# facebookresearch/gtn

Hardware: AMD Instinct MI355X
Metric: CTC forward+backward losses/sec (T=1000, C=256) (higher is better)
Workload: dtype f32; 1 GPU; BASELINE config C3: compose(ctc_target, emissions)+forwardScore CTC loss fwd+bwd, T=1000, C=256, U=100, batch=512 per GPU; global_batch=512, parallelism=dp1 (utterance sharding, all_gather of losses), rccl_ranks=0

## Files before the change

### gtn_amd/_capi.py

```python
import ctypes as C
import os

c_graph = C.c_void_p
c_graph_p = C.POINTER(C.c_void_p)
c_i32_p = C.POINTER(C.c_int)
c_i64_p = C.POINTER(C.c_int64)
c_u8_p = C.POINTER(C.c_uint8)
c_f32_p = C.POINTER(C.c_float)

GRAD_FN = C.CFUNCTYPE(C.c_int, C.c_void_p, c_graph_p, C.c_int, c_graph)
CTX_FREE = C.CFUNCTYPE(None, C.c_void_p)

OK, INVALID_ARGUMENT, LOGIC_ERROR, RUNTIME_ERROR, OUT_OF_RANGE, DEVICE_ERROR = range(6)

_SIGS = {
    "gtnx_set_device": [C.c_int],
    "gtnx_get_device": [c_i32_p],
    "gtnx_set_stream": [C.c_void_p],
    "gtnx_compose_mode": [C.c_int, C.POINTER(C.c_int)],
    "gtnx_synchronize": [],
    "gtnx_memory_stats": [C.POINTER(C.c_uint64), C.POINTER(C.c_uint64)],
    "gtnx_empty_cache": [],
    "gtnx_reclaim": [],
    "gtnx_graph_create": [C.c_int, c_graph_p],
# ... 5 lines not shown
    "gtnx_graph_add_nodes": [c_graph, C.c_int, C.c_void_p, C.c_void_p],
    "gtnx_graph_add_arcs": [c_graph, C.c_int, C.c_void_p, C.c_void_p, C.c_void_p, C.c_void_p, C.c_void_p],
    "gtnx_graph_num_nodes": [c_graph, c_i64_p],
    "gtnx_graph_num_arcs": [c_graph, c_i64_p],
    "gtnx_graph_num_start": [c_graph, c_i64_p],
    "gtnx_graph_num_accept": [c_graph, c_i64_p],
    "gtnx_graph_item": [c_graph, c_f32_p],
    "gtnx_graph_arc_sort": [c_graph, C.c_int],
    "gtnx_graph_mark_arc_sorted": [c_graph, C.c_int],
    "gtnx_graph_ilabel_sorted": [c_graph, c_i32_p],
    "gtnx_graph_olabel_sorted": [c_graph, c_i32_p],
    "gtnx_graph_weights": [c_graph, C.c_int, C.POINTER(c_f32_p)],
    "gtnx_graph_get_weights": [c_graph, C.c_void_p],
    "gtnx_graph_set_weights": [c_graph, C.c_void_p],
    "gtnx_graph_set_weights_device": [c_graph, C.c_void_p],
    "gtnx_graph_weights_device": [c_graph, C.POINTER(C.c_void_p)],
    "gtnx_graph_labels_to_array": [c_graph, C.c_void_p, C.c_int],
    "gtnx_graph_get_start": [c_graph, C.c_void_p],
    "gtnx_graph_get_accept": [c_graph, C.c_void_p],
    "gtnx_graph_is_start": [c_graph, C.c_int, c_i32_p],
    "gtnx_graph_is_accept": [c_graph, C.c_int, c_i32_p],
    "gtnx_graph_make_accept": [c_graph, C.c_int],
    "gtnx_graph_num_out": [c_graph, C.c_int, c_i64_p],
    "gtnx_graph_num_in": [c_graph, C.c_int, c_i64_p],
    "gtnx_graph_get_out": [c_graph, C.c_int, C.c_void_p],
    "gtnx_graph_get_in": [c_graph, C.c_int, C.c_void_p],
    "gtnx_graph_get_arcs": [c_graph, C.c_void_p, C.c_void_p, C.c_void_p, C.c_void_p],
    "gtnx_graph_get_arc": [c_graph, C.c_int, c_i32_p, c_i32_p, c_i32_p, c_i32_p, c_f32_p],
    "gtnx_graph_set_weight": [c_graph, C.c_int, C.c_float],
    "gtnx_graph_calc_grad": [c_graph, c_i32_p],
    "gtnx_graph_set_calc_grad": [c_graph, C.c_int],
    "gtnx_graph_is_grad_available": [c_graph, c_i32_p],
    "gtnx_graph_grad": [c_graph, c_graph_p],
    "gtnx_graph_zero_grad": [c_graph],
    "gtnx_graph_add_grad": [c_graph, C.c_void_p, C.c_int64],
    "gtnx_graph_add_grad_graph": [c_graph, c_graph],
    "gtnx_graph_id": [c_graph, C.POINTER(C.c_size_t)],
    "gtnx_graph_create_op": [c_graph_p, C.c_int, GRAD_FN, C.c_void_p, CTX_FREE, c_graph_p],
    "gtnx_graph_num_inputs": [c_graph, c_i64_p],
    "gtnx_graph_get_input": [c_graph, C.c_int, c_graph_p],
    "gtnx_graph_set_inputs": [c_graph, c_graph_p, C.c_int],
    "gtnx_graph_set_grad_fn": [c_graph, GRAD_FN, C.c_void_p, CTX_FREE],
    "gtnx_graph_has_grad_fn": [c_graph, c_i32_p],
    "gtnx_scalar_graph": [C.c_float, C.c_int, c_graph_p],
    "gtnx_linear_graph": [C.c_int, C.c_int, C.c_int, c_graph_p],
    "gtnx_linear_graph_n": [C.c_int, C.c_int, C.c_int, C.c_int, C.c_void_p, c_graph_p],
    "gtnx_linear_graph_borrow_n": [C.c_int, C.c_int, C.c_int, C.c_int, C.c_void_p, c_graph_p],
    "gtnx_negate": [c_graph, c_graph_p],
    "gtnx_add": [c_graph, c_graph, c_graph_p],
    "gtnx_subtract": [c_graph, c_graph, c_graph_p],
    "gtnx_compose": [c_graph, c_graph, c_graph_p],
    "gtnx_intersect": [c_graph, c_graph, c_graph_p],
    "gtnx_forward_score": [c_graph, c_graph_p],
    "gtnx_viterbi_score": [c_graph, c_graph_p],
    "gtnx_viterbi_path": [c_graph, c_graph_p],
    "gtnx_negate_n": [c_graph_p, C.c_int, c_graph_p],
    "gtnx_add_n": [c_graph_p, C.c_int, c_graph_p, C.c_int, c_graph_p],
    "gtnx_subtract_n": [c_graph_p, C.c_int, c_graph_p, C.c_int, c_graph_p],
    "gtnx_compose_n": [c_graph_p, C.c_int, c_graph_p, C.c_int, c_graph_p],
    "gtnx_intersect_n": [c_graph_p, C.c_int, c_graph_p, C.c_int, c_graph_p],
    "gtnx_forward_score_n": [c_graph_p, C.c_int, c_graph_p],
    "gtnx_viterbi_score_n": [c_graph_p, C.c_int, c_graph_p],
    "gtnx_viterbi_path_n": [c_graph_p, C.c_int, c_graph_p],
    "gtnx_items_n": [c_graph_p, C.c_int, C.c_void_p],
    "gtnx_items_device_n": [c_graph_p, C.c_int, C.c_void_p],
    "gtnx_grads_device_n": [c_graph_p, C.c_int, C.c_void_p, C.c_void_p],
    "gtnx_grads_bind_device_n": [c_graph_p, C.c_int, C.c_void_p, C.c_void_p],
    "gtnx_clone": [c_graph, C.c_int, c_graph_p],
    "gtnx_concat": [c_graph_p, C.c_int, c_graph_p],
    "gtnx_closure": [c_graph, c_graph_p],
    "gtnx_union": [c_graph_p, C.c_int, c_graph_p],
    "gtnx_batch_from_graphs": [c_graph_p, C.c_int, c_graph_p],
    "gtnx_batch_ctc_targets": [C.c_void_p, C.c_void_p, C.c_int, C.c_int, C.c_int, c_graph_p],
    "gtnx_batch_asg_force_align": [C.c_void_p, C.c_void_p, C.c_int, c_graph, C.c_int, c_graph_p],
    "gtnx_batch_linear": [C.c_int, C.c_int, C.c_int, C.c_int, C.c_void_p, C.c_int, c_graph_p],
    "gtnx_batch_linear_rows": [C.c_int, C.c_int, C.c_int, C.c_void_p, C.c_int, C.c_void_p, C.c_int, c_graph_p],
    "gtnx_batch_destroy": [c_graph],
    "gtnx_batch_size": [c_graph, c_i32_p],
    "gtnx_batch_get": [c_graph, C.c_int, c_graph_p],
    "gtnx_batch_negate": [c_graph, c_graph_p],
    "gtnx_batch_add": [c_graph, c_graph, c_graph_p],
    "gtnx_batch_subtract": [c_graph, c_graph, c_graph_p],
    "gtnx_batch_subtract_into": [c_graph, c_graph, C.c_void_p, c_graph_p],
    "gtnx_batch_compose": [c_graph, c_graph, c_graph_p],
    "gtnx_batch_intersect": [c_graph, c_graph, c_graph_p],
    "gtnx_batch_forward_score": [c_graph, c_graph_p],
    "gtnx_batch_viterbi_score": [c_graph, c_graph_p],
    "gtnx_batch_viterbi_path": [c_graph, c_graph_p],
    "gtnx_batch_viterbi_align": [c_graph, C.c_void_p, C.c_void_p, C.c_int64, C.c_void_p, C.c_void_p],
    "gtnx_batch_align_stats": [c_i64_p, c_i64_p],
    "gtnx_batch_viterbi_decode": [c_graph, c_graph, C.c_void_p, C.c_void_p, C.c_int64, C.c_void_p, C.c_void_p,
                                  C.c_void_p],
    "gtnx_batch_decode_stats": [c_i64_p, c_i64_p],
    "gtnx_batch_full_connect_stats": [c_i64_p, c_i64_p],
    "gtnx_batch_linear_decode": [c_graph, C.c_void_p, C.c_int, C.c_void_p, C.c_int64, C.c_void_p, C.c_void_p,
                                 C.c_void_p, C.c_void_p],
    "gtnx_batch_linear_decode_stats": [c_i64_p, c_i64_p],
    "gtnx_batch_ctc_beam_decode": [c_graph, C.c_void_p, C.c_int, C.c_int, C.c_int, C.c_int, C.c_void_p, C.c_int64,
                                   C.c_void_p, C.c_void_p],
    "gtnx_batch_ctc_beam_stats": [c_i64_p, c_i64_p],
    "gtnx_batch_linear_shape": [c_graph, c_i32_p, c_i32_p],
    "gtnx_batch_edit_distance": [C.c_void_p, C.c_int64, C.c_void_p, C.c_void_p, C.c_int64, C.c_void_p, C.c_int, C.c_int,
                                 C.c_int, C.c_int, C.c_void_p, C.c_void_p],
    "gtnx_batch_edit_distance_stats": [c_i64_p, c_i64_p],
    "gtnx_batch_backward": [c_graph, C.c_int],
    "gtnx_batch_items": [c_graph, C.c_void_p],
    "gtnx_batch_items_device": [c_graph, C.c_void_p],
    "gtnx_batch_grads_bind_device": [c_graph, C.c_void_p, C.c_void_p],
    "gtnx_batch_grads_device": [c_graph, C.c_void_p, C.c_void_p],
    "gtnx_backward": [c_graph, C.c_int],
    "gtnx_backward_with_grad": [c_graph, c_graph, C.c_int],
    "gtnx_backward_n": [c_graph_p, C.c_int, C.c_int],
    "gtnx_equal": [c_graph, c_graph, c_i32_p],
    "gtnx_isomorphic": [c_graph, c_graph, c_i32_p],
    "gtnx_remove": [c_graph, C.c_int, C.c_int, c_graph_p],
    "gtnx_graph_load_buffer": [C.c_void_p, C.c_size_t, c_graph_p],
    "gtnx_parallel_enter": [],
    "gtnx_parallel_leave": [],
    "gtnx_parallel_flush": [],
    "gtnx_prof_enable": [C.c_int],
    "gtnx_prof_reset": [],
    "gtnx_prof_get": [C.c_char_p, C.POINTER(C.c_double), c_i64_p, C.POINTER(C.c_double)],
    "gtnx_prof_names": [C.c_char_p, C.c_size_t],
    "gtnx_debug_symbolic_route": [c_graph, C.c_int, c_i32_p],
    "gtnx_debug_route_name": [C.c_int, C.c_char_p, C.c_size_t],
    "gtnx_debug_viterbi_ties": [c_i64_p, c_i64_p],
    "gtnx_debug_tie_ranks": [c_graph, C.c_void_p, C.c_void_p, C.c_void_p],
    "gtnx_comm_create": [c_i32_p, C.c_int, C.POINTER(C.c_void_p)],
    "gtnx_comm_destroy": [C.c_void_p],
    "gtnx_comm_size": [C.c_void_p, c_i32_p],
    "gtnx_comm_all_gather_f32": [C.c_void_p, C.POINTER(C.c_void_p), C.POINTER(C.c_void_p), C.c_int64],
    "gtnx_comm_all_reduce_sum_f32": [C.c_void_p, C.POINTER(C.c_void_p), C.c_int64],
}

_RESTYPE = {
    "gtnx_last_error": (C.c_char_p, []),
    "gtnx_version": (C.c_char_p, []),
    "gtnx_backend": (C.c_char_p, []),
    "gtnx_device_count": (C.c_int, []),
}

ALL_SYMBOLS = sorted(list(_SIGS) + list(_RESTYPE))


def default_library_path():
    return os.path.join(os.path.dirname(os.path.abspath(__file__)), "lib", "libgtn_amd.so")


def load(path=None):
    path = path or default_library_path()
    if not os.path.exists(path):
        raise ImportError(
            f"gtn_amd: native library not found at {path}. Build it with "
            "`python -c 'import __graft_entry__ as g; g.build()'` (hipcc, gfx950). "
            "There is no CPU fallback."
        )
    lib = C.CDLL(path, mode=C.RTLD_GLOBAL if hasattr(C, "RTLD_GLOBAL") else 0)
    for name, args in _SIGS.items():
        try:
            fn = getattr(lib, name)
        except AttributeError:
            if name.startswith("gtnx_batch_") or name.startswith("gtnx_comm_") or name in ("gtnx_linear_graph_borrow_n", "gtnx_grads_bind_device_n",
                                                             "gtnx_parallel_enter", "gtnx_parallel_leave", "gtnx_parallel_flush"):
                continue
            raise
        fn.argtypes = args
# ... 8 lines not shown
```

### gtn_amd/api.py

```python
import ctypes as C
import types

import numpy as np

from . import _capi

_EXC = {
    _capi.INVALID_ARGUMENT: ValueError,
    _capi.LOGIC_ERROR: RuntimeError,
    _capi.RUNTIME_ERROR: RuntimeError,
    _capi.OUT_OF_RANGE: IndexError,
    _capi.DEVICE_ERROR: RuntimeError,
}


class GtnError(RuntimeError):
    pass


def _is_seq(x):
    return isinstance(x, (list, tuple))


def make_api(lib):
# ... 698 lines not shown
                if stride is not None and t.stride(0) != stride:
                    raise ValueError("linear_decode: labels_out, collapsed_out and starts_out must have the same "
                                     "row stride")
                stride = t.stride(0)
            if stride is None:
                raise ValueError("linear_decode: a device address needs row_stride")
            if (lengths_out is not None or starts_out is not None) and collapsed_out is None:
                raise ValueError("linear_decode: lengths_out and starts_out need collapsed_out")
            fr = None if frames is None else np.ascontiguousarray(frames, dtype=np.int32)
            if fr is not None and fr.shape != (n,):
                raise ValueError("linear_decode: one frame count per element")
            check(lib.gtnx_batch_linear_decode(self._h, fr.ctypes.data if fr is not None else None, int(blank),
                                               _as_dev_ptr(labels_out), int(stride),
                                               _as_dev_ptr(scores_out) if scores_out is not None else None,
                                               _as_dev_ptr(collapsed_out) if collapsed_out is not None else None,
                                               _as_dev_ptr(starts_out) if starts_out is not None else None,
                                               _as_dev_ptr(lengths_out) if lengths_out is not None else None))

        def ctc_beam_decode(self, tokens_out, lengths_out, scores_out, frames=None, blank=0, beam_size=16,
                            cutoff_top_n=16, nbest=1, row_stride=None):
            n = len(self)
            stride = row_stride
            t = tokens_out
            if t is not None and hasattr(t, "data_ptr"):
                if (str(t.dtype) != "torch.int32" or t.dim() != 3 or t.shape[0] < n or t.shape[1] != int(nbest)
                        or (t.shape[2] > 1 and t.stride(2) != 1) or (n > 1 and t.stride(0) != t.shape[1] * t.stride(1))):
                    raise ValueError("ctc_beam_decode: tokens_out must be an int32 tensor [B, nbest, M] with contiguous "
                                     "rows, equally spaced")
                if stride is not None and t.stride(1) != stride:
                    raise ValueError("ctc_beam_decode: row_stride is not the row stride of tokens_out")
                stride = t.stride(1)
                m, c = C.c_int(-1), C.c_int(-1)
                check(lib.gtnx_batch_linear_shape(self._h, C.byref(m), C.byref(c)))
                if t.shape[2] < m.value:
                    raise ValueError(f"ctc_beam_decode: tokens_out has rows of {t.shape[2]} entries, the batch has "
                                     f"{m.value} rows")
            if stride is None:
                raise ValueError("ctc_beam_decode: a device address needs row_stride")
            for o, dt, what in ((lengths_out, "torch.int32", "lengths_out must be an int32"),
                                (scores_out, "torch.float32", "scores_out must be a float32")):
                if o is not None and hasattr(o, "data_ptr") and (str(o.dtype) != dt or not o.is_contiguous()
                                                                 or o.numel() < n * int(nbest)):
                    raise ValueError(f"ctc_beam_decode: {what} contiguous tensor [B, nbest]")
            fr = None if frames is None else np.ascontiguousarray(frames, dtype=np.int32)
            if fr is not None and fr.shape != (n,):
                raise ValueError("ctc_beam_decode: one frame count per element")
            check(lib.gtnx_batch_ctc_beam_decode(self._h, fr.ctypes.data if fr is not None else None, int(blank),
                                                 int(beam_size), int(cutoff_top_n), int(nbest),
                                                 _as_dev_ptr(tokens_out) if tokens_out is not None else None,
                                                 int(stride),
                                                 _as_dev_ptr(lengths_out) if lengths_out is not None else None,
                                                 _as_dev_ptr(scores_out) if scores_out is not None else None))

    ns.Batch = Batch

    def _batch_fn(cfn, *args):
        h = C.c_void_p()
        check(cfn(*[a._h for a in args], C.byref(h)))
        return Batch._from_handle(h.value)

    def _with_batches(plain, cfn):
        def f(*args, **kw):
            if args and all(isinstance(a, Batch) for a in args) and not kw:
                return _batch_fn(cfn, *args)
            return plain(*args, **kw)
        f.__doc__ = plain.__doc__
        f.__name__ = getattr(plain, "__name__", "f")
        return f

    if hasattr(lib, "gtnx_batch_negate"):
        for _name in ("negate", "add", "subtract", "compose", "intersect", "forward_score", "viterbi_score",
                      "viterbi_path"):
            setattr(ns, _name, _with_batches(getattr(ns, _name), getattr(lib, "gtnx_batch_" + _name)))

    def subtract_into(a, b, items_device):
        h = C.c_void_p()
        check(lib.gtnx_batch_subtract_into(a._h, b._h, _as_dev_ptr(items_device), C.byref(h)))
        r = Batch._from_handle(h.value)
        r._keep = items_device
        return r

    if hasattr(lib, "gtnx_batch_subtract_into"):
        ns.subtract_into = subtract_into

    _plain_backward = ns.backward

    def backward(g, grad_or_retain=None, retain_graph=False):
        if isinstance(g, Batch):
            r = grad_or_retain if isinstance(grad_or_retain, bool) else retain_graph
            check(lib.gtnx_batch_backward(g._h, int(bool(r))))
            return
        return _plain_backward(g, grad_or_retain, retain_graph)

    ns.backward = backward

    def parallel_for(fn, iterable):
        for i in iterable:
            fn(i)

    ns.parallel_for = parallel_for

    def backend():
        return lib.gtnx_backend().decode()

    def device_count():
        return lib.gtnx_device_count()

    def synchronize():
        check(lib.gtnx_synchronize())

    def set_device(i):
        check(lib.gtnx_set_device(int(i)))

    def set_stream(stream):
        check(lib.gtnx_set_stream(int(stream) if stream else None))

    def compose_mode(mode):
        prev = C.c_int()
        check(lib.gtnx_compose_mode(int(mode), C.byref(prev)))
        return prev.value

    def memory_stats():
        r, u = C.c_uint64(), C.c_uint64()
        check(lib.gtnx_memory_stats(C.byref(r), C.byref(u)))
        return {"reserved": r.value, "in_use": u.value}

    def prof_enable(on=True):
        check(lib.gtnx_prof_enable(int(bool(on))))

    def prof_reset():
        check(lib.gtnx_prof_reset())

    def prof_get(name):
        ms, n, b = C.c_double(), C.c_int64(), C.c_double()
        check(lib.gtnx_prof_get(name.encode(), C.byref(ms), C.byref(n), C.byref(b)))
        return {"total_ms": ms.value, "launches": n.value, "algorithmic_bytes": b.value}

    def prof_names():
        buf = C.create_string_buffer(4096)
        check(lib.gtnx_prof_names(buf, 4096))
        return [s for s in buf.value.decode().split("\n") if s]

    def debug_symbolic_route(g, tropical=False):
        r = C.c_int(-1)
        check(lib.gtnx_debug_symbolic_route(g._h, int(bool(tropical)), C.byref(r)))
        if r.value < 0:
            return None
        buf = C.create_string_buffer(32)
        check(lib.gtnx_debug_route_name(r.value, buf, 32))
        return buf.value.decode()

    def debug_viterbi_ties():
        a, b = C.c_int64(0), C.c_int64(0)
        check(lib.gtnx_debug_viterbi_ties(C.byref(a), C.byref(b)))
        return int(a.value), int(b.value)

    def debug_align_stats():
        a, b = C.c_int64(0), C.c_int64(0)
        check(lib.gtnx_batch_align_stats(C.byref(a), C.byref(b)))
        return int(a.value), int(b.value)

    def debug_decode_stats():
        a, b = C.c_int64(0), C.c_int64(0)
        check(lib.gtnx_batch_decode_stats(C.byref(a), C.byref(b)))
        return int(a.value), int(b.value)

# ... 137 lines not shown
```

### gtn_amd/criteria/ctc_criterion.h

```cpp
#pragma once

#include <chrono>
#include <cstdint>
#include <stdexcept>
#include <vector>

#include "gtn/gtn.h"

namespace gtn {
namespace criteria {

inline Graph ctcTargetGraph(const std::vector<int>& target, int blank = 0, bool calcGrad = true) {
  const int L = 2 * (int)target.size() + 1;
  std::vector<uint8_t> st(L, 0), ac(L, 0);
  std::vector<int> src, dst, lab;
  src.reserve(3 * L);
  dst.reserve(3 * L);
  lab.reserve(3 * L);
  for (int l = 0; l < L; l++) {
    const int idx = (l - 1) / 2;
    st[l] = l == 0;
    ac[l] = l == L - 1 || l + 2 == L;
    const int label = l % 2 ? target[idx] : blank;
    src.push_back(l), dst.push_back(l), lab.push_back(label);
    if (l > 0) src.push_back(l - 1), dst.push_back(l), lab.push_back(label);
    if (l % 2 && l > 1 && label != target[idx - 1]) src.push_back(l - 2), dst.push_back(l), lab.push_back(label);
  }
  Graph ctc(calcGrad);
  detail::check(gtnx_graph_add_nodes(ctc.handle(), L, st.data(), ac.data()));
  detail::check(gtnx_graph_add_arcs(ctc.handle(), (int)src.size(), src.data(), dst.data(), lab.data(), lab.data(), nullptr));
  ctc.arcSort();
  return ctc;
}

struct CtcStepTimes {
  double build = 0, linear = 0, intersect = 0, forward = 0, backward = 0;
};

inline void ctcLossBatch(
    const void* emissions,
    const int* labels,
    const int* lengths,
    int B,
    int T,
    int C,
    int blank,
    void* lossDev,
    void* gradDev,
    bool targetGrad = true,
    CtcStepTimes* times = nullptr,
    Batch* targetsOut = nullptr,
    const int* frames = nullptr) {
  auto now = [] { return std::chrono::steady_clock::now(); };
  auto ms = [](auto a, auto b) { return std::chrono::duration<double, std::milli>(b - a).count(); };
  if (frames)
    for (int b = 0; b < B; ++b)
      if (frames[b] < 1 || frames[b] > T) throw std::invalid_argument("[ctcLossBatch] a frame count outside 1 .. T");
  auto t0 = now();
  Batch ctcs = Batch::ctcTargets(labels, lengths, B, blank, targetGrad);
  auto t1 = now();
  Batch ems = Batch::linear(B, T, C, emissions, gradDev != nullptr, true, frames);
  std::vector<int64_t> off(B);
  for (int b = 0; b < B; ++b) off[b] = (int64_t)b * T * C;
  if (gradDev) ems.bindGrads(gradDev, off.data());
  auto t2 = now();
  Batch comp = batched::intersect(ctcs, ems);
  auto t3 = now();
  Batch score = batched::forwardScore(comp);
  Batch norm = batched::forwardScore(ems);
  Batch losses = batched::subtract(norm, score, lossDev);
  auto t4 = now();
  if (gradDev) batched::backward(losses);
  auto t5 = now();
  if (times) *times = {ms(t0, t1), ms(t1, t2), ms(t2, t3), ms(t3, t4), ms(t4, t5)};
  losses.itemsToDevice(lossDev);
  if (gradDev) ems.gradsToDevice(gradDev, off.data());
  if (targetsOut) *targetsOut = std::move(ctcs);
}

inline void ctcLossBatch(
    const void* emissions,
    const std::vector<std::vector<int>>& targets,
    int T,
    int C,
    int blank,
    void* lossDev,
    void* gradDev,
    bool targetGrad = true,
    CtcStepTimes* times = nullptr) {
  std::vector<int> flat, len;
  for (auto& t : targets) {
    flat.insert(flat.end(), t.begin(), t.end());
    len.push_back((int)t.size());
  }
  ctcLossBatch(emissions, flat.data(), len.data(), (int)targets.size(), T, C, blank, lossDev, gradDev, targetGrad, times);
}

inline void ctcAlignBatch(
    const void* emissions,
    const int* targets,
    const int* lengths,
    int B,
    int T,
    int C,
    int blank,
    const int* frames,
    void* labels,
    void* tokens,
    void* scores) {
  Batch ctcs = Batch::ctcTargets(targets, lengths, B, blank, false);
  Batch ems = Batch::linear(B, T, C, emissions, false, true);
  Batch comp = batched::intersect(ctcs, ems);
  batched::viterbiAlign(comp, static_cast<int*>(labels), T, static_cast<int*>(tokens), static_cast<float*>(scores), frames);
}

inline void ctcDecodeBatch(
    const void* emissions,
    int B,
    int T,
    int C,
    int blank,
    const int* frames,
    void* labelsDev,
    void* scoresDev,
    void* collapsedDev,
    void* startsDev,
    void* lengthsDev) {
  Batch ems = Batch::linear(B, T, C, emissions, false, true);
  batched::linearDecode(ems, static_cast<int*>(labelsDev), T, static_cast<float*>(scoresDev), frames, blank,
                        static_cast<int*>(collapsedDev), static_cast<int*>(startsDev), static_cast<int*>(lengthsDev));
}

inline void ctcBeamDecodeBatch(
    const void* emissions,
    int B,
    int T,
    int C,
    int blank,
    const int* frames,
    int beamSize,
    int cutoffTopN,
    int nbest,
    void* tokensDev,
    void* lengthsDev,
    void* scoresDev) {
  Batch ems = Batch::linear(B, T, C, emissions, false, true);
  batched::ctcBeamDecode(ems, static_cast<int*>(tokensDev), T, static_cast<int*>(lengthsDev),
                         static_cast<float*>(scoresDev), blank, beamSize, cutoffTopN, nbest, frames);
}

}
}
```

### gtn_amd/csrc/band.hip

```cpp
#include <hip/hip_runtime.h>

#include <algorithm>
#include <cstdlib>
#include <stdexcept>
#include <type_traits>

#include "kernels.h"

#ifdef GTNX_BAND_TIMING
__device__ long long g_band_timing[256];
#endif

namespace gtnx {
namespace {

constexpr float NEGF = -1.0e30f;
constexpr float DEADF = -1.0e29f;
constexpr float LOG2E = 1.44269504088896340736f;
constexpr double LN2 = 0.693147180559945309417;
constexpr int BW = 256;
constexpr int WG = 512;
constexpr int WGB = 768;
constexpr int NBE = 5;
constexpr int NBG = 7;
// ... 242 lines not shown
      for (int i = 0; i < NS / 4; ++i) {
        if (i > 0 && 4 * i * LN >= cnt) break;
        if (4 * (i * LN + tid) < cnt) {
          const int e = min(4 * (i * LN + tid), cnt - 4);
          const int r0 = row_of(e, W, invW), c0 = e - r0 * W;
#pragma unroll
          for (int k = 0; k < 4; ++k) {
            int r = r0, col = c0 + k;
            if (col >= W) {
              col -= W;
              ++r;
            }
            f(i, e + k, r, col, gtnx_f4{v[4 * i + k], 0.0f, 0.0f, 0.0f});
          }
        }
      }
    }
  }
};

struct BandLds {
  int CS;
  int o_ering, o_aring, o_oring, o_snode, o_misc, total;
};
__host__ __device__ inline BandLds band_lds(int C, int K, int NSmax, bool backward) {
  BandLds L;
  L.CS = C + 4;
  int o = 0;
  L.o_ering = o;
  o += (backward ? NBGE : NBE) * K * L.CS;
  o = (o + 3) & ~3;
  L.o_aring = o;
  o += backward ? NBE * K * NSmax : 0;
  o = (o + 3) & ~3;
  L.o_oring = o;
  o += backward ? max(NBG * K * NSmax, 2 * C) : 0;
  o = (o + 3) & ~3;
  L.o_snode = o;
  o += backward ? 512 : 0;
  L.o_misc = o;
  o += 160 + 32 + 8 + 2 * NBE * K * 4 + 40 * K + 8 + 512;
  L.total = o;
  return L;
}
struct BandMisc {
  double *offr, *red, *find, *aofr;
  float *bndr, *fin, *lsep;
};
template <int K>
__device__ __forceinline__ BandMisc band_misc(float* lds, const BandLds& L) {
  BandMisc m;
  m.offr = reinterpret_cast<double*>(lds + L.o_misc);
  m.red = m.offr + 80;
  m.find = m.red + 16;
  m.aofr = m.find + 4;
  m.bndr = lds + L.o_misc + 200 + 2 * NBE * K * 4;
  m.fin = m.bndr + 40 * K;
  m.lsep = m.fin + 8;
  return m;
}

__device__ __forceinline__ float wave_max_of(const float* v, int n) {
  float mx = v[0];
  for (int j = 1; j < n; ++j) mx = fmaxf(mx, v[j]);
  return wave_max(mx);
}

template <int NPL, bool UNIT, int K, bool VEC>
__global__ __launch_bounds__(WG) void band_forward_kernel(const BandPair* __restrict__ pairs, int NSmax) {
#define GTNX_BAND_PAIR pairs[blockIdx.x]
#include "band_forward_body.inc"
#undef GTNX_BAND_PAIR
}
template <int NPL, bool UNIT, int K, bool VEC>
__global__ __launch_bounds__(WG) void band_forward_one_kernel(BandPair one, int NSmax) {
#define GTNX_BAND_PAIR one
#include "band_forward_body.inc"
#undef GTNX_BAND_PAIR
}

__device__ __forceinline__ BandPair band_patched(BandPair P, const BandPatch& pt) {
  if (pt.on) {
    const int b = P.bidx;
    P.delta = pt.delta + b;
    P.delta_norm = pt.delta_norm ? pt.delta_norm + b : nullptr;
    P.rowlse = pt.rowlse ? pt.rowlse + int64_t(b) * pt.M : nullptr;
    P.norm = nullptr;
    P.em_copy = nullptr;
    P.grad_em = pt.grad_em ? pt.grad_em + int64_t(b) * pt.A : nullptr;
    P.grad_fixed = pt.grad_fixed ? pt.grad_fixed + P.goff : nullptr;
  }
  return P;
}
template <int NPL, bool UNIT, bool GRADG, int K, bool VEC, bool BIG>
__global__ __launch_bounds__(WGB, BIG ? 3 : 6) void band_backward_kernel(const BandPair* __restrict__ pairs, int NSmax, BandPatch patch) {
#define GTNX_BAND_PAIR band_patched(pairs[blockIdx.x], patch)
#include "band_backward_body.inc"
#undef GTNX_BAND_PAIR
}
template <int NPL, bool UNIT, bool GRADG, int K, bool VEC, bool BIG>
__global__ __launch_bounds__(WGB, BIG ? 3 : 6) void band_backward_one_kernel(BandPair one, int NSmax) {
#define GTNX_BAND_PAIR one
#include "band_backward_body.inc"
#undef GTNX_BAND_PAIR
}


__global__ __launch_bounds__(512) void ctc_targets_kernel(const CtcTargetArgs* __restrict__ args, int blank) {
  const CtcTargetArgs a = args[blockIdx.x];
  __shared__ __attribute__((aligned(16))) int tl[256 + 4];
  __shared__ __attribute__((aligned(16))) int tk[256 + 4];
  const int N = a.N, U = (N - 1) >> 1, m = threadIdx.x;
  if (m < 260) {
    const int v = m < U ? a.labels[m] : 0x7fffffff;
    tl[m] = v;
    tk[m] = (m > 0 && m < U && v != a.labels[m - 1]) ? 1 : 0;
  }
  __syncthreads();
  if (m >= N) return;
  const bool odd = (m & 1) != 0;
  const int my = odd ? tl[(m - 1) >> 1] : blank;
  const int skip = odd ? tk[(m - 1) >> 1] : 0;
  const int mi = (m - 1) >> 1;
  const int before = odd ? mi : (m >> 1);
  int rank = 0, skips = 0;
  for (int o = 0; o < U; o += 4) {
    const gtnx_i4 l4 = *reinterpret_cast<const gtnx_i4*>(tl + o), k4 = *reinterpret_cast<const gtnx_i4*>(tk + o);
    const int lo[4] = {l4.x, l4.y, l4.z, l4.w}, ko[4] = {k4.x, k4.y, k4.z, k4.w};
#pragma unroll
    for (int k = 0; k < 4; ++k) {
      const bool front = o + k < before;
      rank += (lo[k] < my || (lo[k] == my && front)) ? 1 : 0;
      skips += front ? ko[k] : 0;
    }
  }
  rank += blank < my ? U + 1 : (blank == my ? (m + 1) >> 1 : 0);
  const int base = (m > 0 ? 2 * m - 1 : 0) + skips;
  GTNX_G BandNode* nd = const_cast<GTNX_G BandNode*>(a.nodes);
  nd[m].lab = my;
  nd[m].aid[0] = base;
  nd[m].aid[1] = m > 0 ? base + 1 : -1;
  nd[m].aid[2] = skip ? base + 2 : -1;
  a.nflags[m] = uint8_t((m == 0 ? NF_START : 0) | (m + 2 >= N ? NF_ACCEPT : 0));
  a.snode[rank] = m;
  a.slab[rank] = my;
  if (m == N - 1 && a.n_arcs) a.n_arcs[0] = base + 1 + (m > 0 ? 1 : 0) + skip;
}

__global__ __launch_bounds__(512) void band_viterbi_kernel(const BandDecode* __restrict__ pairs) {
  const BandDecode P = pairs[blockIdx.x];
  const int T = P.T, C = P.C, N = P.N, NS = P.NS;
  extern __shared__ float lds[];
  const float NINF = -__builtin_inff();
  float* a0 = lds;
  float* a1 = lds + 516;
  float* stage = lds + 1032;
  const int m = threadIdx.x;
  const GTNX_G gtnx_i4* nodes = reinterpret_cast<const GTNX_G gtnx_i4*>(P.nodes);
  int lab = 0;
  float wi[3] = {NINF, NINF, NINF};
  bool accept = false, start = false;
  if (m < N) {
    const gtnx_i4 q = nodes[m];
    lab = q.x >= 0 ? q.x : 0;
    const int a[3] = {q.y, q.z, q.w};
#pragma unroll
    for (int k = 0; k < 3; ++k)
      if (a[k] >= 0) wi[k] = P.w ? P.w[a[k]] : 0.0f;
    const uint8_t f = P.nflags[m];
    start = (f & NF_START) != 0;
    accept = (f & NF_ACCEPT) != 0;
  }
  if (m < 2) a0[m] = a1[m] = NINF;
  a0[2 + m] = start ? 0.0f : NINF;
  a1[2 + m] = NINF;
  int tie = 0;
  const int R = max(1, min(64, P.stage_floats / C));
  float* cur = a0;
  float* nxt = a1;
  __syncthreads();
  for (int t0 = 0; t0 < T; t0 += R) {
    const int rows = min(R, T - t0);
    for (int e = threadIdx.x; e < rows * C; e += blockDim.x) stage[e] = P.em[int64_t(t0) * C + e];
    __syncthreads();
    for (int i = 0; i < rows; ++i) {
      const float e = stage[i * C + lab];
      const float c0 = cur[2 + m] + (wi[0] + e), c1 = cur[1 + m] + (wi[1] + e), c2 = cur[m] + (wi[2] + e);
      float best = c0;
      int k = 0;
      if (c1 > best) best = c1, k = 1;
      if (c2 > best) best = c2, k = 2;
      if (best > NINF && ((k != 0 && c0 == best) || (k != 1 && c1 == best) || (k != 2 && c2 == best))) tie = 1;
      if (m < NS) P.bp[int64_t(t0 + i) * NS + m] = uint8_t(best > NINF ? k : 3);
      nxt[2 + m] = m < N ? best : NINF;
      __syncthreads();
      float* sw = cur;
      cur = nxt;
      nxt = sw;
    }
  }
  __shared__ float red_v[8];
  __shared__ int red_m[8], s_best, s_tie;
  float v = accept ? cur[2 + m] : NINF;
  int bm = (m < N && accept && v > NINF) ? m : 1 << 30;
  const float wmx = wave_max(v);
  if (!(v == wmx)) bm = 1 << 30;
  int cnt = (bm != (1 << 30)) ? 1 : 0;
  for (int o = 32; o > 0; o >>= 1) {
    bm = min(bm, __shfl_xor(bm, o));
    cnt += __shfl_xor(cnt, o);
  }
  if ((threadIdx.x & 63) == 0) {
    red_v[threadIdx.x >> 6] = wmx;
    red_m[threadIdx.x >> 6] = bm;
  }
  if (cnt > 1) tie = 1;
  if (threadIdx.x == 0) s_tie = 0;
  __syncthreads();
  if (threadIdx.x == 0) {
    float bv = NINF;
    int bn = -1;
    for (int w = 0; w < 8; ++w) {
      if (red_m[w] == (1 << 30)) continue;
      if (red_v[w] > bv) bv = red_v[w], bn = red_m[w];
      else if (red_v[w] == bv && bv > NINF) s_tie = 1;
    }
    s_best = bn;
    P.score[0] = bv;
  }
// ... 419 lines not shown
  return 0;
}

bool band_one_ok(int npl, int C, int max_NS, bool vec, bool backward) {
  if (npl != 1 || !vec) return false;
  if (!backward) return true;
  const int K = band_block_rows(C, max_NS, true);
  return !(K * C > 1024 || K * max_NS > 1024);
}
void launch_band_forward(const BandPair* d_pairs, int n, int npl, int C, int max_NS, bool unit, bool vec, hipStream_t st,
                         const BandPair* one) {
  if (n <= 0) return;
  if (one && (n != 1 || !band_one_ok(npl, C, max_NS, vec, false))) throw std::logic_error("band.hip: not a single-pair launch");
  const int K = band_block_rows(C, 0, false);
  const size_t lds = 4 * size_t(band_lds(C, K, max_NS, false).total) + 64;
  if (npl == 1) {
    if (K == 8) launch_fwd<1, 8>(d_pairs, one, n, max_NS, lds, unit, vec, st);
    else if (K == 4) launch_fwd<1, 4>(d_pairs, one, n, max_NS, lds, unit, vec, st);
    else launch_fwd<1, 2>(d_pairs, one, n, max_NS, lds, unit, vec, st);
  } else {
    if (K == 8) launch_fwd<2, 8>(d_pairs, one, n, max_NS, lds, unit, vec, st);
    else if (K == 4) launch_fwd<2, 4>(d_pairs, one, n, max_NS, lds, unit, vec, st);
    else launch_fwd<2, 2>(d_pairs, one, n, max_NS, lds, unit, vec, st);
  }
}

void launch_band_backward(const BandPair* d_pairs, int n, int npl, int C, int max_NS, bool unit, bool gradg, bool vec,
                          hipStream_t st, const BandPair* one, const BandPatch* patch) {
  if (n <= 0) return;
  if (one && patch) throw std::logic_error("band.hip: a patched launch reads a device table");
  BandPatch pt{};
  if (patch) pt = *patch;
  if (one && (n != 1 || !band_one_ok(npl, C, max_NS, vec, true))) throw std::logic_error("band.hip: not a single-pair launch");
  const int K = band_block_rows(C, max_NS, true);
  const bool big = K * C > 1024 || K * max_NS > 1024;
  const int ns_lds = band_backward_lds_stride(K, max_NS);
  const size_t lds = 4 * size_t(band_lds(C, K, ns_lds, true).total) + 64;
  if (npl == 1) {
    if (K == 4) launch_bwd<1, 4>(d_pairs, one, n, ns_lds, lds, unit, gradg, vec, big, st, pt);
    else launch_bwd<1, 2>(d_pairs, one, n, ns_lds, lds, unit, gradg, vec, big, st, pt);
  } else {
    if (K == 4) throw std::logic_error("band.hip: four rows per block with two nodes per lane");
    launch_bwd<2, 2>(d_pairs, one, n, ns_lds, lds, unit, gradg, vec, big, st, pt);
  }
}

template <int NPL>
static void launch_viterbi_wave(const BandDecode* d_pairs, int n, int ranked, hipStream_t st) {
  if (ranked) hipLaunchKernelGGL((band_viterbi_wave_kernel<NPL, true>), dim3(n), dim3(64), 0, st, d_pairs);
  else hipLaunchKernelGGL((band_viterbi_wave_kernel<NPL, false>), dim3(n), dim3(64), 0, st, d_pairs);
}
bool band_viterbi_wave_ok(int max_nodes, int max_labels, int vec) {
  static const bool force_wg = std::getenv("GTNX_VITERBI_WG") != nullptr;
  return !force_wg && vec && max_nodes <= 512 && max_labels <= VBLK;
}
void launch_band_viterbi(const BandDecode* d_pairs, int n, int stage_floats, int max_nodes, int max_labels, int vec,
                         hipStream_t st, int ranked) {
  if (n <= 0) return;
  if (band_viterbi_wave_ok(max_nodes, max_labels, vec)) {
    if (max_nodes <= 64) launch_viterbi_wave<1>(d_pairs, n, ranked, st);
    else if (max_nodes <= 128) launch_viterbi_wave<2>(d_pairs, n, ranked, st);
    else if (max_nodes <= 256) launch_viterbi_wave<4>(d_pairs, n, ranked, st);
    else launch_viterbi_wave<8>(d_pairs, n, ranked, st);
    return;
  }
  if (ranked) return;
  static std::atomic<uint64_t> done{0};
  if (gtnx_first_on_device first{done}) big_lds(band_viterbi_kernel);
  hipLaunchKernelGGL(band_viterbi_kernel, dim3(n), dim3(512), 4 * size_t(1032 + stage_floats) + 64, st, d_pairs);
}

void launch_asg_fal_targets(const AsgFalArgs* d_args, int n, int n_labels, hipStream_t st) {
  if (n > 0) hipLaunchKernelGGL(asg_fal_targets_kernel, dim3(n), dim3(512), 0, st, d_args, n_labels);
}
void launch_asg_fal_scatter(const float* g, const int* maps, const int64_t* tab, int n_seq, int64_t longest, float* trans_grad,
                            hipStream_t st) {
  if (n_seq > 0 && longest > 0)
    hipLaunchKernelGGL(asg_fal_scatter_kernel, dim3(unsigned(std::min<int64_t>((longest + 255) / 256, 64)), unsigned(n_seq)),
                       dim3(256), 0, st, g, maps, tab, trans_grad);
}
void launch_ctc_targets(const CtcTargetArgs* d_args, int n, int blank, hipStream_t st) {
  if (n > 0) hipLaunchKernelGGL(ctc_targets_kernel, dim3(n), dim3(512), 0, st, d_args, blank);
}

}
```

### gtn_amd/csrc/batch.cpp

```cpp
#include "batch.h"

#include <algorithm>
#include <atomic>
#include <cstdlib>
#include <cstring>
#include <limits>
#include <unordered_map>
#include <unordered_set>

namespace gtnx {

namespace {

std::atomic<uint64_t> g_batch_seq{1};

struct CompMode {
  int old;
  CompMode() : old(compose_mode_hint(2)) {}
  ~CompMode() { compose_mode_hint(old); }
};

BatchP make_batch(Batch::Kind k, int n, bool cg) {
  auto b = std::make_shared<Batch>();
  b->kind = k;
  b->n = n;
  b->calc_grad = cg;
  return b;
}

BatchP result(Batch::Kind k, int n, std::shared_ptr<BatchOp> op) {
  bool cg = false;
  for (auto& i : op->inputs) cg |= i->calc_grad;
  BatchP r = make_batch(k, n, cg);
  op->seq = g_batch_seq.fetch_add(1);
  r->op = std::move(op);
  return r;
}

bool native(const Batch& b, Batch::Kind k) { return b.kind == k; }

void pad_fill(Batch& b, float* base, const int64_t* offs = nullptr) {
  if (b.kind != Batch::LINEAR || b.pad_floats <= 0) return;
  Runtime& rt = Runtime::get();
  const size_t n = size_t(b.n);
  const size_t rows_bytes = align_up(sizeof(int) * n, 256);
  if (!b.pad_mem) {
    std::vector<int64_t> tab(rows_bytes / 8 + n + 1);
    std::memcpy(tab.data(), b.rows.data(), sizeof(int) * n);
    int64_t* prefix = tab.data() + rows_bytes / 8;
    prefix[0] = 0;
    for (size_t i = 0; i < n; ++i) prefix[i + 1] = prefix[i] + int64_t(b.M - b.rows[i]) * b.C;
    b.pad_mem = upload_vec(tab);
  }
  PadFillArgs a{};
  a.base = base;
  a.rows = b.pad_mem->as<int>();
  a.prefix = reinterpret_cast<const int64_t*>(b.pad_mem->as<char>(rows_bytes));
  a.stride = int64_t(b.M) * b.C;
  a.n = b.n;
  a.C = b.C;
  DevMemP d_offs;
  if (offs) {
    d_offs = upload_vec(std::vector<int64_t>(offs, offs + n));
    a.offs = d_offs->as<int64_t>();
  }
  GTNX_PROF("linear_pad_fill", 4.0 * double(b.pad_floats));
  launch_pad_fill(a, b.pad_floats, rt.stream());
}

void alloc_grad(Batch& b, bool zero) {
  Runtime& rt = Runtime::get();
  b.g_off.resize(size_t(b.n) + 1);
  b.g_off[0] = 0;
  for (int i = 0; i < b.n; ++i) b.g_off[size_t(i) + 1] = b.g_off[size_t(i)] + b.elem_size(i);
  const size_t bytes = sizeof(float) * size_t(b.g_off[size_t(b.n)]);
  if (b.dest) {
    b.g_mem = b.dest_mem;
    b.g_dev = b.dest;
    b.dest = nullptr;
    if (zero && bytes) HIP_CHECK(hipMemsetAsync(b.g_dev, 0, bytes, rt.stream()));
  } else {
    b.g_mem = zero ? rt.alloc_zero(bytes ? bytes : 4) : rt.alloc(bytes ? bytes : 4);
    b.g_dev = b.g_mem->as<float>();
  }
  if (!zero) pad_fill(b, b.g_dev);
}

struct GradTarget {
  float* ptr = nullptr;
  DevMemP scratch;
};
GradTarget grad_target(Batch& b, bool zero) {
  GradTarget t;
  if (!b.g_dev) {
    alloc_grad(b, zero);
    t.ptr = b.g_dev;
    return t;
  }
  Runtime& rt = Runtime::get();
  const size_t bytes = sizeof(float) * size_t(b.g_off[size_t(b.n)]);
  t.scratch = zero ? rt.alloc_zero(bytes ? bytes : 4) : rt.alloc(bytes ? bytes : 4);
  t.ptr = t.scratch->as<float>();
  if (!zero) pad_fill(b, t.ptr);
  return t;
}
void add_scratch(Batch& b, const GradTarget& t) {
  if (!t.scratch) return;
  launch_vec_axpby(b.g_dev, t.ptr, nullptr, size_t(b.g_off[size_t(b.n)]), 1.0f, 0.0f, 1, Runtime::get().stream());
}

struct BScalarOp : BatchOp {
  ScalarKind kind;
  void backward(Batch& out) override {
    Runtime& rt = Runtime::get();
    for (size_t i = 0; i < inputs.size(); ++i) {
      Batch& in = *inputs[i];
      if (!in.calc_grad) continue;
      const float s = (kind == SK_NEGATE || (kind == SK_SUBTRACT && i == 1)) ? -1.0f : 1.0f;
      const bool have = in.g_dev != nullptr;
      if (!have) alloc_grad(in, false);
      launch_vec_axpby(in.g_dev, out.g_dev, nullptr, size_t(in.n), s, 0.0f, have ? 1 : 0, rt.stream());
    }
  }
};

struct BackwardPlan {
  std::unordered_map<Batch*, Batch*> lin;
  std::unordered_set<Batch*> fused;
};
thread_local BackwardPlan* t_plan = nullptr;
thread_local bool t_batch_retain = false;

struct BFsLinearOp : BatchOp {
  void backward(Batch& out) override {
    Batch& e = *inputs[0];
    if (!e.calc_grad) return;
    if (t_plan && e.nc_rowlse && !t_plan->lin.count(&e)) {
      t_plan->lin[&e] = &out;
      return;
    }
    run(out);
  }
  void run(Batch& out) {
    Batch& e = *inputs[0];
    Runtime& rt = Runtime::get();
    if (e.w_pend) e.w_pend->settle();
    const bool have = e.g_dev != nullptr;
    if (!have) alloc_grad(e, false);
    std::vector<LinArgs> args;
    args.resize(size_t(e.n));
    const size_t A = size_t(e.M) * size_t(e.C);
    for (int b = 0; b < e.n; ++b) {
      LinArgs& a = args[size_t(b)];
      a.w = e.w_dev + size_t(b) * A;
      a.M = e.rows_of(b);
      a.C = e.C;
      a.out_score = nullptr;
      a.partial = nullptr;
      a.delta = out.g_dev + b;
      a.grad = e.g_dev + size_t(b) * A;
      a.accumulate = have ? 1 : 0;
    }
    DevMemP d = upload_vec(args);
    const bool vec_rows = e.C % 4 == 0 && e.C <= 1024 && (reinterpret_cast<uintptr_t>(e.w_dev) & 15) == 0 &&
                          (reinterpret_cast<uintptr_t>(e.g_dev) & 15) == 0;
    GTNX_PROF("linear_forward_grad", (have ? 12.0 : 8.0) * double(A) * e.n);
    launch_linear_backward(d->as<LinArgs>(), e.n, 0, vec_rows ? 1 : 0, rt.stream());
  }
};

struct BFsBandOp : BatchOp {
  std::vector<BandPair> pairs;
  DevMemP arena;
  DevMemP fwd_table;
  DevMemP through_acc;
  void backward(Batch& out) override {
    Batch& prod = *inputs[0];
    Batch& fx = *prod.fixed;
    Batch& ch = *prod.chain;
    Runtime& rt = Runtime::get();
    const float* delta = out.g_dev;
    if (through_acc || t_batch_retain) {
      const size_t n = size_t(prod.n);
      if (!through_acc) through_acc = rt.alloc_zero(sizeof(float) * (n ? n : 1));
      launch_vec_axpby(through_acc->as<float>(), out.g_dev, nullptr, n, 1.0f, 0.0f, 1, rt.stream());
      delta = through_acc->as<float>();
    }
    GradTarget ge, gf;
    if (ch.calc_grad) ge = grad_target(ch, false);
    if (fx.calc_grad) gf = grad_target(fx, fx.fal);
    Batch* lin_out = nullptr;
    if (t_plan && ch.calc_grad && !ge.scratch) {
      auto it = t_plan->lin.find(&ch);
      if (it != t_plan->lin.end() && !t_plan->fused.count(&ch)) {
        lin_out = it->second;
        t_plan->fused.insert(&ch);
      }
    }
    std::vector<std::pair<BandLaunchKey, BandPair>> tab;
    tab.reserve(pairs.size());
    double bytes = 0;
    const size_t A = size_t(ch.M) * size_t(ch.C);
    bool one_key = true;
    int max_ns = 0;
    for (int b = 0; b < prod.n; ++b) {
      BandPair p = pairs[size_t(b)];
      p.delta = delta + b;
      p.delta_norm = lin_out ? lin_out->g_dev + b : nullptr;
      p.rowlse = lin_out ? ch.nc_rowlse + size_t(b) * size_t(ch.M) : nullptr;
      p.norm = nullptr;
      p.grad_em = ge.ptr ? ge.ptr + size_t(b) * A : nullptr;
      p.grad_fixed = gf.ptr ? gf.ptr + fx.g_off[size_t(b)] : nullptr;
      tab.push_back({BandLaunchKey{p.C, band_npl(p.N), fx.fal ? 0 : 1, p.grad_fixed ? 1 : 0, band_vec_ok(p)}, p});
      one_key = one_key && tab.back().first == tab.front().first;
      max_ns = std::max(max_ns, p.NS);
      bytes += 4.0 * p.T * p.C * (p.grad_em ? 2 : 1) + 4.0 * double(p.T + 1) * p.NS +
               (p.grad_fixed ? 4.0 * double(fx.elem_size(b)) : 0.0);
    }
    static const bool no_patch = std::getenv("GTNX_NO_BAND_PATCH") != nullptr;
    if (fwd_table && one_key && prod.n > 1 && !no_patch) {
      BandPatch pt{};
      pt.on = 1;
      pt.M = ch.M;
      pt.delta = delta;
      pt.delta_norm = lin_out ? lin_out->g_dev : nullptr;
      pt.rowlse = lin_out ? ch.nc_rowlse : nullptr;
      pt.grad_em = ge.ptr;
      pt.grad_fixed = gf.ptr;
      pt.A = int64_t(A);
      band_launch_patched(fwd_table, prod.n, tab.front().first, max_ns, pt, "band_forward_score_grad", bytes);
    } else {
      band_launch(tab, true, "band_forward_score_grad", bytes);
    }
    if (ch.calc_grad) add_scratch(ch, ge);
    if (fx.calc_grad) add_scratch(fx, gf);
    (void)rt;
  }
};


struct BFalOp : BatchOp {
  void backward(Batch& out) override {
    Graph& tr = out.trans;
    if (!tr.calc_grad() || !out.g_dev) return;
    Runtime& rt = Runtime::get();
    const int64_t A = tr.num_arcs();
    DevMemP gm = rt.alloc_zero(sizeof(float) * size_t(A ? A : 1));
    std::vector<int64_t> tab(size_t(out.n) * 3);
    int64_t longest = 0;
    for (int b = 0; b < out.n; ++b) {
      const int64_t len = out.g_off[size_t(b) + 1] - out.g_off[size_t(b)];
      tab[size_t(b) * 3 + 0] = out.g_off[size_t(b)];
      tab[size_t(b) * 3 + 1] = int64_t(out.map_off[size_t(b)] / sizeof(int));
      tab[size_t(b) * 3 + 2] = len;
      longest = std::max(longest, len);
    }
    DevMemP dt = upload_vec(tab);
    launch_asg_fal_scatter(out.g_dev, out.rec_mem->as<int>(), dt->as<int64_t>(), out.n, longest, gm->as<float>(), rt.stream());
    tr.add_grad_device(gm, gm->as<float>(), true);
  }
};

std::atomic<int64_t> g_full_fast{0}, g_full_fallback{0};
struct BFullOp : BatchOp {
  AsgFullArgs args{};
  DevMemP arena;
  DevMemP rows_mem;
  DevMemP w_mem;
  DevMemP through_acc;
  void backward(Batch& out) override {
    Batch& prod = *inputs[0];
    Batch& ch = *prod.chain;
    Graph& tr = prod.fixed->graphs[0];
    Runtime& rt = Runtime::get();
    const float* delta = out.g_dev;
    if (through_acc || t_batch_retain) {
      const size_t n = size_t(prod.n);
      if (!through_acc) through_acc = rt.alloc_zero(sizeof(float) * (n ? n : 1));
      launch_vec_axpby(through_acc->as<float>(), out.g_dev, nullptr, n, 1.0f, 0.0f, 1, rt.stream());
      delta = through_acc->as<float>();
    }
    const bool want_tr = tr.calc_grad();
    if (!ch.calc_grad && !want_tr) return;
    GradTarget ge;
    if (ch.calc_grad) ge = grad_target(ch, false);
    AsgFullArgs a = args;
    a.delta = delta;
    a.grad_em = ge.ptr;
    const size_t A = size_t(a.N) + size_t(a.N) * size_t(a.N);
    DevMemP part;
    if (want_tr) {
      part = rt.alloc(sizeof(float) * A * size_t(a.n));
      a.partial = part->as<float>();
    }
    {
      GTNX_PROF("asg_full_backward", 4.0 * double(a.n) * a.M * a.N * (ge.ptr ? 3 : 2) + (want_tr ? 4.0 * double(A) * a.n : 0.0));
      launch_asg_full_backward(a, rt.stream());
    }
    if (ch.calc_grad) add_scratch(ch, ge);
    if (want_tr) {
      DevMemP gm = rt.alloc(sizeof(float) * A);
      {
        GTNX_PROF("asg_full_reduce", 4.0 * double(A) * (a.n + 1));
        launch_asg_full_reduce(part->as<float>(), a.n, a.N, gm->as<float>(), rt.stream());
      }
      tr.add_grad_device(gm, gm->as<float>(), true);
    }
  }
};

struct BFromGraphsOp : BatchOp {
  DevMemP passed;
  void backward(Batch& out) override {
    Batch& src = *inputs[0];
    Runtime& rt = Runtime::get();
    const size_t n = size_t(src.n);
    DevMemP delta = rt.alloc(sizeof(float) * (n ? n : 1));
    if (passed)
      launch_vec_axpby(delta->as<float>(), out.g_dev, passed->as<float>(), n, 1.0f, -1.0f, 0, rt.stream());
    else
// ... 35 lines not shown
    const size_t e = std::min(graphs.size(), i + 32);
    part->reserve(e - i);
    for (size_t k = i; k < e; ++k) part->push_back(std::move(graphs[k]));
    rt.defer_delete(part, [](void* q) { delete static_cast<std::vector<Graph>*>(q); }, e - i);
  }
  graphs.clear();
}

int64_t Batch::elem_size(int b) const {
  switch (kind) {
    case SCALAR: return 1;
    case LINEAR: return int64_t(M) * C;
    case CTC_TARGETS:
      if (fal) return 2 * int64_t(lab_off[size_t(b) + 1] - lab_off[size_t(b)]);
      return 3 * int64_t(2 * (lab_off[size_t(b) + 1] - lab_off[size_t(b)]) + 1);
    default: return 0;
  }
}

BatchP batch_from_graphs(std::vector<Graph> gs) {
  bool cg = false;
  for (auto& g : gs) cg |= g.calc_grad();
  BatchP b = make_batch(Batch::GRAPHS, int(gs.size()), cg);
  b->graphs = std::move(gs);
  b->materialised = true;
  return b;
}

namespace {
Graph ctc_target_graph_host(const int* t, int U, int blank, bool cg) {
  const int L = 2 * U + 1;
  std::vector<uint8_t> st(size_t(L), 0), ac(size_t(L), 0);
  std::vector<int> src, dst, lab;
  src.reserve(size_t(3 * L));
  dst.reserve(size_t(3 * L));
  lab.reserve(size_t(3 * L));
  for (int l = 0; l < L; ++l) {
    const int idx = (l - 1) / 2;
    st[size_t(l)] = l == 0;
    ac[size_t(l)] = l == L - 1 || l + 2 == L;
    const int label = l % 2 ? t[idx] : blank;
    src.push_back(l), dst.push_back(l), lab.push_back(label);
    if (l > 0) src.push_back(l - 1), dst.push_back(l), lab.push_back(label);
    if (l % 2 && l > 1 && label != t[idx - 1]) src.push_back(l - 2), dst.push_back(l), lab.push_back(label);
  }
  Graph g(cg);
  g.add_nodes(L, st.data(), ac.data());
  g.add_arcs(int(src.size()), src.data(), dst.data(), lab.data(), lab.data(), nullptr);
  g.arc_sort(false);
  return g;
}
}

BatchP batch_ctc_targets(const int* labels, const int* lengths, int n, int blank, bool calc_grad) {
  GTNX_HOST_T("batch.ctc_targets");
  if (n < 0) throw_invalid("[gtnx_batch_ctc_targets] negative batch size");
  BatchP b = make_batch(Batch::CTC_TARGETS, n, calc_grad);
  b->blank = blank;
  b->lab_off.resize(size_t(n) + 1);
  b->lab_off[0] = 0;
  for (int i = 0; i < n; ++i) {
    if (lengths[i] < 0) throw_invalid("[gtnx_batch_ctc_targets] negative length");
    b->lab_off[size_t(i) + 1] = b->lab_off[size_t(i)] + lengths[i];
    b->max_nodes = std::max(b->max_nodes, 2 * lengths[i] + 1);
  }
  const size_t total = size_t(b->lab_off[size_t(n)]);
  b->labels.assign(labels, labels + total);
  int mn = blank;
  b->max_label = blank;
  for (size_t i = 0; i < total; ++i) {
    b->max_label = std::max(b->max_label, labels[i]);
    mn = std::min(mn, labels[i]);
  }
  if (mn < 0 || b->max_nodes > band_max_nodes() || n == 0) {
    std::vector<Graph> gs;
    gs.reserve(size_t(n));
    for (int i = 0; i < n; ++i)
      gs.push_back(ctc_target_graph_host(labels + b->lab_off[size_t(i)], lengths[i], blank, calc_grad));
    return batch_from_graphs(std::move(gs));
  }
  Runtime& rt = Runtime::get();
  const size_t lab_bytes = align_up(sizeof(int) * (total ? total : 1), 256);
  const size_t arg_bytes = align_up(sizeof(CtcTargetArgs) * size_t(n), 256);
  size_t bytes = lab_bytes + arg_bytes;
  b->rec_off.resize(size_t(n));
  for (int i = 0; i < n; ++i) {
    const size_t N = size_t(2 * lengths[i] + 1);
    b->rec_off[size_t(i)] = bytes;
    bytes += align_up(sizeof(BandNode) * N, 64) + align_up(N, 64) + 2 * align_up(4 * N, 64) + 64;
  }
  b->rec_mem = rt.alloc(bytes);
  PinnedMemP pin = rt.alloc_pinned(lab_bytes + arg_bytes);
  std::memcpy(pin->ptr, labels, sizeof(int) * total);
  CtcTargetArgs* args = reinterpret_cast<CtcTargetArgs*>(static_cast<char*>(pin->ptr) + lab_bytes);
  for (int i = 0; i < n; ++i) {
    const size_t N = size_t(2 * lengths[i] + 1);
    char* base = b->rec_mem->as<char>(b->rec_off[size_t(i)]);
    CtcTargetArgs& a = args[size_t(i)];
    a.labels = b->rec_mem->as<int>() + b->lab_off[size_t(i)];
    a.nodes = reinterpret_cast<BandNode*>(base);
    base += align_up(sizeof(BandNode) * N, 64);
    a.nflags = reinterpret_cast<uint8_t*>(base);
    base += align_up(N, 64);
    a.snode = reinterpret_cast<int*>(base);
    base += align_up(4 * N, 64);
    a.slab = reinterpret_cast<int*>(base);
    base += align_up(4 * N, 64);
    a.n_arcs = reinterpret_cast<int*>(base);
    a.N = int(N);
    a.pad = 0;
  }
  rt.h2d_pinned(b->rec_mem->ptr, pin->ptr, lab_bytes + arg_bytes);
  launch_ctc_targets(reinterpret_cast<const CtcTargetArgs*>(b->rec_mem->as<char>(lab_bytes)), n, blank, rt.stream());
  return b;
}


BatchP batch_asg_force_align(const int* labels, const int* lengths, int n, Graph& transitions, int n_labels) {
  if (n < 0) throw_invalid("[gtnx_batch_asg_force_align] negative batch size");
  if (transitions.num_nodes() != int64_t(n_labels) + 1 || transitions.num_arcs() != int64_t(n_labels) * (n_labels + 1))
    throw_invalid("[gtnx_batch_asg_force_align] the transitions graph must have the asgTransitions(N) layout");
  BatchP b = make_batch(Batch::CTC_TARGETS, n, transitions.calc_grad());
  b->fal = true;
  b->trans = transitions;
  b->trans_labels = n_labels;
  b->lab_off.resize(size_t(n) + 1);
  b->lab_off[0] = 0;
  int max_u = 0;
  for (int i = 0; i < n; ++i) {
    if (lengths[i] < 0) throw_invalid("[gtnx_batch_asg_force_align] negative length");
    b->lab_off[size_t(i) + 1] = b->lab_off[size_t(i)] + lengths[i];
    max_u = std::max(max_u, lengths[i]);
  }
  b->max_nodes = max_u + 1;
  const size_t total = size_t(b->lab_off[size_t(n)]);
  b->labels.assign(labels, labels + total);
  int mn = 0;
  for (size_t i = 0; i < total; ++i) {
    b->max_label = std::max(b->max_label, labels[i]);
    mn = std::min(mn, labels[i]);
  }
  if (mn < 0 || b->max_label >= n_labels || b->max_nodes > band_max_nodes() || n == 0) {
    b->kind = Batch::GRAPHS;
    batch_materialise(*b);
    return b;
  }
  Runtime& rt = Runtime::get();
  std::vector<Weights*> ws{transitions.w.get()};
  ensure_weights_device_batch(ws);
  size_t bytes = align_up(sizeof(int) * (total ? total : 1), 256);
  b->rec_off.resize(size_t(n));
  b->w_off.resize(size_t(n));
  b->map_off.resize(size_t(n));
  for (int i = 0; i < n; ++i) {
    const size_t N = size_t(lengths[i]) + 1, A = 2 * size_t(lengths[i]);
    b->rec_off[size_t(i)] = bytes;
    bytes += align_up(sizeof(BandNode) * N, 64) + align_up(N, 64) + 2 * align_up(4 * N, 64);
    b->w_off[size_t(i)] = bytes;
    bytes += align_up(4 * (A ? A : 1), 64);
    b->map_off[size_t(i)] = bytes;
    bytes += align_up(4 * (A ? A : 1), 64);
  }
  b->rec_mem = rt.alloc(bytes);
  {
    PinnedMemP pin = rt.alloc_pinned(sizeof(int) * (total ? total : 1));
    std::memcpy(pin->ptr, labels, sizeof(int) * total);
    rt.h2d_pinned(b->rec_mem->ptr, pin->ptr, sizeof(int) * total);
  }
  std::vector<AsgFalArgs> args;
  args.resize(size_t(n));
  for (int i = 0; i < n; ++i) {
    const size_t N = size_t(lengths[i]) + 1;
    char* base = b->rec_mem->as<char>(b->rec_off[size_t(i)]);
    AsgFalArgs& a = args[size_t(i)];
    a.labels = b->rec_mem->as<int>() + b->lab_off[size_t(i)];
    a.trans_w = transitions.w->dev;
    a.nodes = reinterpret_cast<BandNode*>(base);
    base += align_up(sizeof(BandNode) * N, 64);
    a.nflags = reinterpret_cast<uint8_t*>(base);
    base += align_up(N, 64);
    a.snode = reinterpret_cast<int*>(base);
    base += align_up(4 * N, 64);
    a.slab = reinterpret_cast<int*>(base);
    a.w = b->rec_mem->as<float>(b->w_off[size_t(i)]);
    a.arc_map = b->rec_mem->as<int>(b->map_off[size_t(i)]);
    a.U = lengths[i];
    a.pad = 0;
  }
  DevMemP d = upload_vec(args);
  launch_asg_fal_targets(d->as<AsgFalArgs>(), n, n_labels, rt.stream());
  auto op = std::make_shared<BFalOp>();
  op->seq = g_batch_seq.fetch_add(1);
  b->op = op;
  return b;
}

BatchP batch_linear(int n, int M, int C, bool calc_grad, const void* dev, bool borrow, const int* rows) {
  if (n < 0 || M < 0 || C < 0) throw_invalid("[gtnx_batch_linear] negative size");
  int64_t pad_rows = 0;
  if (rows)
    for (int i = 0; i < n; ++i) {
      if (rows[i] < 1 || rows[i] > M) throw_invalid("[gtnx_batch_linear_rows] a row count outside 1 .. M");
      pad_rows += M - rows[i];
    }
  Runtime& rt = Runtime::get();
  BatchP b = make_batch(Batch::LINEAR, n, calc_grad);
  b->M = M;
  b->C = C;
  const size_t bytes = sizeof(float) * size_t(n) * size_t(M) * size_t(C);
  if (borrow && dev) {
    b->w_mem = std::make_shared<DevMem>();
    b->w_mem->ptr = const_cast<void*>(dev);
    b->w_mem->bytes = bytes;
    b->w_mem->borrowed = true;
  } else {
    b->w_mem = dev ? rt.alloc(bytes ? bytes : 4) : rt.alloc_zero(bytes ? bytes : 4);
    if (dev && bytes) rt.d2d(b->w_mem->ptr, dev, bytes);
  }
  b->w_dev = b->w_mem->as<float>();
  if (pad_rows > 0) {
    b->rows.assign(rows, rows + n);
    b->pad_floats = pad_rows * C;
  }
  return b;
}

BatchP batch_ctc_targets_from_graphs(const std::vector<Graph>& gs) {
  GTNX_HOST_T("batch.ctc_targets_from_graphs");
  const int n = int(gs.size());
  if (n == 0) return nullptr;
  detect_ctc_shape(*gs[0].s);
  const Structure& s0 = *gs[0].s;
  if (!s0.ctc_labels) return nullptr;
  const bool cg = gs[0].calc_grad();
  std::vector<int> flat, len;
  len.reserve(size_t(n));
  flat.reserve(size_t(n) * s0.ctc_labels->size());
  for (auto& g : gs) {
    detect_ctc_shape(*g.s);
    const Structure& s = *g.s;
    if (!s.ctc_labels || s.ctc_blank != s0.ctc_blank || g.calc_grad() != cg || s.N > band_max_nodes() ||
        !g.w->is_all_zero())
      return nullptr;
    flat.insert(flat.end(), s.ctc_labels->begin(), s.ctc_labels->end());
    len.push_back(int(s.ctc_labels->size()));
  }
  BatchP b = batch_ctc_targets(flat.data(), len.data(), n, s0.ctc_blank, cg);
  if (b->kind != Batch::CTC_TARGETS) return nullptr;
  b->graphs = gs;
  b->leaf = true;
  for (auto& g : gs) g.s->leaf_batch = b;
  return b;
}

BatchP batch_linear_from_graphs(const std::vector<Graph>& gs) {
  GTNX_HOST_T("batch.linear_from_graphs");
  const int n = int(gs.size());
  if (n == 0) return nullptr;
  const Structure& s0 = *gs[0].s;
  if (s0.kind != KIND_LINEAR || s0.M < 1 || s0.C < 1) return nullptr;
  const bool cg = gs[0].calc_grad();
  std::vector<Weights*> ws;
  ws.reserve(size_t(n));
  std::unordered_set<Weights*> distinct;
  for (auto& g : gs) {
    const Structure& s = *g.s;
    if (s.kind != KIND_LINEAR || s.M != s0.M || s.C != s0.C || g.calc_grad() != cg || g.w->host_escaped ||
        !distinct.insert(g.w.get()).second)
      return nullptr;
    ws.push_back(g.w.get());
  }
  ensure_weights_device_batch(ws);
  Runtime& rt = Runtime::get();
  const size_t A = size_t(s0.M) * size_t(s0.C);
  BatchP b = make_batch(Batch::LINEAR, n, cg);
  b->M = s0.M;
  b->C = s0.C;
  bool contiguous = true;
  for (int i = 0; i < n && contiguous; ++i)
    contiguous = ws[size_t(i)]->dev == ws[0]->dev + size_t(i) * A && ws[size_t(i)]->dev_mem == ws[0]->dev_mem;
  if (contiguous) {
    b->w_mem = ws[0]->dev_mem;
    b->w_dev = ws[0]->dev;
  } else {
    b->w_mem = rt.alloc(sizeof(float) * A * size_t(n));
    b->w_dev = b->w_mem->as<float>();
    std::vector<CopySeg> segs;
    segs.resize(size_t(n));
    for (int i = 0; i < n; ++i) segs[size_t(i)] = {b->w_dev + size_t(i) * A, ws[size_t(i)]->dev, int64_t(4 * A)};
    DevMemP d = upload_vec(segs);
    launch_copy_segments(d->as<CopySeg>(), n, int64_t(4 * A), rt.stream());
    for (int i = 0; i < n; ++i) {
      ws[size_t(i)]->dev_mem = b->w_mem;
      ws[size_t(i)]->dev = b->w_dev + size_t(i) * A;
    }
  }
  b->graphs = gs;
  b->leaf = true;
  for (auto& g : gs) {
    g.w->leaf_batch = b;
    g.w->leaf_version = g.w->version;
  }
  if (cg && gs[0].g->grad_dest && !gs[0].is_grad_available()) {
    bool block = true;
    for (int i = 0; i < n && block; ++i)
      block = gs[size_t(i)].g->grad_dest == gs[0].g->grad_dest + size_t(i) * A && !gs[size_t(i)].is_grad_available();
    if (block) {
      b->dest_mem = gs[0].g->grad_dest_mem;
      b->dest = gs[0].g->grad_dest;
    }
  }
  return b;
}

namespace {
void push_grads_to_graphs(Batch& x) {
  if (!x.g_dev) return;
  GTNX_HOST_T("batch.push_grads_to_graphs");
  GradSink sink;
  const size_t n = size_t(x.n);
  for (size_t i = 0; i < n; ++i) {
    if (i + 6 < n) __builtin_prefetch(x.graphs[i + 6].g.get(), 1);
    if (i + 3 < n) __builtin_prefetch(x.graphs[i + 3].s.get(), 1);
    Graph& g = x.graphs[i];
    if (!g.calc_grad()) continue;
    float* ptr = x.g_dev + x.g_off[i];
    if (!g.s->deferred) {
      std::lock_guard<std::mutex> lk(g.s->grad_lock);
      if (!g.is_grad_available()) {
        g.g->lazy_owner = x.g_mem;
        g.g->lazy_ptr = ptr;
// ... 224 lines not shown
    std::vector<Weights*> ws{tr.w.get()};
    ensure_weights_device_batch(ws);
    const int n = x->n, M = ch.M, N = ch.C;
    const bool keep = x->calc_grad;
    auto op = std::make_shared<BFullOp>();
    op->inputs = {x};
    size_t bytes = align_up(4 * size_t(n), 256);
    const size_t o_zd = bytes;
    bytes = align_up(bytes + 8 * size_t(n), 256);
    const size_t o_L = bytes;
    if (keep) bytes = align_up(bytes + 8 * size_t(n) * size_t(M), 256);
    const size_t o_la = bytes;
    if (keep) bytes += 4 * size_t(n) * size_t(M) * size_t(N);
    op->arena = rt.alloc(bytes);
    if (!ch.rows.empty()) op->rows_mem = upload_vec(ch.rows);
    op->w_mem = tr.w->dev_mem;
    AsgFullArgs& a = op->args;
    a.em = ch.w_dev;
    a.rows = op->rows_mem ? op->rows_mem->as<int>() : nullptr;
    a.w = tr.w->dev;
    a.score = op->arena->as<float>();
    a.zd = op->arena->as<double>(o_zd);
    a.L = keep ? op->arena->as<double>(o_L) : nullptr;
    a.la = keep ? op->arena->as<float>(o_la) : nullptr;
    a.n = n;
    a.M = M;
    a.N = N;
    int64_t frames = 0;
    for (int b = 0; b < n; ++b) frames += ch.rows_of(b);
    {
      GTNX_PROF("asg_full_forward", 4.0 * double(frames) * N * (keep ? 2 : 1));
      launch_asg_full_forward(a, rt.stream());
    }
    g_full_fast.fetch_add(n);
    DevMemP arena = op->arena;
    BatchP r = result(Batch::SCALAR, n, op);
    r->v_mem = arena;
    r->v_dev = arena->as<float>();
    return r;
  }
  if (!tropical && native(*x, Batch::PRODUCT) && !x->materialised && !x->wide && !x->full) {
    Batch& fx = *x->fixed;
    Batch& ch = *x->chain;
    const int n = x->n, T = ch.M, C = ch.C;
    auto op = std::make_shared<BFsBandOp>();
    op->inputs = {x};
    const bool want_norm = ch.nc_norm == nullptr;
    size_t bytes = align_up(4 * size_t(n), 256);
    const size_t o_norm = bytes;
    bytes = align_up(bytes + 4 * size_t(n), 256);
    const size_t o_lse = bytes;
    bytes = align_up(bytes + 4 * size_t(n) * size_t(T > 0 ? T : 1), 256);
    std::vector<size_t> oo, ao;
    oo.resize(size_t(n));
    ao.resize(size_t(n));
    for (int b = 0; b < n; ++b) {
      const int Ub = fx.lab_off[size_t(b) + 1] - fx.lab_off[size_t(b)];
      const int N = fx.fal ? Ub + 1 : 2 * Ub + 1;
      const int ns = band_row_stride(N, band_npl(N));
      oo[size_t(b)] = bytes;
      bytes = align_up(bytes + 8 * (4 * size_t(T) + 16), 256);
      ao[size_t(b)] = bytes;
      bytes = align_up(bytes + 4 * size_t(T + 1) * size_t(ns), 256);
    }
    op->arena = rt.alloc(bytes);
    op->pairs.resize(size_t(n));
    std::vector<std::pair<BandLaunchKey, BandPair>> tab;
    tab.reserve(size_t(n));
    double abytes = 0;
    std::shared_ptr<PendingCopy> pend = ch.w_pend;
    std::unique_lock<std::mutex> pend_lock;
    bool fuse_copy = false;
    if (pend && !pend->done.load(std::memory_order_acquire)) {
      pend_lock = std::unique_lock<std::mutex>(pend->mu);
      fuse_copy = !pend->done.load(std::memory_order_relaxed) && pend->device == rt.device();
      const size_t A = size_t(T) * size_t(C);
      for (int b = 0; b < n && fuse_copy; ++b) fuse_copy = pend->src_of(ch.w_dev + size_t(b) * A) != nullptr;
      fuse_copy = fuse_copy && pend->segs.size() == size_t(n);
      if (!fuse_copy) {
        pend_lock.unlock();
        pend->settle();
      }
    }
    int64_t goff_run = 0;
    for (int b = 0; b < n; ++b) {
      BandPair& p = op->pairs[size_t(b)];
      p = BandPair{};
      const int U = fx.lab_off[size_t(b) + 1] - fx.lab_off[size_t(b)];
      const size_t N = fx.fal ? size_t(U) + 1 : size_t(2 * U + 1);
      char* base = fx.rec_mem->as<char>(fx.rec_off[size_t(b)]);
      p.nodes = reinterpret_cast<BandNode*>(base);
      base += align_up(sizeof(BandNode) * N, 64);
      p.nflags = reinterpret_cast<uint8_t*>(base);
      base += align_up(N, 64);
      p.snode = reinterpret_cast<int*>(base);
      base += align_up(4 * N, 64);
      p.slab = reinterpret_cast<int*>(base);
      p.n_lab = fx.fal ? U : int(N);
      p.w = fx.fal ? fx.rec_mem->as<float>(fx.w_off[size_t(b)]) : nullptr;
      p.em = ch.w_dev + size_t(b) * size_t(T) * size_t(C);
      p.N = int(N);
      p.T = ch.rows_of(b);
      p.C = C;
      p.NS = band_row_stride(p.N, band_npl(p.N));
      p.alpha = op->arena->as<float>(ao[size_t(b)]);
      p.aoff = op->arena->as<double>(oo[size_t(b)]);
      p.score = op->arena->as<float>(4 * size_t(b));
      if (want_norm) {
        p.norm = op->arena->as<float>(o_norm + 4 * size_t(b));
        p.rowlse = op->arena->as<float>(o_lse + 4 * size_t(b) * size_t(T));
      }
      p.hot = (!fx.fal && U + 1 >= 8) ? fx.blank : -1;
      p.lgrn = band_forward_lgrn(C);
      p.bidx = b;
      p.goff = goff_run;
      goff_run += int64_t(fx.elem_size(b));
      BandPair q = p;
      if (fuse_copy) {
        q.em = static_cast<const float*>(pend->src_of(p.em));
        q.em_copy = const_cast<float*>(p.em);
      }
      tab.push_back({BandLaunchKey{C, band_npl(q.N), fx.fal ? 0 : 1, 0, band_vec_ok(q)}, q});
      abytes += 4.0 * p.T * C + 4.0 * double(p.T + 1) * p.NS + (fuse_copy ? 4.0 * T * C : 0.0);
    }
    band_launch(tab, false, "band_forward_score", abytes, fuse_copy ? nullptr : &op->fwd_table);
    if (fuse_copy) pend->done.store(true, std::memory_order_release);
    if (want_norm) {
      ch.nc_mem = op->arena;
      ch.nc_norm = op->arena->as<float>(o_norm);
      ch.nc_rowlse = op->arena->as<float>(o_lse);
    }
    DevMemP arena = op->arena;
    BatchP r = result(Batch::SCALAR, n, op);
    r->v_mem = arena;
    r->v_dev = arena->as<float>();
    return r;
  }
  if (!tropical && native(*x, Batch::LINEAR) && !x->materialised && x->nc_norm) {
    auto op = std::make_shared<BFsLinearOp>();
    op->inputs = {x};
    BatchP r = result(Batch::SCALAR, x->n, op);
    r->v_mem = x->nc_mem;
    r->v_dev = x->nc_norm;
    return r;
  }
  if (!tropical && native(*x, Batch::LINEAR) && !x->materialised && x->n > 0 && x->M > 0) {
    if (x->w_pend) x->w_pend->settle();
    auto op = std::make_shared<BFsLinearOp>();
    op->inputs = {x};
    const int n = x->n;
    DevMemP res = rt.alloc(sizeof(float) * size_t(n) * 9);
    float* scal = res->as<float>();
    float* partial = scal + n;
    std::vector<LinArgs> args;
    args.resize(size_t(n));
    const size_t A = size_t(x->M) * size_t(x->C);
    for (int b = 0; b < n; ++b) {
      LinArgs& a = args[size_t(b)];
      a.w = x->w_dev + size_t(b) * A;
      a.M = x->rows_of(b);
      a.C = x->C;
      a.out_score = scal + b;
      a.partial = partial + size_t(b) * 8;
      a.delta = nullptr;
      a.grad = nullptr;
      a.accumulate = 0;
    }
    DevMemP d = upload_vec(args);
    const bool vec_rows = x->C % 4 == 0 && x->C <= 1024 && (reinterpret_cast<uintptr_t>(x->w_dev) & 15) == 0 && (A % 4) == 0;
    {
      GTNX_PROF("linear_forward", 4.0 * double(A) * n);
      launch_linear_forward(d->as<LinArgs>(), n, 0, vec_rows ? 1 : 0, rt.stream());
    }
    BatchP r = result(Batch::SCALAR, n, op);
    r->v_mem = res;
    r->v_dev = scal;
    return r;
  }
  batch_materialise(*x);
  return batch_from_graphs(op_shortest_distance(x->graphs, tropical));
}

BatchP batch_viterbi_path(const BatchP& x) {
  batch_materialise(*x);
  return batch_from_graphs(op_viterbi_path(x->graphs));
}

namespace {
std::atomic<int64_t> g_align_fast{0}, g_align_fallback{0};

void align_fallback(const BatchP& x, const int* frames, int* labels_dev, int64_t row_stride, int* tokens_dev,
                    float* scores_dev) {
  if (tokens_dev)
    throw_invalid("[gtnx_batch_viterbi_align] token indices are defined for device-built CTC targets or ASG force-alignment "
                  "acceptors composed with a linear batch only (this batch takes the path-graph route)");
  if (frames)
    throw_invalid("[gtnx_batch_viterbi_align] per-utterance frame counts need device-built CTC targets or ASG "
                  "force-alignment acceptors composed with a linear batch (this batch takes the path-graph route)");
  GTNX_HOST_T("batch.viterbi_align.fallback");
  Runtime& rt = Runtime::get();
  const int n = x->n;
  int64_t width = (x->kind == Batch::PRODUCT && x->chain && x->chain->kind == Batch::LINEAR) ? x->chain->M : 0;
  BatchP paths = batch_viterbi_path(x);
  for (int b = 0; b < n; ++b) width = std::max<int64_t>(width, paths->graphs[size_t(b)].num_arcs());
  if (width > row_stride) throw_invalid("[gtnx_batch_viterbi_align] row_stride is shorter than the longest path");
  PinnedMemP hl = rt.alloc_pinned(sizeof(int) * size_t(n) * size_t(width ? width : 1));
  PinnedMemP hs = rt.alloc_pinned(sizeof(float) * size_t(n));
  std::fill(hl->as<int>(), hl->as<int>() + size_t(n) * size_t(width), -1);
  for (int b = 0; b < n; ++b) {
    Graph& g = paths->graphs[size_t(b)];
    const int64_t len = g.num_arcs();
    float score = g.num_nodes() > 0 ? 0.0f : -std::numeric_limits<float>::infinity();
    if (len > 0) {
      g.s->ensure_host();
      std::copy(g.s->il.begin(), g.s->il.begin() + len, hl->as<int>() + size_t(b) * size_t(width));
      const float* w = g.weights_host(false);
      for (int64_t t = 0; t < len; ++t) score += w[t];
    }
    hs->as<float>()[b] = score;
  }
  if (width > 0)
    HIP_CHECK(hipMemcpy2DAsync(labels_dev, sizeof(int) * size_t(row_stride), hl->ptr, sizeof(int) * size_t(width),
                               sizeof(int) * size_t(width), size_t(n), hipMemcpyHostToDevice, rt.stream()));
  if (scores_dev) rt.h2d_pinned(scores_dev, hs->ptr, sizeof(float) * size_t(n));
  g_align_fallback.fetch_add(n);
}
}

void batch_align_stats(int64_t* fast, int64_t* fallback) {
  if (fast) *fast = g_align_fast.load();
  if (fallback) *fallback = g_align_fallback.load();
}

void batch_viterbi_align(const BatchP& x, const int* frames, int* labels_dev, int64_t row_stride, int* tokens_dev,
                         float* scores_dev) {
  GTNX_HOST_T("batch.viterbi_align");
  Runtime& rt = Runtime::get();
  if (!labels_dev) throw_invalid("[gtnx_batch_viterbi_align] null labels pointer");
  if (row_stride < 0) throw_invalid("[gtnx_batch_viterbi_align] negative row stride");
  const int n = x->n;
  if (n <= 0) return;
  if (!ptr_local_to(labels_dev, rt.device()) || (tokens_dev && !ptr_local_to(tokens_dev, rt.device())) ||
      (scores_dev && !ptr_local_to(scores_dev, rt.device())))
    throw_invalid("[gtnx_batch_viterbi_align] an output pointer is not memory of the engine's current device");
  bool fast = x->kind == Batch::PRODUCT && x->fixed && x->chain && x->fixed->kind == Batch::CTC_TARGETS && !x->fixed->fal &&
              x->chain->kind == Batch::LINEAR && x->fixed->rec_mem && x->fixed->n == n && x->chain->n == n;
  if (fast) {
    const Batch& fx = *x->fixed;
    const Batch& ch = *x->chain;
    const int vec = ch.C % 4 == 0 && (reinterpret_cast<uintptr_t>(ch.w_dev) & 15) == 0;
    fast = band_align_ok(fx.max_nodes, ch.C, vec) && fx.max_label < ch.C;
    for (size_t i = 0; i < fx.labels.size() && fast; ++i) fast = fx.labels[i] > fx.blank;
  }
  bool asg = x->kind == Batch::PRODUCT && x->fixed && x->chain && x->fixed->kind == Batch::CTC_TARGETS && x->fixed->fal &&
             x->chain->kind == Batch::LINEAR && x->fixed->rec_mem && x->fixed->n == n && x->chain->n == n;
  if (asg) {
    const Batch& fx = *x->fixed;
    const Batch& ch = *x->chain;
    const int vec = ch.C % 4 == 0 && (reinterpret_cast<uintptr_t>(ch.w_dev) & 15) == 0;
    asg = asg_align_ok(fx.max_nodes, ch.C, vec) && fx.trans_labels == ch.C && fx.max_label < ch.C;
  }
  if (!fast && !asg) {
    align_fallback(x, frames, labels_dev, row_stride, tokens_dev, scores_dev);
    return;
  }
  Batch& fx = *x->fixed;
  Batch& ch = *x->chain;
  const int T = ch.M, C = ch.C;
  if (row_stride < T) throw_invalid("[gtnx_batch_viterbi_align] row_stride is shorter than the chains");
  if (frames)
    for (int b = 0; b < n; ++b) {
      if (frames[b] < 0 || frames[b] > T) throw_invalid("[gtnx_batch_viterbi_align] a frame count outside 0 .. T");
      if (frames[b] > ch.rows_of(b))
        throw_invalid("[gtnx_batch_viterbi_align] a frame count beyond the rows the chain carries");
    }
  if (ch.w_pend) ch.w_pend->settle();
  if (asg) {
    const int npl = asg_align_npl(fx.max_nodes);
    const size_t plane = asg_align_plane_bytes(T, npl);
    DevMemP work = rt.alloc(plane * size_t(n));
    std::vector<AsgAlignArgs> tab(static_cast<size_t>(n));
    double abytes = 0;
    for (int b = 0; b < n; ++b) {
      AsgAlignArgs& a = tab[size_t(b)];
      a = AsgAlignArgs{};
      const int U = fx.lab_off[size_t(b) + 1] - fx.lab_off[size_t(b)];
      const size_t N = size_t(U) + 1;
      char* base = fx.rec_mem->as<char>(fx.rec_off[size_t(b)]);
      a.nodes = reinterpret_cast<BandNode*>(base);
      a.nflags = reinterpret_cast<uint8_t*>(base + align_up(sizeof(BandNode) * N, 64));
      a.w = fx.rec_mem->as<float>(fx.w_off[size_t(b)]);
      a.em = ch.w_dev + size_t(b) * size_t(T) * size_t(C);
      a.bp = work->as<unsigned>(plane * size_t(b));
      a.labels = labels_dev + int64_t(b) * row_stride;
      a.tokens = tokens_dev ? tokens_dev + int64_t(b) * row_stride : nullptr;
      a.score = scores_dev ? scores_dev + b : nullptr;
      a.N = int(N);
      a.T = frames ? frames[b] : ch.rows_of(b);
      a.T_full = T;
      a.C = C;
      abytes += 4.0 * a.T * C + 0.25 * double(a.T) * double(N) + 8.0 * a.T;
    }
    DevMemP d = upload_vec(tab);
    GTNX_PROF("asg_viterbi_align", abytes);
    launch_asg_align(d->as<AsgAlignArgs>(), n, fx.max_nodes, rt.stream());
    g_align_fast.fetch_add(n);
    return;
  }
  const int npl = align_npl(fx.max_nodes);
  const size_t plane = align_up((size_t(T) * size_t(npl) + 15) / 16 * 256 + 256, 256);
  DevMemP work = rt.alloc(plane * size_t(n));
  std::vector<AlignArgs> tab(static_cast<size_t>(n));
  double abytes = 0;
  for (int b = 0; b < n; ++b) {
    AlignArgs& a = tab[size_t(b)];
    a = AlignArgs{};
    const int* t = fx.labels.data() + fx.lab_off[size_t(b)];
    const int U = fx.lab_off[size_t(b) + 1] - fx.lab_off[size_t(b)];
    const size_t N = size_t(2 * U + 1);
    char* base = fx.rec_mem->as<char>(fx.rec_off[size_t(b)]);
    a.nodes = reinterpret_cast<BandNode*>(base);
    a.nflags = reinterpret_cast<uint8_t*>(base + align_up(sizeof(BandNode) * N, 64));
    a.em = ch.w_dev + size_t(b) * size_t(T) * size_t(C);
    a.bp = work->as<unsigned>(plane * size_t(b));
    a.labels = labels_dev + int64_t(b) * row_stride;
    a.tokens = tokens_dev ? tokens_dev + int64_t(b) * row_stride : nullptr;
    a.score = scores_dev ? scores_dev + b : nullptr;
    a.N = int(N);
    a.T = frames ? frames[b] : ch.rows_of(b);
    a.T_full = T;
    a.C = C;
    int p = 0;
    while (p + 1 < U && t[p] < t[p + 1]) ++p;
    a.p = p;
    abytes += 4.0 * a.T * C + 0.5 * double(a.T) * double(N) + 8.0 * a.T;
  }
  DevMemP d = upload_vec(tab);
  GTNX_PROF("band_viterbi_align", abytes);
  launch_band_align(d->as<AlignArgs>(), n, fx.max_nodes, rt.stream());
  g_align_fast.fetch_add(n);
}

namespace {
std::atomic<int64_t> g_decode_fast{0}, g_decode_fallback{0};

void decode_fallback(const BatchP& ems, Graph& transitions, const int* frames, int* labels_dev, int64_t row_stride,
                     float* scores_dev, int* collapsed_dev, int* lengths_dev) {
  if (frames)
    throw_invalid("[gtnx_batch_viterbi_decode] per-utterance frame counts need a linear batch and a dense transitions "
                  "graph of 8 .. 1024 nodes whose ties go by node order (this batch takes the path-graph route, which "
                  "decodes the rows the elements carry: pass frames = null)");
  GTNX_HOST_T("batch.viterbi_decode.fallback");
  Runtime& rt = Runtime::get();
  const int n = ems->n;
  batch_materialise(*ems);
  std::vector<Graph> tr{transitions};
  std::vector<Graph> comp = op_compose(ems->graphs, tr, false);
  std::vector<Graph> paths = op_viterbi_path(comp);
  int64_t width = ems->kind == Batch::LINEAR ? ems->M : 0;
// ... 370 lines not shown
  a.ops = ops_dev;
  a.hyp_stride = hyp_stride;
  a.ref_stride = ref_stride;
  a.N = N;
  a.L = L;
  a.U = U;
  a.nbU = nbU;
  const double io_bytes = double(pairs) * (4.0 * L + 8.0) + double(B) * (4.0 * U + 4.0);
  if (!ops_dev) {
    a.pair0 = 0;
    a.count = int(pairs);
    GTNX_PROF("edit_distance", io_bytes);
    launch_edit_distance(a, rt.stream());
  } else {
    const int64_t per_pair = int64_t(16) * L * nbU;
    const int64_t slice = per_pair > 0 ? std::max<int64_t>(1, edit_distance_scratch_cap() / per_pair) : pairs;
    for (int64_t p0 = 0; p0 < pairs; p0 += slice) {
      const int64_t cnt = std::min(slice, pairs - p0);
      DevMemP words = rt.alloc(size_t(std::max<int64_t>(per_pair * cnt, 16)));
      a.scratch = words->as<gtnx_ul2>();
      a.pair0 = p0;
      a.count = int(cnt);
      GTNX_PROF("edit_distance_ops", (io_bytes / double(pairs) + 2.0 * double(per_pair) + 12.0) * double(cnt));
      launch_edit_distance(a, rt.stream());
    }
  }
  g_edit_distance_calls.fetch_add(1);
  g_edit_distance_pairs.fetch_add(pairs);
}


namespace {
BatchP scalars_from_graphs(const BatchP& gsb) {
  Runtime& rt = Runtime::get();
  for (auto& g : gsb->graphs)
    if (g.num_arcs() != 1) return nullptr;
  auto op = std::make_shared<BFromGraphsOp>();
  op->inputs = {gsb};
  BatchP r = result(Batch::SCALAR, gsb->n, op);
  r->v_mem = rt.alloc(sizeof(float) * size_t(gsb->n ? gsb->n : 1));
  r->v_dev = r->v_mem->as<float>();
  items_device(gsb->graphs, r->v_dev);
  return r;
}
}

BatchP batch_scalar(ScalarKind k, const BatchP& a0, const BatchP& b0, void* items_dev) {
  BatchP a = a0, b = b0;
  const bool binary = k != SK_NEGATE;
  if (binary && a->n == b->n) {
    const bool an = a->kind == Batch::SCALAR && !a->materialised, bn = b->kind == Batch::SCALAR && !b->materialised;
    if (an && !bn && b->kind == Batch::GRAPHS) {
      if (BatchP w = scalars_from_graphs(b)) b = w;
    } else if (bn && !an && a->kind == Batch::GRAPHS) {
      if (BatchP w = scalars_from_graphs(a)) a = w;
    }
  }

  if (native(*a, Batch::SCALAR) && !a->materialised &&
      (!binary || (native(*b, Batch::SCALAR) && !b->materialised && b->n == a->n))) {
    Runtime& rt = Runtime::get();
    auto op = std::make_shared<BScalarOp>();
    op->kind = k;
    op->inputs = binary ? std::vector<BatchP>{a, b} : std::vector<BatchP>{a};
    BatchP r = result(Batch::SCALAR, a->n, op);
    if (items_dev) {
      r->v_dev = static_cast<float*>(items_dev);
    } else {
      r->v_mem = rt.alloc(sizeof(float) * size_t(a->n ? a->n : 1));
      r->v_dev = r->v_mem->as<float>();
    }
    launch_vec_axpby(r->v_dev, a->v_dev, binary ? b->v_dev : nullptr, size_t(a->n), k == SK_NEGATE ? -1.0f : 1.0f,
                     k == SK_SUBTRACT ? -1.0f : 1.0f, 0, rt.stream());
    return r;
  }
  batch_materialise(*a);
  std::vector<Graph> none;
  if (binary) batch_materialise(*b);
  BatchP r = batch_from_graphs(op_scalar(k, a->graphs, binary ? b->graphs : none));
  if (items_dev) batch_items_device(r, items_dev);
  return r;
}

void batch_backward(const BatchP& root, bool retain) {
  GTNX_HOST_T("batch.backward");
  if (root->tape_cleared)
    throw_invalid("[autograd::backward] Cannot Backward twice without retaining the graph.");
  if (root->materialised || !root->op || root->kind != Batch::SCALAR) {
    batch_materialise(*root);
    op_backward(root->graphs, nullptr, retain);
    return;
  }
  Runtime& rt = Runtime::get();
  std::vector<Batch*> order;
  std::unordered_set<Batch*> seen;
  std::vector<BatchP> hold;
  std::vector<BatchP> stack{root};
  while (!stack.empty()) {
    BatchP b = stack.back();
    stack.pop_back();
    if (!b->calc_grad || !seen.insert(b.get()).second) continue;
    hold.push_back(b);
    if (b->op) {
      order.push_back(b.get());
      for (auto& in : b->op->inputs) stack.push_back(in);
    }
  }
  std::sort(order.begin(), order.end(), [](Batch* a, Batch* b) { return a->op->seq > b->op->seq; });
  bool root_done = false;
  if (!root->g_dev) {
    alloc_grad(*root, false);
    auto* sop = dynamic_cast<BScalarOp*>(root->op.get());
    bool plain = sop != nullptr && !sop->inputs.empty() && sop->inputs.size() <= 2;
    if (plain)
      for (auto& in : sop->inputs) plain = plain && in->kind == Batch::SCALAR && !in->materialised && in->n == root->n;
    if (plain && sop->inputs.size() == 2 && sop->inputs[0].get() == sop->inputs[1].get()) plain = false;
    if (plain) {
      float* g[2] = {nullptr, nullptr};
      float sc[2] = {0.0f, 0.0f};
      int acc[2] = {0, 0};
      for (size_t i = 0; i < sop->inputs.size(); ++i) {
        Batch& in = *sop->inputs[i];
        if (!in.calc_grad) continue;
        sc[i] = (sop->kind == SK_NEGATE || (sop->kind == SK_SUBTRACT && i == 1)) ? -1.0f : 1.0f;
        acc[i] = in.g_dev != nullptr;
        if (!in.g_dev) alloc_grad(in, false);
        g[i] = in.g_dev;
      }
      launch_scalar_seed(root->g_dev, g[0], sc[0], acc[0], g[1], sc[1], acc[1], size_t(root->n), rt.stream());
      root_done = true;
    } else {
      launch_fill_f32(root->g_dev, 1.0f, size_t(root->n), rt.stream());
    }
  } else {
    DevMemP ones = rt.alloc(sizeof(float) * size_t(root->n ? root->n : 1));
    launch_fill_f32(ones->as<float>(), 1.0f, size_t(root->n), rt.stream());
    launch_vec_axpby(root->g_dev, ones->as<float>(), nullptr, size_t(root->n), 1.0f, 0.0f, 1, rt.stream());
  }
  std::vector<Batch*> from_graphs;
  BackwardPlan plan;
  t_plan = &plan;
  struct RetainScope {
    bool prev;
    explicit RetainScope(bool r) : prev(t_batch_retain) { t_batch_retain = r; }
    ~RetainScope() { t_batch_retain = prev; }
  } retain_scope(retain);
  try {
    for (Batch* b : order) {
      if (!b->g_dev) continue;
      if (root_done && b == root.get()) continue;
      if (auto* f = dynamic_cast<BFromGraphsOp*>(b->op.get())) {
        f->retain = retain;
        from_graphs.push_back(b);
        continue;
      }
      b->op->backward(*b);
    }
    for (auto& kv : plan.lin)
      if (!plan.fused.count(kv.first)) static_cast<BFsLinearOp*>(kv.second->op.get())->run(*kv.second);
  } catch (...) {
    t_plan = nullptr;
    throw;
  }
  t_plan = nullptr;
  for (Batch* b : seen)
    if ((b->materialised || b->leaf) && b->g_dev && !b->op) push_grads_to_graphs(*b);
  for (Batch* b : from_graphs) b->op->backward(*b);
  if (!retain)
    for (Batch* b : order) {
      if (b != root.get()) {
        b->g_dev = nullptr;
        b->g_mem.reset();
      }
      b->op.reset();
      b->tape_cleared = true;
    }
}

void batch_items_device(const BatchP& x, void* dev_out) {
  if (x->kind == Batch::SCALAR && !x->materialised) {
    if (static_cast<const void*>(x->v_dev) == dev_out) return;
    Runtime::get().d2d(dev_out, x->v_dev, sizeof(float) * size_t(x->n));
    return;
  }
  batch_materialise(*x);
  items_device(x->graphs, dev_out);
}
float batch_item_host(const BatchP& x, int i) {
  if (i < 0 || i >= x->n) throw_range("[gtnx_batch_get] element index out of range");
  if (!x->host_vals_valid) {
    x->host_vals.resize(size_t(x->n));
    if (x->host_ev) {
      Runtime::get().drain_until(x->host_ev);
      std::memcpy(x->host_vals.data(), x->host_pin->ptr, sizeof(float) * size_t(x->n));
      (void)hipEventDestroy(static_cast<hipEvent_t>(x->host_ev));
      x->host_ev = nullptr;
      x->host_pin.reset();
    } else {
      Runtime::get().d2h_sync(x->host_vals.data(), x->v_dev, sizeof(float) * size_t(x->n));
    }
    x->host_vals_valid = true;
  }
  return x->host_vals[size_t(i)];
}
void batch_prefetch_items(const BatchP& x) {
  if (!x || x->kind != Batch::SCALAR || x->materialised || x->host_vals_valid || x->host_ev || x->n <= 0 || !x->v_dev) return;
  Runtime& rt = Runtime::get();
  hipEvent_t ev;
  if (hipEventCreateWithFlags(&ev, hipEventDisableTiming) != hipSuccess) {
    (void)hipGetLastError();
    return;
  }
  x->host_pin = rt.alloc_pinned(sizeof(float) * size_t(x->n));
  rt.d2h_pinned_async(x->host_pin->ptr, x->v_dev, sizeof(float) * size_t(x->n));
  HIP_CHECK(hipEventRecord(ev, rt.stream()));
  x->host_ev = ev;
}
void batch_items_host(const BatchP& x, float* out) {
  if (x->kind == Batch::SCALAR && !x->materialised) {
    Runtime::get().d2h_sync(out, x->v_dev, sizeof(float) * size_t(x->n));
    return;
  }
  batch_materialise(*x);
  items_host(x->graphs, out);
}
void batch_grads_bind(const BatchP& x, void* dev_out, const int64_t* offsets) {
  if (x->materialised) {
    grads_bind_device(x->graphs, dev_out, offsets);
    return;
  }
  if (x->kind != Batch::LINEAR && x->kind != Batch::SCALAR) return;
  int64_t o = 0;
  for (int i = 0; i < x->n; ++i) {
    if (offsets[i] != offsets[0] + o) return;
    o += x->elem_size(i);
  }
  if (x->n == 0) return;
  x->dest_mem = std::make_shared<DevMem>();
  x->dest_mem->ptr = dev_out;
  x->dest_mem->borrowed = true;
  x->dest = static_cast<float*>(dev_out) + offsets[0];
}
void batch_grads_device(const BatchP& x, void* dev_out, const int64_t* offsets) {
  if (x->kind == Batch::CTC_TARGETS) batch_materialise(*x);
  if (x->materialised) {
    grads_device(x->graphs, dev_out, offsets);
    pad_fill(*x, static_cast<float*>(dev_out), offsets);
    return;
  }
  if (!x->g_dev) throw_logic("[gtn::Graph::grad] Gradient not calculated yet.");
  Runtime& rt = Runtime::get();
  std::vector<AxpyArgs> ax;
  int64_t maxn = 0;
  for (int i = 0; i < x->n; ++i) {
    float* dst = static_cast<float*>(dev_out) + offsets[i];
    float* src = x->g_dev + x->g_off[size_t(i)];
    if (dst == src) continue;
    const int64_t len = x->g_off[size_t(i) + 1] - x->g_off[size_t(i)];
    ax.push_back({dst, src, len, 1.0f});
    maxn = std::max(maxn, len);
  }
  if (ax.empty()) return;
  DevMemP d = upload_vec(ax);
  launch_axpy_batch(d->as<AxpyArgs>(), int(ax.size()), maxn,  2, rt.stream());
}

}
```

### gtn_amd/csrc/batch.h

```cpp
#pragma once

#include <memory>
#include <vector>

#include "ops.h"

namespace gtnx {

struct Batch;
using BatchP = std::shared_ptr<Batch>;

struct BatchOp {
  uint64_t seq = 0;
  std::vector<BatchP> inputs;
  virtual void backward(Batch& out) = 0;
  virtual ~BatchOp() {}
};

struct Batch {
  enum Kind { GRAPHS, CTC_TARGETS, LINEAR, PRODUCT, SCALAR };
  Kind kind = GRAPHS;
  int n = 0;
  bool calc_grad = false;

  bool materialised = false;
  std::vector<Graph> graphs;
  bool leaf = false;
  struct Origin {
    std::shared_ptr<void> home;
    size_t begin, end;
  };
  std::vector<Origin> origins;
  void (*give_back)(const std::shared_ptr<void>& home, std::vector<Graph>* part) = nullptr;
  std::vector<float> host_vals;
  bool host_vals_valid = false;
  PinnedMemP host_pin;
  void* host_ev = nullptr;

  std::vector<int> labels, lab_off;
  int blank = 0;
  int max_label = -1, max_nodes = 0;
  DevMemP rec_mem;
  std::vector<size_t> rec_off;
  bool fal = false;
  Graph trans;
  int trans_labels = 0;
  std::vector<size_t> w_off, map_off;
  int M = 0, C = 0;
  DevMemP w_mem;
  float* w_dev = nullptr;
  std::shared_ptr<PendingCopy> w_pend;
  DevMemP nc_mem;
  float* nc_norm = nullptr;
  float* nc_rowlse = nullptr;
  std::vector<int> rows;
  int64_t pad_floats = 0;
  DevMemP pad_mem;
  int rows_of(int b) const { return rows.empty() ? M : rows[size_t(b)]; }
  BatchP fixed, chain;
  bool chain_first = false, intersect = false;
  bool wide = false;
  bool full = false;
  DevMemP v_mem;
  float* v_dev = nullptr;

  std::shared_ptr<BatchOp> op;
  bool tape_cleared = false;
  DevMemP g_mem;
  float* g_dev = nullptr;
  std::vector<int64_t> g_off;
  DevMemP dest_mem;
  float* dest = nullptr;

  int64_t elem_size(int b) const;
  ~Batch();
};

BatchP batch_from_graphs(std::vector<Graph> gs);
BatchP batch_ctc_targets(const int* labels, const int* lengths, int n, int blank, bool calc_grad);
BatchP batch_asg_force_align(const int* labels, const int* lengths, int n, Graph& transitions, int n_labels);
BatchP batch_linear(int n, int M, int C, bool calc_grad, const void* dev, bool borrow, const int* rows = nullptr);
BatchP batch_compose(const BatchP& a, const BatchP& b, bool intersect);
BatchP batch_shortest_distance(const BatchP& x, bool tropical);
void batch_full_connect_stats(int64_t* fast, int64_t* fallback);
BatchP batch_viterbi_path(const BatchP& x);
void batch_viterbi_align(const BatchP& x, const int* frames, int* labels_dev, int64_t row_stride, int* tokens_dev,
                         float* scores_dev);
void batch_align_stats(int64_t* fast, int64_t* fallback);
void batch_viterbi_decode(const BatchP& ems, Graph& transitions, const int* frames, int* labels_dev, int64_t row_stride,
                          float* scores_dev, int* collapsed_dev, int* lengths_dev);
void batch_decode_stats(int64_t* fast, int64_t* fallback);
void batch_linear_decode(const BatchP& ems, const int* frames, int blank, int* labels_dev, int64_t row_stride,
                         float* scores_dev, int* collapsed_dev, int* starts_dev, int* lengths_dev);
void batch_linear_decode_stats(int64_t* fast, int64_t* fallback);
void batch_ctc_beam_decode(const BatchP& ems, const int* frames, int blank, int beam, int topn, int nbest,
                           int* tokens_dev, int64_t row_stride, int* lengths_dev, float* scores_dev);
void batch_ctc_beam_stats(int64_t* calls, int64_t* utterances);
void batch_edit_distance(const int* hyp_dev, int64_t hyp_stride, const int* hyp_len_dev, const int* ref_dev,
                         int64_t ref_stride, const int* ref_len_dev, int B, int N, int L, int U, int* dist_dev,
                         int* ops_dev);
void batch_edit_distance_stats(int64_t* calls, int64_t* pairs);
BatchP batch_scalar(ScalarKind k, const BatchP& a, const BatchP& b, void* items_dev = nullptr);
void batch_backward(const BatchP& root, bool retain);
void batch_items_host(const BatchP& x, float* out);
void batch_items_device(const BatchP& x, void* dev_out);
void batch_grads_device(const BatchP& x, void* dev_out, const int64_t* offsets);
void batch_grads_bind(const BatchP& x, void* dev_out, const int64_t* offsets);
Graph batch_get(const BatchP& x, int i);
float batch_item_host(const BatchP& x, int i);
void batch_prefetch_items(const BatchP& x);
BatchP batch_ctc_targets_from_graphs(const std::vector<Graph>& gs);
BatchP batch_linear_from_graphs(const std::vector<Graph>& gs);
void batch_materialise(Batch& x);

}
```

### gtn_amd/csrc/capi.cpp

```cpp
#include <atomic>
#include <chrono>
#include <condition_variable>
#include <cstdlib>
#include <cstring>
#include <mutex>
#include <string>
#include <vector>

#include "batch.h"
#include "ops.h"
#include "ops_internal.h"
#include "region.h"

#define GTNX_API extern "C" __attribute__((visibility("default")))

using namespace gtnx;

namespace {
thread_local std::string g_err;

gtnx_status_t fail(gtnx_status_t s, const std::string& m) {
  g_err = m;
  return s;
}
// ... 702 lines not shown
  return guard([&] {
    if (projection < 0 || projection > 2) throw_invalid("[gtnx_clone] projection must be 0, 1 or 2");
    std::vector<Graph> v{G(g)};
    *out = H(op_rational(RAT_CLONE, v, projection));
  });
}
GTNX_API gtnx_status_t gtnx_concat(const gtnx_graph_t* g, int n, gtnx_graph_t* out) {
  return guard([&] {
    auto v = vec(g, n);
    *out = H(op_rational(RAT_CONCAT, v, 0));
  });
}
GTNX_API gtnx_status_t gtnx_closure(gtnx_graph_t g, gtnx_graph_t* out) {
  return guard([&] {
    std::vector<Graph> v{G(g)};
    *out = H(op_rational(RAT_CLOSURE, v, 0));
  });
}
GTNX_API gtnx_status_t gtnx_union(const gtnx_graph_t* g, int n, gtnx_graph_t* out) {
  return guard([&] {
    auto v = vec(g, n);
    *out = H(op_rational(RAT_UNION, v, 0));
  });
}

GTNX_API gtnx_status_t gtnx_remove(gtnx_graph_t g, int ilabel, int olabel, gtnx_graph_t* out) {
  return guard([&] { *out = H(op_remove(G(g), ilabel, olabel)); });
}

namespace {
inline BatchP& BH(gtnx_batch_t h) {
  if (!h) throw_invalid("null batch handle");
  return *reinterpret_cast<BatchP*>(h);
}
inline gtnx_batch_t HB(BatchP b) { return reinterpret_cast<gtnx_batch_t>(new BatchP(std::move(b))); }
}
GTNX_API gtnx_status_t gtnx_batch_from_graphs(const gtnx_graph_t* g, int n, gtnx_batch_t* out) {
  return guard([&] { *out = HB(batch_from_graphs(vec(g, n, true))); });
}
GTNX_API gtnx_status_t gtnx_batch_ctc_targets(const int* labels, const int* lengths, int n, int blank, int cg,
                                              gtnx_batch_t* out) {
  return guard([&] { *out = HB(batch_ctc_targets(labels, lengths, n, blank, cg != 0)); });
}
GTNX_API gtnx_status_t gtnx_batch_asg_force_align(const int* labels, const int* lengths, int n, gtnx_graph_t transitions,
                                                  int n_labels, gtnx_batch_t* out) {
  return guard([&] { *out = HB(batch_asg_force_align(labels, lengths, n, G(transitions), n_labels)); });
}
GTNX_API gtnx_status_t gtnx_batch_linear(int n, int M, int N, int cg, const void* dev, int borrow, gtnx_batch_t* out) {
  return guard([&] { *out = HB(batch_linear(n, M, N, cg != 0, dev, borrow != 0)); });
}
GTNX_API gtnx_status_t gtnx_batch_linear_rows(int n, int M, int N, const int* rows, int cg, const void* dev, int borrow,
                                             gtnx_batch_t* out) {
  return guard([&] { *out = HB(batch_linear(n, M, N, cg != 0, dev, borrow != 0, rows)); });
}
GTNX_API gtnx_status_t gtnx_batch_destroy(gtnx_batch_t b) {
  return guard([&] {
    auto* p = reinterpret_cast<BatchP*>(b);
    if (!p) return;
    if (Runtime::initialized())
      Runtime::get().defer_delete(p, [](void* q) { delete static_cast<BatchP*>(q); },
                                  (*p && (*p)->materialised) ? size_t((*p)->n > 0 ? (*p)->n : 1) : 1);
    else
      delete p;
  });
}
GTNX_API gtnx_status_t gtnx_batch_size(gtnx_batch_t b, int* out) {
  return guard([&] { *out = BH(b)->n; });
}
GTNX_API gtnx_status_t gtnx_batch_get(gtnx_batch_t b, int i, gtnx_graph_t* out) {
  return guard([&] { *out = H(batch_get(BH(b), i)); });
}
GTNX_API gtnx_status_t gtnx_batch_negate(gtnx_batch_t a, gtnx_batch_t* out) {
  return guard([&] { *out = HB(batch_scalar(SK_NEGATE, BH(a), nullptr)); });
}
GTNX_API gtnx_status_t gtnx_batch_add(gtnx_batch_t a, gtnx_batch_t b, gtnx_batch_t* out) {
  return guard([&] { *out = HB(batch_scalar(SK_ADD, BH(a), BH(b))); });
}
GTNX_API gtnx_status_t gtnx_batch_subtract(gtnx_batch_t a, gtnx_batch_t b, gtnx_batch_t* out) {
  return guard([&] { *out = HB(batch_scalar(SK_SUBTRACT, BH(a), BH(b))); });
}
GTNX_API gtnx_status_t gtnx_batch_subtract_into(gtnx_batch_t a, gtnx_batch_t b, void* items_device, gtnx_batch_t* out) {
  return guard([&] { *out = HB(batch_scalar(SK_SUBTRACT, BH(a), BH(b), items_device)); });
}
GTNX_API gtnx_status_t gtnx_batch_compose(gtnx_batch_t a, gtnx_batch_t b, gtnx_batch_t* out) {
  return guard([&] { *out = HB(batch_compose(BH(a), BH(b), false)); });
}
GTNX_API gtnx_status_t gtnx_batch_intersect(gtnx_batch_t a, gtnx_batch_t b, gtnx_batch_t* out) {
  return guard([&] { *out = HB(batch_compose(BH(a), BH(b), true)); });
}
GTNX_API gtnx_status_t gtnx_batch_forward_score(gtnx_batch_t a, gtnx_batch_t* out) {
  return guard([&] { *out = HB(batch_shortest_distance(BH(a), false)); });
}
GTNX_API gtnx_status_t gtnx_batch_viterbi_score(gtnx_batch_t a, gtnx_batch_t* out) {
  return guard([&] { *out = HB(batch_shortest_distance(BH(a), true)); });
}
GTNX_API gtnx_status_t gtnx_batch_full_connect_stats(int64_t* fast, int64_t* fallback) {
  return guard([&] { batch_full_connect_stats(fast, fallback); });
}
GTNX_API gtnx_status_t gtnx_batch_viterbi_path(gtnx_batch_t a, gtnx_batch_t* out) {
  return guard([&] { *out = HB(batch_viterbi_path(BH(a))); });
}
GTNX_API gtnx_status_t gtnx_batch_viterbi_align(gtnx_batch_t a, const int* frames, void* labels_device, int64_t row_stride,
                                                void* tokens_device, void* scores_device) {
  return guard([&] {
    batch_viterbi_align(BH(a), frames, static_cast<int*>(labels_device), row_stride, static_cast<int*>(tokens_device),
                        static_cast<float*>(scores_device));
  });
}
GTNX_API gtnx_status_t gtnx_batch_align_stats(int64_t* fast, int64_t* fallback) {
  return guard([&] { batch_align_stats(fast, fallback); });
}
GTNX_API gtnx_status_t gtnx_batch_viterbi_decode(gtnx_batch_t ems, gtnx_graph_t transitions, const int* frames,
                                                 void* labels_device, int64_t row_stride, void* scores_device,
                                                 void* collapsed_device, void* lengths_device) {
  return guard([&] {
    batch_viterbi_decode(BH(ems), G(transitions), frames, static_cast<int*>(labels_device), row_stride,
                         static_cast<float*>(scores_device), static_cast<int*>(collapsed_device),
                         static_cast<int*>(lengths_device));
  });
}
GTNX_API gtnx_status_t gtnx_batch_decode_stats(int64_t* fast, int64_t* fallback) {
  return guard([&] { batch_decode_stats(fast, fallback); });
}
GTNX_API gtnx_status_t gtnx_batch_linear_decode(gtnx_batch_t ems, const int* frames, int blank, void* labels_device,
                                                int64_t row_stride, void* scores_device, void* collapsed_device,
                                                void* starts_device, void* lengths_device) {
  return guard([&] {
    batch_linear_decode(BH(ems), frames, blank, static_cast<int*>(labels_device), row_stride,
                        static_cast<float*>(scores_device), static_cast<int*>(collapsed_device),
                        static_cast<int*>(starts_device), static_cast<int*>(lengths_device));
  });
}
GTNX_API gtnx_status_t gtnx_batch_linear_decode_stats(int64_t* fast, int64_t* fallback) {
  return guard([&] { batch_linear_decode_stats(fast, fallback); });
}
GTNX_API gtnx_status_t gtnx_batch_ctc_beam_decode(gtnx_batch_t ems, const int* frames, int blank, int beam_size,
                                                  int cutoff_top_n, int nbest, void* tokens_device, int64_t row_stride,
                                                  void* lengths_device, void* scores_device) {
  return guard([&] {
    batch_ctc_beam_decode(BH(ems), frames, blank, beam_size, cutoff_top_n, nbest, static_cast<int*>(tokens_device),
                          row_stride, static_cast<int*>(lengths_device), static_cast<float*>(scores_device));
  });
}
GTNX_API gtnx_status_t gtnx_batch_ctc_beam_stats(int64_t* calls, int64_t* utterances) {
  return guard([&] { batch_ctc_beam_stats(calls, utterances); });
}
GTNX_API gtnx_status_t gtnx_batch_edit_distance(const void* hyp_device, int64_t hyp_stride,
                                                const void* hyp_lengths_device, const void* ref_device,
                                                int64_t ref_stride, const void* ref_lengths_device, int B, int N, int L,
                                                int U, void* dist_device, void* ops_device) {
  return guard([&] {
    batch_edit_distance(static_cast<const int*>(hyp_device), hyp_stride, static_cast<const int*>(hyp_lengths_device),
                        static_cast<const int*>(ref_device), ref_stride, static_cast<const int*>(ref_lengths_device), B,
                        N, L, U, static_cast<int*>(dist_device), static_cast<int*>(ops_device));
  });
}
GTNX_API gtnx_status_t gtnx_batch_edit_distance_stats(int64_t* calls, int64_t* pairs) {
  return guard([&] { batch_edit_distance_stats(calls, pairs); });
}
GTNX_API gtnx_status_t gtnx_batch_linear_shape(gtnx_batch_t ems, int* rows, int* labels) {
  return guard([&] {
    const BatchP& b = BH(ems);
    const bool linear = b->kind == Batch::LINEAR;
    if (rows) *rows = linear ? b->M : -1;
    if (labels) *labels = linear ? b->C : -1;
  });
// ... 102 lines not shown
```

### gtn_amd/csrc/kernels.h

```cpp
#pragma once

#include <hip/hip_runtime.h>

#include <cstdint>

#include <atomic>
#include <cstdint>
struct gtnx_first_on_device {
  std::atomic<uint64_t>& done;
  uint64_t bit;
  bool first;
  explicit gtnx_first_on_device(std::atomic<uint64_t>& d) : done(d) {
    int dev = 0;
    (void)hipGetDevice(&dev);
    bit = uint64_t(1) << (dev & 63);
    first = !(done.load(std::memory_order_acquire) & bit);
  }
  gtnx_first_on_device(const gtnx_first_on_device&) = delete;
  ~gtnx_first_on_device() {
    if (first) done.fetch_or(bit, std::memory_order_acq_rel);
  }
  explicit operator bool() const { return first; }
};

// ... 282 lines not shown
  const int* mp_colidx;
  const int* mp_colnode;
  const int* mp_dead;
  int mp_ncol, mp_ndead;
};
size_t lazy_step_lds_bytes(const LazyGroup& g);
int lazy_tile_nodes();
int lazy_tile_batch();
void launch_lazy_pack(const LazyGroup& g, gtnx_i4* lrec_in, gtnx_i4* lrec_out, hipStream_t st);
void launch_lazy_init(const LazyGroup& g, int which, hipStream_t st);
void launch_lazy_step(const LazyGroup& g, int t, int mode, int backward, hipStream_t st);
void launch_lazy_final(const LazyGroup& g, int mode, hipStream_t st);
void launch_lazy_path(const LazyGroup& g, int* path_arc, int* path_il, int* path_ol, float* path_w, int* path_len,
                      hipStream_t st);
void launch_lazy_local_z(const LazyGroup& g, float* zt, hipStream_t st);
void launch_lazy_chain_grad(const LazyGroup& g, const int* node_label, hipStream_t st);
bool lazy_z_chain_grad_ok(const LazyGroup& g);
void launch_lazy_z_chain_grad(const LazyGroup& g, const int* node_label, float* zt, hipStream_t st);
void launch_lazy_fixed_grad(const LazyGroup& g, int max_in_deg, hipStream_t st);
struct LazyPathGrad {
  const float* delta;
  int delta_stride;
  const int* path_arc;
  const int* il;
  const int* ol;
  int len, C, chain_first;
  float* grad_chain;
  float* grad_fixed;
};
void launch_lazy_path_grad(const LazyPathGrad& a, hipStream_t st);
struct LazyPair {
  DGraph g;
  const GTNX_G float* em;
  GTNX_G float* alpha;
  GTNX_G float* score;
  const GTNX_G float* delta;
  GTNX_G float* grad_em;
  GTNX_G float* grad_fixed;
  int T, C, chain_first, pad;
};
int lazy_pair_max_nodes();
int lazy_pair_max_degree();
int lazy_pair_block(int max_nodes);
int lazy_pair_max_labels(int block);
void launch_lazy_pair_forward(const LazyPair* d_pairs, int n, int block, int C, int cus, hipStream_t st);
void launch_lazy_pair_backward(const LazyPair* d_pairs, int n, int block, int C, int cus, hipStream_t st);
struct BandNode {
  int lab;
  int aid[3];
};
struct BandPair {
  const GTNX_G BandNode* nodes;
  const GTNX_G uint8_t* nflags;
  const GTNX_G int* snode;
  const GTNX_G int* slab;
  const GTNX_G float* w;
  const GTNX_G float* em;
  GTNX_G float* em_copy;
  GTNX_G float* alpha;
  GTNX_G double* aoff;
  GTNX_G float* score;
  GTNX_G float* norm;
  GTNX_G float* rowlse;
  const GTNX_G float* delta;
  const GTNX_G float* delta_norm;
  GTNX_G float* grad_em;
  GTNX_G float* grad_fixed;
  int N, T, C, NS;
  int hot;
  int lgrn;
  int n_lab;
  int bidx;
  int64_t goff;
};
struct BandPatch {
  int on;
  int M;
  const GTNX_G float* delta;
  const GTNX_G float* delta_norm;
  GTNX_G float* rowlse;
  GTNX_G float* grad_em;
  GTNX_G float* grad_fixed;
  int64_t A;
};
struct BandDecode {
  const GTNX_G BandNode* nodes;
  const GTNX_G uint8_t* nflags;
  const GTNX_G float* w;
  const GTNX_G float* em;
  GTNX_G uint8_t* bp;
  GTNX_G int* pnode;
  GTNX_G int* path_arc;
  GTNX_G int* path_lab;
  GTNX_G float* path_w;
  GTNX_G int* path_len;
  GTNX_G float* score;
  GTNX_G int* tie;
  const GTNX_G int* rank_in;
  const GTNX_G int* rank_acc;
  int N, T, C, NS;
  int stage_floats, pad;
};
void launch_band_viterbi(const BandDecode* d_pairs, int n, int stage_floats, int max_nodes, int max_labels, int vec,
                         hipStream_t st, int ranked = 0);
bool band_viterbi_wave_ok(int max_nodes, int max_labels, int vec);
struct AlignArgs {
  const GTNX_G BandNode* nodes;
  const GTNX_G uint8_t* nflags;
  const GTNX_G float* em;
  GTNX_G unsigned* bp;
  GTNX_G int* labels;
  GTNX_G int* tokens;
  GTNX_G float* score;
  int N, T, T_full, C;
  int p, pad;
};
int align_npl(int max_nodes);
bool band_align_ok(int max_nodes, int max_labels, int vec);
void launch_band_align(const AlignArgs* d_args, int n, int max_nodes, hipStream_t st);
struct AsgAlignArgs {
  const GTNX_G BandNode* nodes;
  const GTNX_G uint8_t* nflags;
  const GTNX_G float* w;
  const GTNX_G float* em;
  GTNX_G unsigned* bp;
  GTNX_G int* labels;
  GTNX_G int* tokens;
  GTNX_G float* score;
  int N, T, T_full, C;
};
int asg_align_npl(int max_nodes);
int asg_align_max_labels();
bool asg_align_ok(int max_nodes, int max_labels, int vec);
size_t asg_align_plane_bytes(int T, int npl);
void launch_asg_align(const AsgAlignArgs* d_args, int n, int max_nodes, hipStream_t st);
struct RationalSeg {
  DGraph g;
  int node_off, arc_off;
  int conn_off;
  int keep_start, keep_accept;
  int pad;
};
struct RationalOut {
  int N, A;
  GTNX_G int* src;
  GTNX_G int* dst;
  GTNX_G int* il;
  GTNX_G int* ol;
  GTNX_G float* w;
  GTNX_G uint8_t* nflags;
  GTNX_G int* start_list;
  GTNX_G int* accept_list;
  GTNX_G int* out_off;
  GTNX_G int* out_list;
  GTNX_G int* in_off;
  GTNX_G int* in_list;
};
size_t rational_csr_temp_bytes(int N, int A);
void launch_rational_build(const RationalSeg* d_segs, int nseg, int max_A, int max_N, int max_conn, const RationalOut& out,
                           int projection, int closure, void* temp, hipStream_t st);
void launch_rational_adjacency(const RationalOut& out, void* temp, hipStream_t st);
struct RemoveArgs {
  DGraph g;
  int ilabel, olabel;
  const GTNX_G int* new_id;
  const GTNX_G int* roots;
  int K, root0, rows;
  GTNX_G int* stamp;
  GTNX_G int* queue;
  GTNX_G int* arc_cnt;
  const GTNX_G int* arc_off;
  RationalOut out;
};
void launch_remove_keep(const DGraph& g, int ilabel, int olabel, int* keep, hipStream_t st);
void launch_remove_roots(const int* keep, const int* new_id, int N, int* roots, hipStream_t st);
void launch_remove_walk(const RemoveArgs& a, bool emit, hipStream_t st);
size_t scan_temp_bytes(int n);
void launch_exclusive_scan(const int* in, int* out, int n, void* temp, size_t temp_bytes, hipStream_t st);
void launch_rational_load(const void* rows, const float* w, const uint8_t* flags, const RationalOut& out, void* temp,
                          hipStream_t st);
struct CtcTargetArgs {
  const GTNX_G int* labels;
  GTNX_G BandNode* nodes;
  GTNX_G uint8_t* nflags;
  GTNX_G int* snode;
  GTNX_G int* slab;
  GTNX_G int* n_arcs;
  int N, pad;
};
void launch_ctc_targets(const CtcTargetArgs* d_args, int n, int blank, hipStream_t st);
struct AsgFalArgs {
  const GTNX_G int* labels;
  const GTNX_G float* trans_w;
  GTNX_G BandNode* nodes;
  GTNX_G uint8_t* nflags;
  GTNX_G int* snode;
  GTNX_G int* slab;
  GTNX_G float* w;
  GTNX_G int* arc_map;
  int U, pad;
};
void launch_asg_fal_targets(const AsgFalArgs* d_args, int n, int n_labels, hipStream_t st);
void launch_asg_fal_scatter(const float* g, const int* maps, const int64_t* tab , int n_seq, int64_t longest,
                            float* trans_grad, hipStream_t st);
int band_max_nodes();
int band_max_labels();
int band_min_labels();
int band_npl(int max_nodes);
int band_row_stride(int N, int npl);
int band_forward_lgrn(int C);
bool band_one_ok(int npl, int C, int max_NS, bool vec, bool backward);
void launch_band_forward(const BandPair* d_pairs, int n, int npl, int C, int max_NS, bool unit, bool vec, hipStream_t st,
                         const BandPair* one = nullptr);
void launch_band_backward(const BandPair* d_pairs, int n, int npl, int C, int max_NS, bool unit, bool gradg, bool vec,
                          hipStream_t st, const BandPair* one = nullptr, const BandPatch* patch = nullptr);
void launch_lazy_dense_prep(const LazyGroup& g, float* E, float* cmax, hipStream_t st);
void launch_lazy_dense_step(const LazyGroup& g, int t, int backward, hipStream_t st, const float* vin = nullptr,
                            float* vout = nullptr);
void launch_lazy_dense_fixed_grad(const LazyGroup& g, hipStream_t st);
size_t maxplus_w_floats(const LazyGroup& g);
void launch_maxplus_prep(const LazyGroup& g, hipStream_t st);
void launch_maxplus_step(const LazyGroup& g, int t, hipStream_t st);
void launch_maxplus_path(const LazyGroup& g, int* path_arc, int* path_il, int* path_ol, float* path_w, int* path_len,
                         hipStream_t st);
void launch_asg_decode(const LazyGroup& g, const int* d_frames, int* labels, int64_t row_stride, float* scores,
                       int* collapsed, int* lengths, hipStream_t st);
void launch_lazy_mfma_prep(const LazyGroup& g, hipStream_t st);
void launch_lazy_mfma_init(const LazyGroup& g, int which, hipStream_t st);
void launch_lazy_mfma_step(const LazyGroup& g, int t, int backward, hipStream_t st);
size_t lazy_mfma_chain_sync_ints(const LazyGroup& g);
bool launch_lazy_mfma_chain(const LazyGroup& g, int backward, int* zeroed_sync, int cus, hipStream_t st);
void launch_lazy_mfma_keys(float* keys, int64_t n, hipStream_t st);
void launch_lazy_mfma_rowmax(const LazyGroup& g, int which, hipStream_t st);
void launch_lazy_mfma_score(const LazyGroup& g, hipStream_t st);
size_t lazy_mfma_fixed_grad_scratch_bytes(const LazyGroup& g);
void launch_lazy_mfma_fixed_grad(const LazyGroup& g, void* pair_consts , hipStream_t st, void* partials = nullptr,
                                 size_t partials_bytes = 0);

void launch_fill_i32(int* p, int v, size_t n, hipStream_t st);
void launch_fill_f32(float* p, float v, size_t n, hipStream_t st);
void launch_scalar_seed(float* root, float* g0, float s0, int acc0, float* g1, float s1, int acc1, size_t n, hipStream_t st);
struct ScalarArgs {
  const GTNX_G float* a;
  const GTNX_G float* b;
  GTNX_G float* out;
  GTNX_G float* mirror;
};
void launch_scalar_combine(const ScalarArgs* d_args, int n, float sa, float sb, hipStream_t st);
void launch_copy_small(void* dst, const void* src, size_t bytes, hipStream_t st);
void launch_scalar_combine_one(const ScalarArgs& a, float sa, float sb, hipStream_t st);
struct ScalarFanArgs {
  const GTNX_G float* d;
  GTNX_G float* seed;
  GTNX_G float* o0;
  GTNX_G float* o1;
};
void launch_scalar_fan(const ScalarFanArgs* d_args, int n, float s0, float s1, hipStream_t st);
void launch_scalar_fan_one(const ScalarFanArgs& a, float s0, float s1, hipStream_t st);
struct AxpyArgs {
  GTNX_G float* dst;
  const GTNX_G float* src;
  int64_t n;
  float scale;
};
void launch_axpy_batch(const AxpyArgs* d_args, int n, int64_t maxn, int atomic, hipStream_t st);
struct CopySeg {
  void* dst;
  const void* src;
  int64_t bytes;
};
void launch_copy_segments(const CopySeg* d_segs, int n, int64_t max_bytes, hipStream_t st);
void launch_gather_scalars(const float* const* d_ptrs, float* out, int n, hipStream_t st);
void launch_vec_axpby(float* out, const float* a, const float* b, size_t n, float sa, float sb, int accumulate, hipStream_t st);
// ... 79 lines not shown
```

### gtn_amd/csrc/ops.h

```cpp
#pragma once

#include <cstring>
#include <tuple>
#include <vector>

#include "graph.h"

namespace gtnx {

struct Member {
  int idx;
  Graph out;
};

struct OpRecord {
  uint64_t seq = 0;
  virtual void backward(std::vector<Member>& members) = 0;
  virtual bool joins_chain_plan() const { return false; }
  virtual ~OpRecord() {}
};

struct GradSink {
  struct Item {
    Graph g;
    DevMemP owner;
    float* ptr;
  };
  std::vector<Item> items;
  void add(const Graph& g, const DevMemP& owner, float* ptr) {
    if (g.calc_grad()) items.push_back({g, owner, ptr});
  }
  void flush();
};

struct BandLaunchKey {
  int C, npl, unit, gradg, vec;
  bool operator<(const BandLaunchKey& o) const {
    return std::tie(C, npl, unit, gradg, vec) < std::tie(o.C, o.npl, o.unit, o.gradg, o.vec);
  }
  bool operator==(const BandLaunchKey& o) const { return !(*this < o) && !(o < *this); }
};
int band_vec_ok(const BandPair& p);
void band_launch(std::vector<std::pair<BandLaunchKey, BandPair>>& tab, bool backward, const char* prof_name = nullptr,
                 double prof_bytes = 0.0, DevMemP* table_out = nullptr);
void band_launch_patched(const DevMemP& table, int n, const BandLaunchKey& key, int max_ns, const BandPatch& patch,
                         const char* prof_name, double prof_bytes);

enum ScalarKind { SK_NEGATE = 0, SK_ADD = 1, SK_SUBTRACT = 2 };

std::vector<Graph> op_scalar(ScalarKind k, std::vector<Graph>& a, std::vector<Graph>& b);
std::vector<Graph> op_shortest_distance(std::vector<Graph>& gs, bool tropical);
std::vector<Graph> op_viterbi_path(std::vector<Graph>& gs);
std::vector<Graph> op_compose(std::vector<Graph>& a, std::vector<Graph>& b, bool intersect);
bool lazy_decode_ok(Graph& fixed, int M, int C);
void lazy_viterbi_decode(std::vector<Graph>& chains, Graph& fixed, const std::vector<int>& frames, int* labels_dev,
                         int64_t row_stride, float* scores_dev, int* collapsed_dev, int* lengths_dev);
enum RationalKind { RAT_CLONE = 0, RAT_CONCAT = 1, RAT_CLOSURE = 2, RAT_UNION = 3 };
Graph op_rational(int kind, std::vector<Graph>& inputs, int projection);
Graph op_remove(Graph& g, int ilabel, int olabel);
Graph op_load_buffer(const void* data, size_t bytes);
void op_backward(std::vector<Graph>& roots, Graph* grad, bool retain, bool seed = true);
void backward_validate(Graph& root);
int compose_mode_hint(int mode);
void realize(Graph& g);

Graph make_scalar_graph(float v, bool calc_grad);
Graph make_linear_graph(int M, int N, bool calc_grad);
std::vector<Graph> make_linear_graphs_device(int B, int M, int N, bool calc_grad, const void* dev, bool borrow = false);
Graph make_user_op(std::vector<Graph>& inputs, gtnx_grad_fn fn, void* ctx, void (*ctx_free)(void*));
void set_user_grad_fn(Graph& g, gtnx_grad_fn fn, void* ctx, void (*ctx_free)(void*));

void items_host(std::vector<Graph>& gs, float* out);
void items_device(std::vector<Graph>& gs, void* dev_out);
void grads_device(std::vector<Graph>& gs, void* dev_out, const int64_t* offsets);
void grads_bind_device(std::vector<Graph>& gs, void* dev_out, const int64_t* offsets);

inline bool upload_in_place(size_t bytes) {
  static const size_t lim = [] {
    const char* e = std::getenv("GTNX_ARGS_IN_PLACE");
    return e ? size_t(std::atol(e)) : size_t(0);
  }();
  return bytes <= lim;
}
template <class T>
DevMemP upload_vec(const std::vector<T>& v) {
  Runtime& rt = Runtime::get();
  size_t bytes = sizeof(T) * v.size();
  if (bytes && upload_in_place(bytes)) {
    PinnedMemP p = rt.alloc_pinned(bytes);
    std::memcpy(p->ptr, v.data(), bytes);
    DevMemP d = std::make_shared<DevMem>();
    d->ptr = p->ptr;
    d->bytes = bytes;
    d->borrowed = true;
    d->keep = p;
    return d;
  }
  DevMemP d = rt.alloc(bytes ? bytes : 1);
  if (bytes) {
    PinnedMemP p = rt.alloc_pinned(bytes);
    std::memcpy(p->ptr, v.data(), bytes);
    rt.h2d_pinned(d->ptr, p->ptr, bytes);
  }
  return d;
}

}
```

### gtn_amd/csrc/ops_band.cpp

```cpp
#include "ops_internal.h"

#include <memory>

namespace gtnx {

int band_vec_ok(const BandPair& p) { return p.C % 4 == 0 && (reinterpret_cast<uintptr_t>(p.em) & 15) == 0; }
void band_launch_patched(const DevMemP& table, int n, const BandLaunchKey& k, int max_ns, const BandPatch& patch,
                         const char* prof_name, double prof_bytes) {
  Runtime& rt = Runtime::get();
  std::unique_ptr<Runtime::Scope> prof(prof_name ? new Runtime::Scope(&rt, prof_name, prof_bytes) : nullptr);
  launch_band_backward(table->as<BandPair>(), n, k.npl, k.C, max_ns, k.unit != 0, k.gradg != 0, k.vec != 0, rt.stream(), nullptr,
                       &patch);
}
void band_launch(std::vector<std::pair<BandLaunchKey, BandPair>>& tab, bool backward, const char* prof_name, double prof_bytes,
                 DevMemP* table_out) {
  Runtime& rt = Runtime::get();
  if (table_out) table_out->reset();
  if (tab.empty()) return;
  bool one_key = true;
  for (size_t i = 1; i < tab.size() && one_key; ++i) one_key = tab[i].first == tab[0].first;
  if (!one_key) std::stable_sort(tab.begin(), tab.end(), [](const auto& x, const auto& y) { return x.first < y.first; });
  if (tab.size() == 1) {
    const BandLaunchKey& k = tab[0].first;
    const BandPair& p = tab[0].second;
    if (band_one_ok(k.npl, k.C, p.NS, k.vec != 0, backward)) {
      std::unique_ptr<Runtime::Scope> prof(prof_name ? new Runtime::Scope(&rt, prof_name, prof_bytes) : nullptr);
      if (backward) launch_band_backward(nullptr, 1, k.npl, k.C, p.NS, k.unit != 0, k.gradg != 0, true, rt.stream(), &p);
      else launch_band_forward(nullptr, 1, k.npl, k.C, p.NS, k.unit != 0, true, rt.stream(), &p);
      return;
    }
  }
  std::vector<BandPair> flat;
  flat.reserve(tab.size());
  for (auto& e : tab) flat.push_back(e.second);
  DevMemP d = upload_vec(flat);
  const BandPair* dp = d->as<BandPair>();
  if (table_out && one_key) *table_out = d;
  std::unique_ptr<Runtime::Scope> prof(prof_name ? new Runtime::Scope(&rt, prof_name, prof_bytes) : nullptr);
  for (size_t i0 = 0; i0 < tab.size();) {
    size_t i1 = i0;
    int max_ns = 0;
    while (i1 < tab.size() && tab[i1].first == tab[i0].first) max_ns = std::max(max_ns, tab[i1++].second.NS);
    const BandLaunchKey& k = tab[i0].first;
    if (backward)
      launch_band_backward(dp + i0, int(i1 - i0), k.npl, k.C, max_ns, k.unit != 0, k.gradg != 0, k.vec != 0, rt.stream());
    else
      launch_band_forward(dp + i0, int(i1 - i0), k.npl, k.C, max_ns, k.unit != 0, k.vec != 0, rt.stream());
    i0 = i1;
  }
}
bool band_shape_ok(const Structure& cs, Structure& fs, bool chain_first) {
  if (cs.kind != KIND_LINEAR || cs.C < band_min_labels() || cs.C > band_max_labels() || cs.M < 0 || cs.M > (1 << 20)) return false;
  std::shared_ptr<BandInfo> b = band_info(fs, chain_first);
  return b->ok && b->max_label < cs.C;
}
bool band_ok(const LazyProduct& lp, std::shared_ptr<BandInfo>* out) {
  if (!band_shape_ok(*lp.chain.s, *lp.fixed.s, lp.chain_side == 1)) return false;
  if (out) *out = band_info(*lp.fixed.s, lp.chain_side == 1);
  return true;
}
static bool tie_ranks(Structure& fs, BandInfo& bi, bool use_ilabel);
void band_prepare(const std::vector<Graph*>& fixed, const std::vector<uint8_t>& chain_first, bool want_ranks) {
  std::vector<size_t> todo;
  std::unordered_set<Structure*> seen;
  for (size_t i = 0; i < fixed.size(); ++i) {
    Structure* st = fixed[i]->s.get();
    const std::shared_ptr<BandInfo>& b = st->band[chain_first[i] ? 0 : 1];
    if ((!b || (want_ranks && b->ok && b->rank_state == 0)) && seen.insert(st).second) todo.push_back(i);
  }
  auto body = [&](size_t q) {
    Graph& g = *fixed[todo[q]];
    std::shared_ptr<BandInfo> b = band_info(*g.s, chain_first[todo[q]] != 0);
    (void)g.w->is_all_zero();
    if (want_ranks && b && b->ok) (void)tie_ranks(*g.s, *b, chain_first[todo[q]] != 0);
  };
  if (todo.size() >= 64) gtn::detail::runIndexed(todo.size(), body, 32, false);
  else for (size_t q = 0; q < todo.size(); ++q) body(q);
}

struct BandSdOp : OpRecord {
  std::vector<BandPair> pairs;
  std::vector<Graph> chains, fixed;
  std::vector<std::shared_ptr<BandInfo>> infos;
  std::vector<uint8_t> unit;
  DevMemP arena;

  using Key = BandLaunchKey;
  static int band_vec(const BandPair& p) { return band_vec_ok(p); }
  static void launch(std::vector<std::pair<Key, BandPair>>& tab, bool backward, const char* prof_name = nullptr, double prof_bytes = 0.0) {
    band_launch(tab, backward, prof_name, prof_bytes);
  }

  void backward(std::vector<Member>& ms) override {
    Runtime& rt = Runtime::get();
    size_t eb = 0, fb = 0;
    std::vector<size_t> eo(ms.size(), 0), fo(ms.size(), 0);
    std::vector<float*> dest(ms.size(), nullptr);
    std::vector<DevMemP> dest_mem(ms.size());
    for (size_t k = 0; k < ms.size(); ++k) {
      const int i = ms[k].idx;
      if (chains[i].calc_grad()) {
        GradState& cg = *chains[i].g;
        if (cg.grad_dest && !chains[i].is_grad_available()) {
          dest[k] = cg.grad_dest;
          dest_mem[k] = cg.grad_dest_mem;
          cg.grad_dest = nullptr;
        } else {
          eo[k] = eb;
          eb = align_up(eb + 4 * size_t(pairs[i].T) * size_t(pairs[i].C), 256);
        }
      }
      if (fixed[i].calc_grad()) {
        fo[k] = fb;
        fb = align_up(fb + 4 * size_t(fixed[i].s->A), 256);
      }
    }
    DevMemP gem = rt.alloc(eb ? eb : 1);
    DevMemP gfx = rt.alloc_zero(fb ? fb : 1);
// ... 609 lines not shown
```

### gtn_amd/csrc/runtime.cpp

```cpp
#include "runtime.h"

#include "kernels.h"

#include <malloc.h>

#include <atomic>
#include <condition_variable>
#include <cstring>
#include <deque>
#include <thread>

namespace gtnx {

namespace {
constexpr int kMaxDevices = 64;
std::atomic<Runtime*> g_rts[kMaxDevices];
std::atomic<bool> g_any_rt{false};
std::mutex g_rt_mu;
std::atomic<int> g_default_device{-1};
thread_local int t_device = -1;

int hip_device_now() {
  int d = -1;
  if (hipGetDevice(&d) != hipSuccess) {
// ... 502 lines not shown
  }
  (void)hipEventRecord(ev, stream_);
  pending_pinned_.push_back({ev, std::move(unstamped_pinned_)});
  unstamped_pinned_.clear();
}

void Runtime::empty_cache() {
  OnDevice here(device_);
  drain_all_inboxes();
  (void)hipStreamSynchronize(stream_);
  std::lock_guard<std::mutex> lk(mu_);
  for (auto& kv : free_dev_) {
    (void)hipFree(kv.second);
    reserved_ -= kv.first;
  }
  free_dev_.clear();
  for (auto& b : unstamped_pinned_) free_pinned_.emplace(b.second, b.first);
  unstamped_pinned_.clear();
  for (auto& g : pending_pinned_) {
    for (auto& b : g.blocks) free_pinned_.emplace(b.second, b.first);
    ev_pool_.push_back(g.ev);
  }
  pending_pinned_.clear();
  for (auto& kv : free_pinned_) (void)hipHostFree(kv.second);
  free_pinned_.clear();
}

void Runtime::stats(uint64_t* reserved, uint64_t* in_use) {
  drain_deferred();
  std::lock_guard<std::mutex> lk(mu_);
  if (reserved) *reserved = reserved_;
  if (in_use) *in_use = in_use_;
}

void Runtime::h2d(void* dst, const void* src, size_t bytes) {
  if (bytes) HIP_CHECK(hipMemcpyAsync(dst, src, bytes, hipMemcpyHostToDevice, stream_));
}
void Runtime::d2h_sync(void* dst, const void* src, size_t bytes) {
  if (bytes && bytes <= 4096) {
    PinnedMemP p = alloc_pinned(bytes);
    d2h_pinned_async(p->ptr, src, bytes);
    drain_while_busy();
    HIP_CHECK(hipStreamSynchronize(stream_));
    std::memcpy(dst, p->ptr, bytes);
    return;
  }
  if (bytes) HIP_CHECK(hipMemcpyAsync(dst, src, bytes, hipMemcpyDeviceToHost, stream_));
  drain_while_busy();
  HIP_CHECK(hipStreamSynchronize(stream_));
}
void Runtime::sync_while_draining() {
  drain_while_busy();
  HIP_CHECK(hipStreamSynchronize(stream_));
}
namespace {
bool local_to(const void* p, int dev) {
  static const int ndev = Runtime::device_count();
  if (ndev <= 1) return true;
  hipPointerAttribute_t a;
  if (hipPointerGetAttributes(&a, p) != hipSuccess) {
    (void)hipGetLastError();
    return false;
  }
  return a.type == hipMemoryTypeHost || (a.type == hipMemoryTypeDevice && a.device == dev);
}
}
bool ptr_local_to(const void* p, int dev) { return local_to(p, dev); }
void Runtime::d2d(void* dst, const void* src, size_t bytes) {
  if (!bytes) return;
  if (bytes <= (size_t(1) << 20) && local_to(src, device_) && local_to(dst, device_)) {
    launch_copy_small(dst, src, bytes, stream_);
    return;
  }
  HIP_CHECK(hipMemcpyAsync(dst, src, bytes, hipMemcpyDeviceToDevice, stream_));
}
void Runtime::d2h_pinned_async(void* pinned_dst, const void* src, size_t bytes) {
  if (!bytes) return;
  if (bytes <= (size_t(1) << 20) && local_to(src, device_)) {
    launch_copy_small(pinned_dst, src, bytes, stream_);
    return;
  }
  HIP_CHECK(hipMemcpyAsync(pinned_dst, src, bytes, hipMemcpyDeviceToHost, stream_));
}
void Runtime::h2d_pinned(void* dst, const void* pinned_src, size_t bytes) {
  if (!bytes) return;
  static const size_t lim = [] {
    const char* e = std::getenv("GTNX_H2D_KERNEL_BYTES");
    return e ? size_t(std::atol(e)) : size_t(1) << 20;
  }();
  if (bytes <= lim && local_to(dst, device_)) {
    launch_copy_small(dst, pinned_src, bytes, stream_);
    return;
  }
  HIP_CHECK(hipMemcpyAsync(dst, pinned_src, bytes, hipMemcpyHostToDevice, stream_));
}

Runtime::MirrorSlot Runtime::mirror_slot() {
  {
    std::lock_guard<std::mutex> lk(mu_);
    if (!mirror_ring_) {
      OnDevice here(device_);
      void* p = nullptr;
      HIP_CHECK(hipHostMalloc(&p, sizeof(float) * kMirrorSlots, hipHostMallocDefault));
      mirror_gen_ = new std::atomic<uint64_t>[kMirrorSlots];
      for (size_t i = 0; i < kMirrorSlots; ++i) mirror_gen_[i].store(0);
      mirror_ring_ = static_cast<float*>(p);
    }
  }
  const uint64_t g = mirror_next_.fetch_add(1) + 1;
  const size_t i = size_t(g % kMirrorSlots);
  mirror_gen_[i].store(g);
  return {mirror_ring_ + i, g};
}
bool Runtime::mirror_read(const MirrorSlot& m, float* out) {
  if (!m.ptr || !mirror_ring_) return false;
  const size_t i = size_t(m.ptr - mirror_ring_);
  if (i >= kMirrorSlots || mirror_gen_[i].load() != m.gen) return false;
  sync();
  const float v = *static_cast<volatile float*>(m.ptr);
  if (mirror_gen_[i].load() != m.gen) return false;
  *out = v;
  return true;
}

void Runtime::prof_enable(bool on) {
  if (!on) collect_prof();
  prof_on_ = on;
}
void Runtime::prof_reset() {
  collect_prof();
  prof_.clear();
}

Runtime::Scope::Scope(Runtime* r, const char* name, double bytes) : rt(r), idx(-1) {
  if (!rt->prof_on_) return;
  ProfRec rec;
  rec.name = name;
  rec.bytes = bytes;
  auto get_ev = [&]() {
    hipEvent_t e;
    HIP_CHECK(hipEventCreate(&e));
    return e;
  };
  rec.a = get_ev();
  rec.b = get_ev();
  HIP_CHECK(hipEventRecord(rec.a, rt->stream_));
  idx = (int)rt->prof_recs_.size();
  rt->prof_recs_.push_back(rec);
}
Runtime::Scope::~Scope() {
  if (idx >= 0) (void)hipEventRecord(rt->prof_recs_[idx].b, rt->stream_);
}

void Runtime::prof_add_bytes(const std::string& name, double bytes) { prof_[name].bytes += bytes; }

void Runtime::collect_prof() {
  if (prof_recs_.empty()) return;
  (void)hipStreamSynchronize(stream_);
  for (auto& r : prof_recs_) {
    float ms = 0;
    if (hipEventElapsedTime(&ms, r.a, r.b) == hipSuccess) {
      auto& e = prof_[r.name];
      e.total_ms += ms;
      e.launches += 1;
      e.bytes += r.bytes;
    } else {
      (void)hipGetLastError();
    }
    (void)hipEventDestroy(r.a);
    (void)hipEventDestroy(r.b);
  }
  prof_recs_.clear();
// ... 66 lines not shown
```

### gtn_amd/csrc/runtime.h

```cpp
#pragma once

#include <atomic>
#include <functional>
#include <map>
#include <memory>
#include <mutex>
#include <string>
#include <vector>

#include "common.h"

namespace gtnx {

class Runtime;

struct DevMem {
  void* ptr = nullptr;
  size_t bytes = 0;
  bool borrowed = false;
  Runtime* owner = nullptr;
  std::shared_ptr<void> keep;
  ~DevMem();
  template <class T>
  T* as(size_t byte_off = 0) const { return reinterpret_cast<T*>(static_cast<char*>(ptr) + byte_off); }
};
using DevMemP = std::shared_ptr<DevMem>;

struct PinnedMem {
  void* ptr = nullptr;
  size_t bytes = 0;
  Runtime* owner = nullptr;
  ~PinnedMem();
  template <class T>
  T* as(size_t byte_off = 0) const { return reinterpret_cast<T*>(static_cast<char*>(ptr) + byte_off); }
};
using PinnedMemP = std::shared_ptr<PinnedMem>;

struct ProfEntry {
  double total_ms = 0;
  int64_t launches = 0;
  double bytes = 0;
};

class Runtime {
 public:
  static Runtime& get();
  static Runtime& of(int device);
  static int device_count();
  static bool initialized();
  static void set_current_device(int d);
  static int current_device();
  int device() const { return device_; }
  void activate();

  hipStream_t stream() const { return stream_; }
  void set_stream(hipStream_t s);
  void sync();

  DevMemP alloc(size_t bytes);
  DevMemP alloc_zero(size_t bytes);
  PinnedMemP alloc_pinned(size_t bytes);
  void release_dev(void* p, size_t bytes);
  void release_pinned(void* p, size_t bytes);
  void empty_cache();
  void stats(uint64_t* reserved, uint64_t* in_use);

  struct Inbox {
    std::mutex mu;
    std::vector<std::pair<void*, void (*)(void*)>> items;
    size_t load = 0;
    bool dead = false;
  };
  using InboxP = std::shared_ptr<Inbox>;
  static InboxP home();
  static void send(const InboxP& to, void* p, void (*del)(void*));
  static void drain_all_inboxes();
  static void defer_delete(void* p, void (*del)(void*), size_t weight = 1);
  static void drain_deferred();
  static bool drain_some(size_t max_items);
  static size_t deferred_count();
  void drain_until(void* hip_event);
  void drain_while_busy();
  void sync_while_draining();

  struct SideJob;
  using SideJobP = std::shared_ptr<SideJob>;
  SideJobP side_launch(std::function<void(hipStream_t)> fn);
  void side_join(const SideJobP& job);

  void h2d(void* dst, const void* src, size_t bytes);
  void d2h_sync(void* dst, const void* src, size_t bytes);
  void d2d(void* dst, const void* src, size_t bytes);
  void h2d_pinned(void* dst, const void* pinned_src, size_t bytes);
  void d2h_pinned_async(void* pinned_dst, const void* src, size_t bytes);

  struct MirrorSlot {
    float* ptr = nullptr;
    uint64_t gen = 0;
  };
  static constexpr size_t kMirrorSlots = 1024;
  MirrorSlot mirror_slot();
  bool mirror_read(const MirrorSlot& m, float* out);

  void prof_enable(bool on);
  void prof_add_bytes(const std::string& name, double bytes);
  void prof_reset();
  bool prof_on() const { return prof_on_; }
  struct Scope {
    Runtime* rt;
    int idx;
    Scope(Runtime* r, const char* name, double bytes);
    ~Scope();
  };
  ProfEntry prof_get(const std::string& name);
  std::string prof_names();
  int cu_count() const { return cu_count_; }

 private:
  explicit Runtime(int device);
  void collect_prof();
  float* mirror_ring_ = nullptr;
  std::atomic<uint64_t>* mirror_gen_ = nullptr;
  std::atomic<uint64_t> mirror_next_{0};
  hipStream_t own_stream_ = nullptr;
  hipStream_t stream_ = nullptr;
  int device_ = 0;
  int cu_count_ = 256;
  std::mutex mu_;
  std::multimap<size_t, void*> free_dev_;
  std::multimap<size_t, void*> free_pinned_;
  struct PinnedGroup {
    hipEvent_t ev;
    std::vector<std::pair<void*, size_t>> blocks;
  };
  static constexpr size_t kPinnedStampEvery = 8;
  std::vector<PinnedGroup> pending_pinned_;
  std::vector<std::pair<void*, size_t>> unstamped_pinned_;
  void stamp_pinned_locked();
  uint64_t reserved_ = 0, in_use_ = 0;
  bool prof_on_ = false;
  struct ProfRec {
    std::string name;
    double bytes;
    hipEvent_t a, b;
  };
  std::vector<ProfRec> prof_recs_;
  std::vector<hipEvent_t> ev_pool_;
  struct Side;
  std::atomic<Side*> side_{nullptr};
  std::map<std::string, ProfEntry> prof_;
  friend struct Scope;
};

bool ptr_local_to(const void* p, int dev);

#define GTNX_PROF(name, bytes) ::gtnx::Runtime::Scope _prof_scope(&::gtnx::Runtime::get(), name, bytes)

struct HostTimer {
  const char* name;
  double t0;
  explicit HostTimer(const char* n);
  ~HostTimer();
  static bool enabled();
};
double host_now_ms();
void host_timer_add(const char* name, double ms);
#define GTNX_HT_CAT2(a, b) a##b
#define GTNX_HT_CAT(a, b) GTNX_HT_CAT2(a, b)
#define GTNX_HOST_T(name) ::gtnx::HostTimer GTNX_HT_CAT(_host_t_, __LINE__)(name)

}
```

### include/gtn/batch.h

```cpp
#pragma once
#include <cstdint>
#include <utility>
#include <vector>

#include "gtn/functions.h"

namespace gtn {

class Batch {
 public:
  Batch() = default;
  explicit Batch(const std::vector<Graph>& graphs) {
    auto h = detail::handles(graphs);
    detail::check(gtnx_batch_from_graphs(h.data(), static_cast<int>(h.size()), &h_));
  }
  Batch(const Batch&) = delete;
  Batch& operator=(const Batch&) = delete;
  Batch(Batch&& o) noexcept : h_(o.h_) { o.h_ = nullptr; }
  Batch& operator=(Batch&& o) noexcept {
    if (this != &o) {
      reset();
      h_ = o.h_;
      o.h_ = nullptr;
    }
// ... 12 lines not shown
      len.push_back(static_cast<int>(t.size()));
    }
    return ctcTargets(flat.data(), len.data(), static_cast<int>(targets.size()), blank, calcGrad);
  }
  static Batch ctcTargets(const int* labels, const int* lengths, int n, int blank = 0, bool calcGrad = true) {
    Batch b;
    detail::check(gtnx_batch_ctc_targets(labels, lengths, n, blank, calcGrad, &b.h_));
    return b;
  }
  static Batch asgForceAlign(const int* labels, const int* lengths, int n, const Graph& transitions, int numLabels) {
    Batch b;
    detail::check(gtnx_batch_asg_force_align(labels, lengths, n, transitions.handle(), numLabels, &b.h_));
    return b;
  }
  static Batch linear(int n, int M, int N, const void* deviceWeights, bool calcGrad = true, bool borrow = false,
                      const int* rows = nullptr) {
    Batch b;
    if (rows)
      detail::check(gtnx_batch_linear_rows(n, M, N, rows, calcGrad, deviceWeights, borrow, &b.h_));
    else
      detail::check(gtnx_batch_linear(n, M, N, calcGrad, deviceWeights, borrow, &b.h_));
    return b;
  }

  int size() const {
    int n = 0;
    if (h_) detail::check(gtnx_batch_size(h_, &n));
    return n;
  }
  Graph operator[](int i) const {
    gtnx_graph_t g;
    detail::check(gtnx_batch_get(h_, i, &g));
    return Graph::fromHandle(g);
  }
  std::vector<float> items() const {
    std::vector<float> v(static_cast<size_t>(size()));
    if (!v.empty()) detail::check(gtnx_batch_items(h_, v.data()));
    return v;
  }
  void itemsToDevice(void* deviceOut) const { detail::check(gtnx_batch_items_device(h_, deviceOut)); }
  void bindGrads(void* deviceOut, const int64_t* offsets) { detail::check(gtnx_batch_grads_bind_device(h_, deviceOut, offsets)); }
  void gradsToDevice(void* deviceOut, const int64_t* offsets) const {
    detail::check(gtnx_batch_grads_device(h_, deviceOut, offsets));
  }
  gtnx_batch_t handle() const { return h_; }
  static Batch fromHandle(gtnx_batch_t h) {
    Batch b;
    b.h_ = h;
    return b;
  }

 private:
  void reset() {
    if (h_) gtnx_batch_destroy(h_);
    h_ = nullptr;
  }
  gtnx_batch_t h_ = nullptr;
};

namespace detail {
template <class F>
Batch batchUnary(F f, const Batch& a) {
  gtnx_batch_t out;
  check(f(a.handle(), &out));
  return Batch::fromHandle(out);
}
template <class F>
Batch batchBinary(F f, const Batch& a, const Batch& b) {
  gtnx_batch_t out;
  check(f(a.handle(), b.handle(), &out));
  return Batch::fromHandle(out);
}
}

namespace batched {
inline Batch negate(const Batch& a) { return detail::batchUnary(&gtnx_batch_negate, a); }
inline Batch add(const Batch& a, const Batch& b) { return detail::batchBinary(&gtnx_batch_add, a, b); }
inline Batch subtract(const Batch& a, const Batch& b) { return detail::batchBinary(&gtnx_batch_subtract, a, b); }
inline Batch subtract(const Batch& a, const Batch& b, void* itemsDevice) {
  gtnx_batch_t out;
  detail::check(gtnx_batch_subtract_into(a.handle(), b.handle(), itemsDevice, &out));
  return Batch::fromHandle(out);
}
inline Batch compose(const Batch& a, const Batch& b) { return detail::batchBinary(&gtnx_batch_compose, a, b); }
inline Batch intersect(const Batch& a, const Batch& b) { return detail::batchBinary(&gtnx_batch_intersect, a, b); }
inline Batch forwardScore(const Batch& a) { return detail::batchUnary(&gtnx_batch_forward_score, a); }
inline Batch viterbiScore(const Batch& a) { return detail::batchUnary(&gtnx_batch_viterbi_score, a); }
inline Batch viterbiPath(const Batch& a) { return detail::batchUnary(&gtnx_batch_viterbi_path, a); }
inline void viterbiAlign(const Batch& product, int* labelsDevice, int64_t rowStride, int* tokensDevice = nullptr,
                         float* scoresDevice = nullptr, const int* frames = nullptr) {
  detail::check(gtnx_batch_viterbi_align(product.handle(), frames, labelsDevice, rowStride, tokensDevice, scoresDevice));
}
inline void viterbiDecode(const Batch& ems, const Graph& transitions, int* labelsDevice, int64_t rowStride,
                          float* scoresDevice = nullptr, const int* frames = nullptr, int* collapsedDevice = nullptr,
                          int* lengthsDevice = nullptr) {
  detail::check(gtnx_batch_viterbi_decode(ems.handle(), transitions.handle(), frames, labelsDevice, rowStride,
                                          scoresDevice, collapsedDevice, lengthsDevice));
}
inline void linearDecode(const Batch& ems, int* labelsDevice, int64_t rowStride, float* scoresDevice = nullptr,
                         const int* frames = nullptr, int blank = -1, int* collapsedDevice = nullptr,
                         int* startsDevice = nullptr, int* lengthsDevice = nullptr) {
  detail::check(gtnx_batch_linear_decode(ems.handle(), frames, blank, labelsDevice, rowStride, scoresDevice,
                                         collapsedDevice, startsDevice, lengthsDevice));
}
inline void ctcBeamDecode(const Batch& ems, int* tokensDevice, int64_t rowStride, int* lengthsDevice, float* scoresDevice,
                          int blank = 0, int beamSize = 16, int cutoffTopN = 16, int nbest = 1,
                          const int* frames = nullptr) {
  detail::check(gtnx_batch_ctc_beam_decode(ems.handle(), frames, blank, beamSize, cutoffTopN, nbest, tokensDevice,
                                           rowStride, lengthsDevice, scoresDevice));
}
inline void editDistance(const int* hypDevice, int64_t hypStride, const int* hypLengthsDevice, const int* refDevice,
                         int64_t refStride, const int* refLengthsDevice, int B, int N, int L, int U, int* distDevice,
                         int* opsDevice = nullptr) {
  detail::check(gtnx_batch_edit_distance(hypDevice, hypStride, hypLengthsDevice, refDevice, refStride, refLengthsDevice,
                                         B, N, L, U, distDevice, opsDevice));
}
inline void backward(const Batch& a, bool retainGraph = false) { detail::check(gtnx_batch_backward(a.handle(), retainGraph)); }
}

}
```

### include/gtn_amd.h

```cpp
#ifndef GTN_AMD_H
#define GTN_AMD_H

#include <stddef.h>
#include <stdint.h>

#ifdef __cplusplus
extern "C" {
#endif

typedef int gtnx_status_t;
#define GTNX_OK 0
#define GTNX_INVALID_ARGUMENT 1
#define GTNX_LOGIC_ERROR 2
#define GTNX_RUNTIME_ERROR 3
#define GTNX_OUT_OF_RANGE 4
#define GTNX_DEVICE_ERROR 5

typedef struct gtnx_graph_s* gtnx_graph_t;

#define GTNX_EPSILON (-1)

const char* gtnx_last_error(void);
const char* gtnx_version(void);
const char* gtnx_backend(void);
// ... 40 lines not shown
gtnx_status_t gtnx_graph_get_start(gtnx_graph_t g, int* out);
gtnx_status_t gtnx_graph_get_accept(gtnx_graph_t g, int* out);
gtnx_status_t gtnx_graph_is_start(gtnx_graph_t g, int node, int* out);
gtnx_status_t gtnx_graph_is_accept(gtnx_graph_t g, int node, int* out);
gtnx_status_t gtnx_graph_make_accept(gtnx_graph_t g, int node);
gtnx_status_t gtnx_graph_num_out(gtnx_graph_t g, int node, int64_t* out);
gtnx_status_t gtnx_graph_num_in(gtnx_graph_t g, int node, int64_t* out);
gtnx_status_t gtnx_graph_get_out(gtnx_graph_t g, int node, int* out);
gtnx_status_t gtnx_graph_get_in(gtnx_graph_t g, int node, int* out);
gtnx_status_t gtnx_graph_get_arcs(gtnx_graph_t g, int* src, int* dst, int* ilabel, int* olabel);
gtnx_status_t gtnx_graph_get_arc(gtnx_graph_t g, int arc, int* src, int* dst,
                                 int* ilabel, int* olabel, float* weight);
gtnx_status_t gtnx_graph_set_weight(gtnx_graph_t g, int arc, float weight);
gtnx_status_t gtnx_graph_calc_grad(gtnx_graph_t g, int* out);
gtnx_status_t gtnx_graph_set_calc_grad(gtnx_graph_t g, int calc_grad);
gtnx_status_t gtnx_graph_is_grad_available(gtnx_graph_t g, int* out);
gtnx_status_t gtnx_graph_grad(gtnx_graph_t g, gtnx_graph_t* out);
gtnx_status_t gtnx_graph_zero_grad(gtnx_graph_t g);
gtnx_status_t gtnx_graph_add_grad(gtnx_graph_t g, const float* host_grad, int64_t n);
gtnx_status_t gtnx_graph_add_grad_graph(gtnx_graph_t g, gtnx_graph_t other);
gtnx_status_t gtnx_graph_id(gtnx_graph_t g, uintptr_t* out);
typedef gtnx_status_t (*gtnx_grad_fn)(void* ctx, gtnx_graph_t* inputs, int n_inputs, gtnx_graph_t deltas);
gtnx_status_t gtnx_graph_create_op(gtnx_graph_t* inputs, int n_inputs, gtnx_grad_fn grad_fn,
                                   void* ctx, void (*ctx_free)(void*), gtnx_graph_t* out);
gtnx_status_t gtnx_graph_num_inputs(gtnx_graph_t g, int64_t* out);
gtnx_status_t gtnx_graph_get_input(gtnx_graph_t g, int i, gtnx_graph_t* out);
gtnx_status_t gtnx_graph_set_inputs(gtnx_graph_t g, const gtnx_graph_t* inputs, int n);
gtnx_status_t gtnx_graph_set_grad_fn(gtnx_graph_t g, gtnx_grad_fn grad_fn, void* ctx,
                                     void (*ctx_free)(void*));
gtnx_status_t gtnx_graph_has_grad_fn(gtnx_graph_t g, int* out);

gtnx_status_t gtnx_scalar_graph(float value, int calc_grad, gtnx_graph_t* out);
gtnx_status_t gtnx_linear_graph(int M, int N, int calc_grad, gtnx_graph_t* out);
gtnx_status_t gtnx_linear_graph_n(int B, int M, int N, int calc_grad,
                                  const void* device_weights, gtnx_graph_t* out );
gtnx_status_t gtnx_linear_graph_borrow_n(int B, int M, int N, int calc_grad,
                                         const void* device_weights, gtnx_graph_t* out );

gtnx_status_t gtnx_negate(gtnx_graph_t g, gtnx_graph_t* out);
gtnx_status_t gtnx_add(gtnx_graph_t a, gtnx_graph_t b, gtnx_graph_t* out);
gtnx_status_t gtnx_subtract(gtnx_graph_t a, gtnx_graph_t b, gtnx_graph_t* out);
gtnx_status_t gtnx_compose(gtnx_graph_t a, gtnx_graph_t b, gtnx_graph_t* out);
gtnx_status_t gtnx_intersect(gtnx_graph_t a, gtnx_graph_t b, gtnx_graph_t* out);
gtnx_status_t gtnx_forward_score(gtnx_graph_t g, gtnx_graph_t* out);
gtnx_status_t gtnx_viterbi_score(gtnx_graph_t g, gtnx_graph_t* out);
gtnx_status_t gtnx_viterbi_path(gtnx_graph_t g, gtnx_graph_t* out);

gtnx_status_t gtnx_negate_n(const gtnx_graph_t* g, int n, gtnx_graph_t* out);
gtnx_status_t gtnx_add_n(const gtnx_graph_t* a, int na, const gtnx_graph_t* b, int nb, gtnx_graph_t* out);
gtnx_status_t gtnx_subtract_n(const gtnx_graph_t* a, int na, const gtnx_graph_t* b, int nb, gtnx_graph_t* out);
gtnx_status_t gtnx_compose_n(const gtnx_graph_t* a, int na, const gtnx_graph_t* b, int nb, gtnx_graph_t* out);
gtnx_status_t gtnx_intersect_n(const gtnx_graph_t* a, int na, const gtnx_graph_t* b, int nb, gtnx_graph_t* out);
gtnx_status_t gtnx_forward_score_n(const gtnx_graph_t* g, int n, gtnx_graph_t* out);
gtnx_status_t gtnx_viterbi_score_n(const gtnx_graph_t* g, int n, gtnx_graph_t* out);
gtnx_status_t gtnx_viterbi_path_n(const gtnx_graph_t* g, int n, gtnx_graph_t* out);
gtnx_status_t gtnx_items_n(const gtnx_graph_t* g, int n, float* out);
gtnx_status_t gtnx_items_device_n(const gtnx_graph_t* g, int n, void* device_out);
gtnx_status_t gtnx_grads_device_n(const gtnx_graph_t* g, int n, void* device_out, const int64_t* offsets);
gtnx_status_t gtnx_grads_bind_device_n(const gtnx_graph_t* g, int n, void* device_out, const int64_t* offsets);

gtnx_status_t gtnx_clone(gtnx_graph_t g, int projection , gtnx_graph_t* out);
gtnx_status_t gtnx_concat(const gtnx_graph_t* g, int n, gtnx_graph_t* out);
gtnx_status_t gtnx_closure(gtnx_graph_t g, gtnx_graph_t* out);
gtnx_status_t gtnx_union(const gtnx_graph_t* g, int n, gtnx_graph_t* out);
gtnx_status_t gtnx_remove(gtnx_graph_t g, int ilabel, int olabel, gtnx_graph_t* out);

typedef struct gtnx_batch_s* gtnx_batch_t;
gtnx_status_t gtnx_batch_from_graphs(const gtnx_graph_t* g, int n, gtnx_batch_t* out);
gtnx_status_t gtnx_batch_ctc_targets(const int* labels, const int* lengths, int n, int blank, int calc_grad,
                                     gtnx_batch_t* out);
gtnx_status_t gtnx_batch_asg_force_align(const int* labels, const int* lengths, int n, gtnx_graph_t transitions,
                                         int n_labels, gtnx_batch_t* out);
gtnx_status_t gtnx_batch_linear(int n, int M, int N, int calc_grad, const void* device_weights, int borrow,
                                gtnx_batch_t* out);
gtnx_status_t gtnx_batch_linear_rows(int n, int M, int N, const int* rows, int calc_grad, const void* device_weights,
                                     int borrow, gtnx_batch_t* out);
gtnx_status_t gtnx_batch_destroy(gtnx_batch_t b);
gtnx_status_t gtnx_batch_size(gtnx_batch_t b, int* out);
gtnx_status_t gtnx_batch_get(gtnx_batch_t b, int i, gtnx_graph_t* out);
gtnx_status_t gtnx_batch_negate(gtnx_batch_t a, gtnx_batch_t* out);
gtnx_status_t gtnx_batch_add(gtnx_batch_t a, gtnx_batch_t b, gtnx_batch_t* out);
gtnx_status_t gtnx_batch_subtract(gtnx_batch_t a, gtnx_batch_t b, gtnx_batch_t* out);
gtnx_status_t gtnx_batch_subtract_into(gtnx_batch_t a, gtnx_batch_t b, void* items_device, gtnx_batch_t* out);
gtnx_status_t gtnx_batch_compose(gtnx_batch_t a, gtnx_batch_t b, gtnx_batch_t* out);
gtnx_status_t gtnx_batch_intersect(gtnx_batch_t a, gtnx_batch_t b, gtnx_batch_t* out);
gtnx_status_t gtnx_batch_forward_score(gtnx_batch_t a, gtnx_batch_t* out);
gtnx_status_t gtnx_batch_viterbi_score(gtnx_batch_t a, gtnx_batch_t* out);
gtnx_status_t gtnx_batch_viterbi_path(gtnx_batch_t a, gtnx_batch_t* out);
gtnx_status_t gtnx_batch_viterbi_align(gtnx_batch_t a, const int* frames, void* labels_device, int64_t row_stride,
                                       void* tokens_device, void* scores_device);
gtnx_status_t gtnx_batch_align_stats(int64_t* fast, int64_t* fallback);
gtnx_status_t gtnx_batch_viterbi_decode(gtnx_batch_t ems, gtnx_graph_t transitions, const int* frames,
                                        void* labels_device, int64_t row_stride, void* scores_device,
                                        void* collapsed_device, void* lengths_device);
gtnx_status_t gtnx_batch_decode_stats(int64_t* fast, int64_t* fallback);
gtnx_status_t gtnx_batch_full_connect_stats(int64_t* fast, int64_t* fallback);
gtnx_status_t gtnx_batch_linear_decode(gtnx_batch_t ems, const int* frames, int blank, void* labels_device,
                                       int64_t row_stride, void* scores_device, void* collapsed_device,
                                       void* starts_device, void* lengths_device);
gtnx_status_t gtnx_batch_linear_decode_stats(int64_t* fast, int64_t* fallback);
gtnx_status_t gtnx_batch_ctc_beam_decode(gtnx_batch_t ems, const int* frames, int blank, int beam_size,
                                         int cutoff_top_n, int nbest, void* tokens_device, int64_t row_stride,
                                         void* lengths_device, void* scores_device);
gtnx_status_t gtnx_batch_ctc_beam_stats(int64_t* calls, int64_t* utterances);
gtnx_status_t gtnx_batch_edit_distance(const void* hyp_device, int64_t hyp_stride, const void* hyp_lengths_device,
                                       const void* ref_device, int64_t ref_stride, const void* ref_lengths_device,
                                       int B, int N, int L, int U, void* dist_device, void* ops_device);
gtnx_status_t gtnx_batch_edit_distance_stats(int64_t* calls, int64_t* pairs);
gtnx_status_t gtnx_batch_linear_shape(gtnx_batch_t ems, int* rows, int* labels);
gtnx_status_t gtnx_batch_backward(gtnx_batch_t a, int retain_graph);
gtnx_status_t gtnx_batch_items(gtnx_batch_t a, float* out);
gtnx_status_t gtnx_batch_items_device(gtnx_batch_t a, void* device_out);
gtnx_status_t gtnx_batch_grads_bind_device(gtnx_batch_t a, void* device_out, const int64_t* offsets);
gtnx_status_t gtnx_batch_grads_device(gtnx_batch_t a, void* device_out, const int64_t* offsets);

gtnx_status_t gtnx_backward(gtnx_graph_t g, int retain_graph);
gtnx_status_t gtnx_backward_with_grad(gtnx_graph_t g, gtnx_graph_t grad, int retain_graph);
gtnx_status_t gtnx_backward_n(const gtnx_graph_t* g, int n, int retain_graph);

gtnx_status_t gtnx_equal(gtnx_graph_t a, gtnx_graph_t b, int* out);
gtnx_status_t gtnx_isomorphic(gtnx_graph_t a, gtnx_graph_t b, int* out);

gtnx_status_t gtnx_graph_load_buffer(const void* data, size_t bytes, gtnx_graph_t* out);

typedef struct gtnx_comm_s* gtnx_comm_t;
gtnx_status_t gtnx_comm_create(const int* devices, int n, gtnx_comm_t* out);
gtnx_status_t gtnx_comm_destroy(gtnx_comm_t c);
gtnx_status_t gtnx_comm_size(gtnx_comm_t c, int* n);
gtnx_status_t gtnx_comm_all_gather_f32(gtnx_comm_t c, const void* const* send, void* const* recv, int64_t count);
gtnx_status_t gtnx_comm_all_reduce_sum_f32(gtnx_comm_t c, void* const* bufs, int64_t count);

gtnx_status_t gtnx_prof_enable(int on);
gtnx_status_t gtnx_prof_reset(void);
gtnx_status_t gtnx_prof_get(const char* name, double* total_ms, int64_t* launches,
                            double* algorithmic_bytes);
gtnx_status_t gtnx_debug_viterbi_ties(int64_t* seen, int64_t* unresolved);
gtnx_status_t gtnx_debug_tie_ranks(gtnx_graph_t g, int* queue_rank, int* creation_rank, int* applies);
gtnx_status_t gtnx_prof_names(char* buf, size_t cap);
gtnx_status_t gtnx_debug_symbolic_route(gtnx_graph_t g, int tropical, int* route);
gtnx_status_t gtnx_debug_route_name(int route, char* buf, size_t cap);

#ifdef __cplusplus
}
#endif
#endif
```

Measured before the change: 975,800 losses/s.

## Fuse CTC target build with band table upload and loss into backward sweep

Defers the CTC target-graph build kernel so it runs in one launch together with the upload of the band forward-score pair table (the table is written into pinned memory and copied by extra blocks of the same kernel). Adds a fused subtract-and-backward path that writes the per-utterance loss inside the patched backward band sweep, seeds gradients from cached constant buffers and lazily fills the ones-gradient. This cuts several small kernel launches, host-to-device copies and tape traversal work per step. In exchange it adds mutex-guarded lazy state on target batches and a number of fallback conditions that must all hold for the fast path.

New measurement: 972,500 losses/s. Within noise of the previous version (-0.3%).

```diff
diff --git a/gtn_amd/_capi.py b/gtn_amd/_capi.py
--- a/gtn_amd/_capi.py
+++ b/gtn_amd/_capi.py
@@ -111,6 +111,8 @@
     "gtnx_batch_add": [c_graph, c_graph, c_graph_p],
     "gtnx_batch_subtract": [c_graph, c_graph, c_graph_p],
     "gtnx_batch_subtract_into": [c_graph, c_graph, C.c_void_p, c_graph_p],
+    "gtnx_batch_subtract_backward": [c_graph, c_graph, C.c_void_p, c_graph_p],
+    "gtnx_batch_set_step_fused": [C.c_int, c_i32_p],
     "gtnx_batch_compose": [c_graph, c_graph, c_graph_p],
     "gtnx_batch_intersect": [c_graph, c_graph, c_graph_p],
     "gtnx_batch_forward_score": [c_graph, c_graph_p],
diff --git a/gtn_amd/api.py b/gtn_amd/api.py
--- a/gtn_amd/api.py
+++ b/gtn_amd/api.py
@@ -804,6 +804,23 @@
 
     if hasattr(lib, "gtnx_batch_subtract_into"):
         ns.subtract_into = subtract_into
+
+    def subtract_backward(a, b, items_device=None):
+        h = C.c_void_p()
+        dev = None if items_device is None else _as_dev_ptr(items_device)
+        check(lib.gtnx_batch_subtract_backward(a._h, b._h, dev, C.byref(h)))
+        r = Batch._from_handle(h.value)
+        r._keep = items_device
+        return r
+
+    def set_ctc_step_fused(on):
+        prev = C.c_int(0)
+        check(lib.gtnx_batch_set_step_fused(int(bool(on)), C.byref(prev)))
+        return bool(prev.value)
+
+    if hasattr(lib, "gtnx_batch_subtract_backward"):
+        ns.subtract_backward = subtract_backward
+        ns.set_ctc_step_fused = set_ctc_step_fused
 
     _plain_backward = ns.backward
 
diff --git a/gtn_amd/criteria/ctc_criterion.h b/gtn_amd/criteria/ctc_criterion.h
--- a/gtn_amd/criteria/ctc_criterion.h
+++ b/gtn_amd/criteria/ctc_criterion.h
@@ -68,9 +68,8 @@
   auto t3 = now();
   Batch score = batched::forwardScore(comp);
   Batch norm = batched::forwardScore(ems);
-  Batch losses = batched::subtract(norm, score, lossDev);
   auto t4 = now();
-  if (gradDev) batched::backward(losses);
+  Batch losses = gradDev ? batched::subtractBackward(norm, score, lossDev) : batched::subtract(norm, score, lossDev);
   auto t5 = now();
   if (times) *times = {ms(t0, t1), ms(t1, t2), ms(t2, t3), ms(t3, t4), ms(t4, t5)};
   losses.itemsToDevice(lossDev);
diff --git a/gtn_amd/csrc/band.hip b/gtn_amd/csrc/band.hip
--- a/gtn_amd/csrc/band.hip
+++ b/gtn_amd/csrc/band.hip
@@ -348,6 +348,7 @@
 __device__ __forceinline__ BandPair band_patched(BandPair P, const BandPatch& pt) {
   if (pt.on) {
     const int b = P.bidx;
+    if (pt.loss && threadIdx.x == 0) pt.loss[b] = *P.norm - *P.score;
     P.delta = pt.delta + b;
     P.delta_norm = pt.delta_norm ? pt.delta_norm + b : nullptr;
     P.rowlse = pt.rowlse ? pt.rowlse + int64_t(b) * pt.M : nullptr;
@@ -372,15 +373,14 @@
 }
 
 
-__global__ __launch_bounds__(512) void ctc_targets_kernel(const CtcTargetArgs* __restrict__ args, int blank) {
-  const CtcTargetArgs a = args[blockIdx.x];
+__device__ __forceinline__ void ctc_targets_body(const CtcTargetArgs& a, const GTNX_G int* __restrict__ labels, int blank) {
   __shared__ __attribute__((aligned(16))) int tl[256 + 4];
   __shared__ __attribute__((aligned(16))) int tk[256 + 4];
   const int N = a.N, U = (N - 1) >> 1, m = threadIdx.x;
   if (m < 260) {
-    const int v = m < U ? a.labels[m] : 0x7fffffff;
+    const int v = m < U ? labels[m] : 0x7fffffff;
     tl[m] = v;
-    tk[m] = (m > 0 && m < U && v != a.labels[m - 1]) ? 1 : 0;
+    tk[m] = (m > 0 && m < U && v != labels[m - 1]) ? 1 : 0;
   }
   __syncthreads();
   if (m >= N) return;
@@ -411,6 +411,23 @@
   a.snode[rank] = m;
   a.slab[rank] = my;
   if (m == N - 1 && a.n_arcs) a.n_arcs[0] = base + 1 + (m > 0 ? 1 : 0) + skip;
+}
+__global__ __launch_bounds__(512) void ctc_targets_kernel(const CtcTargetArgs* __restrict__ args, int blank) {
+  const CtcTargetArgs a = args[blockIdx.x];
+  ctc_targets_body(a, a.labels, blank);
+}
+__global__ __launch_bounds__(512) void ctc_head_kernel(const CtcTargetArgs* __restrict__ args, int n, int blank, int64_t lab_shift,
+                                                       const gtnx_i4* __restrict__ tab_src, gtnx_i4* __restrict__ tab_dst,
+                                                       unsigned tab_vecs) {
+  if (int(blockIdx.x) >= n) {
+    const unsigned i = (blockIdx.x - unsigned(n)) * 512u + threadIdx.x;
+    if (i < tab_vecs) tab_dst[i] = tab_src[i];
+    return;
+  }
+  const CtcTargetArgs a = args[blockIdx.x];
+  const GTNX_G int* labels =
+      reinterpret_cast<const GTNX_G int*>(reinterpret_cast<const GTNX_G char*>(a.labels) + lab_shift);
+  ctc_targets_body(a, labels, blank);
 }
 
 __global__ __launch_bounds__(512) void band_viterbi_kernel(const BandDecode* __restrict__ pairs) {
@@ -996,5 +1013,13 @@
 void launch_ctc_targets(const CtcTargetArgs* d_args, int n, int blank, hipStream_t st) {
   if (n > 0) hipLaunchKernelGGL(ctc_targets_kernel, dim3(n), dim3(512), 0, st, d_args, blank);
 }
-
-}
+void launch_ctc_head(const CtcTargetArgs* args, int n, int blank, int64_t lab_shift, const void* tab_src, void* tab_dst,
+                     size_t tab_bytes, hipStream_t st) {
+  if (n <= 0) return;
+  if (tab_bytes % 16 != 0 || tab_bytes / 16 > 0x7fffffffu) throw std::logic_error("band.hip: the head copies whole 16-byte words");
+  const unsigned vecs = unsigned(tab_bytes / 16);
+  hipLaunchKernelGGL(ctc_head_kernel, dim3(unsigned(n) + (vecs + 511u) / 512u), dim3(512), 0, st, args, n, blank, lab_shift,
+                     static_cast<const gtnx_i4*>(tab_src), static_cast<gtnx_i4*>(tab_dst), vecs);
+}
+
+}
diff --git a/gtn_amd/csrc/batch.cpp b/gtn_amd/csrc/batch.cpp
--- a/gtn_amd/csrc/batch.cpp
+++ b/gtn_amd/csrc/batch.cpp
@@ -38,6 +38,34 @@
 }
 
 bool native(const Batch& b, Batch::Kind k) { return b.kind == k; }
+
+std::atomic<bool> g_step_fused{true};
+bool band_patch_enabled() {
+  static const bool no_patch = std::getenv("GTNX_NO_BAND_PATCH") != nullptr;
+  return !no_patch;
+}
+const float* seed_constants(Runtime& rt, size_t n, const float** plus) {
+  struct Slot {
+    DevMemP mem;
+    size_t cap = 0;
+  };
+  static std::mutex mu;
+  static auto* slots = new std::unordered_map<int, Slot>();
+  std::lock_guard<std::mutex> lk(mu);
+  Slot& sl = (*slots)[rt.device()];
+  if (sl.cap < n) {
+    size_t cap = 1024;
+    while (cap < n) cap *= 2;
+    rt.sync();
+    sl.mem = rt.alloc(2 * sizeof(float) * cap);
+    sl.cap = cap;
+    launch_fill_f32(sl.mem->as<float>(), -1.0f, cap, rt.stream());
+    launch_fill_f32(sl.mem->as<float>() + cap, 1.0f, cap, rt.stream());
+    rt.sync();
+  }
+  *plus = sl.mem->as<float>() + sl.cap;
+  return sl.mem->as<float>();
+}
 
 void pad_fill(Batch& b, float* base, const int64_t* offs = nullptr) {
   if (b.kind != Batch::LINEAR || b.pad_floats <= 0) return;
@@ -174,6 +202,7 @@
   DevMemP arena;
   DevMemP fwd_table;
   DevMemP through_acc;
+  bool head = false;
   void backward(Batch& out) override {
     Batch& prod = *inputs[0];
     Batch& fx = *prod.fixed;
@@ -197,6 +226,14 @@
         t_plan->fused.insert(&ch);
       }
     }
+    sweep(delta, lin_out ? lin_out->g_dev : nullptr, ge.ptr, gf.ptr, nullptr);
+    if (ch.calc_grad) add_scratch(ch, ge);
+    if (fx.calc_grad) add_scratch(fx, gf);
+  }
+  bool sweep(const float* delta, const float* delta_norm, float* grad_em, float* grad_fixed, float* loss) {
+    Batch& prod = *inputs[0];
+    Batch& fx = *prod.fixed;
+    Batch& ch = *prod.chain;
     std::vector<std::pair<BandLaunchKey, BandPair>> tab;
     tab.reserve(pairs.size());
     double bytes = 0;
@@ -206,36 +243,36 @@
     for (int b = 0; b < prod.n; ++b) {
       BandPair p = pairs[size_t(b)];
       p.delta = delta + b;
-      p.delta_norm = lin_out ? lin_out->g_dev + b : nullptr;
-      p.rowlse = lin_out ? ch.nc_rowlse + size_t(b) * size_t(ch.M) : nullptr;
+      p.delta_norm = delta_norm ? delta_norm + b : nullptr;
+      p.rowlse = delta_norm ? ch.nc_rowlse + size_t(b) * size_t(ch.M) : nullptr;
       p.norm = nullptr;
-      p.grad_em = ge.ptr ? ge.ptr + size_t(b) * A : nullptr;
-      p.grad_fixed = gf.ptr ? gf.ptr + fx.g_off[size_t(b)] : nullptr;
+      p.grad_em = grad_em ? grad_em + size_t(b) * A : nullptr;
+      p.grad_fixed = grad_fixed ? grad_fixed + fx.g_off[size_t(b)] : nullptr;
       tab.push_back({BandLaunchKey{p.C, band_npl(p.N), fx.fal ? 0 : 1, p.grad_fixed ? 1 : 0, band_vec_ok(p)}, p});
       one_key = one_key && tab.back().first == tab.front().first;
       max_ns = std::max(max_ns, p.NS);
       bytes += 4.0 * p.T * p.C * (p.grad_em ? 2 : 1) + 4.0 * double(p.T + 1) * p.NS +
                (p.grad_fixed ? 4.0 * double(fx.elem_size(b)) : 0.0);
     }
-    static const bool no_patch = std::getenv("GTNX_NO_BAND_PATCH") != nullptr;
-    if (fwd_table && one_key && prod.n > 1 && !no_patch) {
+    if (fwd_table && one_key && prod.n > 1 && band_patch_enabled()) {
       BandPatch pt{};
       pt.on = 1;
       pt.M = ch.M;
       pt.delta = delta;
-      pt.delta_norm = lin_out ? lin_out->g_dev : nullptr;
-      pt.rowlse = lin_out ? ch.nc_rowlse : nullptr;
-      pt.grad_em = ge.ptr;
-      pt.grad_fixed = gf.ptr;
+      pt.delta_norm = delta_norm;
+      pt.rowlse = delta_norm ? ch.nc_rowlse : nullptr;
+      pt.grad_em = grad_em;
+      pt.grad_fixed = grad_fixed;
       pt.A = int64_t(A);
+      pt.loss = loss;
       band_launch_patched(fwd_table, prod.n, tab.front().first, max_ns, pt, "band_forward_score_grad", bytes);
-    } else {
-      band_launch(tab, true, "band_forward_score_grad", bytes);
-    }
-    if (ch.calc_grad) add_scratch(ch, ge);
-    if (fx.calc_grad) add_scratch(fx, gf);
-    (void)rt;
-  }
+      return true;
+    }
+    if (loss) throw_logic("BFsBandOp::sweep: the losses are stored by the patched launch only");
+    band_launch(tab, true, "band_forward_score_grad", bytes);
+    return false;
+  }
+  bool patched() const { return fwd_table && inputs[0]->n > 1 && band_patch_enabled(); }
 };
 
 
@@ -437,7 +474,10 @@
   Runtime& rt = Runtime::get();
   const size_t lab_bytes = align_up(sizeof(int) * (total ? total : 1), 256);
   const size_t arg_bytes = align_up(sizeof(CtcTargetArgs) * size_t(n), 256);
-  size_t bytes = lab_bytes + arg_bytes;
+  const size_t tab_bytes = align_up(sizeof(BandPair) * size_t(n), 256);
+  const bool lazy = g_step_fused.load(std::memory_order_relaxed) && band_patch_enabled() && n > 1 &&
+                    lab_bytes + arg_bytes + tab_bytes <= Runtime::h2d_kernel_limit();
+  size_t bytes = lab_bytes + arg_bytes + (lazy ? tab_bytes : 0);
   b->rec_off.resize(size_t(n));
   for (int i = 0; i < n; ++i) {
     const size_t N = size_t(2 * lengths[i] + 1);
@@ -445,7 +485,7 @@
     bytes += align_up(sizeof(BandNode) * N, 64) + align_up(N, 64) + 2 * align_up(4 * N, 64) + 64;
   }
   b->rec_mem = rt.alloc(bytes);
-  PinnedMemP pin = rt.alloc_pinned(lab_bytes + arg_bytes);
+  PinnedMemP pin = rt.alloc_pinned(lab_bytes + arg_bytes + (lazy ? tab_bytes : 0));
   std::memcpy(pin->ptr, labels, sizeof(int) * total);
   CtcTargetArgs* args = reinterpret_cast<CtcTargetArgs*>(static_cast<char*>(pin->ptr) + lab_bytes);
   for (int i = 0; i < n; ++i) {
@@ -465,10 +505,30 @@
     a.N = int(N);
     a.pad = 0;
   }
+  if (lazy) {
+    b->rec_pin = pin;
+    b->rec_lab_bytes = lab_bytes;
+    b->rec_head_bytes = lab_bytes + arg_bytes;
+    b->rec_tab_bytes = tab_bytes;
+    b->rec_pending = true;
+    return b;
+  }
   rt.h2d_pinned(b->rec_mem->ptr, pin->ptr, lab_bytes + arg_bytes);
   launch_ctc_targets(reinterpret_cast<const CtcTargetArgs*>(b->rec_mem->as<char>(lab_bytes)), n, blank, rt.stream());
   return b;
 }
+
+void batch_targets_settle(Batch& x) {
+  if (x.kind != Batch::CTC_TARGETS || !x.rec_mem) return;
+  std::lock_guard<std::mutex> lk(x.rec_mu);
+  if (!x.rec_pending) return;
+  Runtime& rt = Runtime::get();
+  rt.h2d_pinned(x.rec_mem->ptr, x.rec_pin->ptr, x.rec_head_bytes);
+  launch_ctc_targets(reinterpret_cast<const CtcTargetArgs*>(x.rec_mem->as<char>(x.rec_lab_bytes)), x.n, x.blank, rt.stream());
+  x.rec_pending = false;
+  x.rec_pin.reset();
+}
+bool batch_step_fused_set(bool on) { return g_step_fused.exchange(on); }
 
 
 BatchP batch_asg_force_align(const int* labels, const int* lengths, int n, Graph& transitions, int n_labels) {
@@ -602,6 +662,7 @@
   }
   BatchP b = batch_ctc_targets(flat.data(), len.data(), n, s0.ctc_blank, cg);
   if (b->kind != Batch::CTC_TARGETS) return nullptr;
+  batch_targets_settle(*b);
   b->graphs = gs;
   b->leaf = true;
   for (auto& g : gs) g.s->leaf_batch = b;
@@ -992,6 +1053,12 @@
         pend->settle();
       }
     }
+    std::unique_lock<std::mutex> rec_lock(fx.rec_mu);
+    bool head = fx.rec_pending && !fx.fal && !fuse_copy && n > 1 && g_step_fused.load(std::memory_order_relaxed);
+    if (!head) {
+      rec_lock.unlock();
+      batch_targets_settle(fx);
+    }
     int64_t goff_run = 0;
     for (int b = 0; b < n; ++b) {
       BandPair& p = op->pairs[size_t(b)];
@@ -1033,7 +1100,31 @@
       tab.push_back({BandLaunchKey{C, band_npl(q.N), fx.fal ? 0 : 1, 0, band_vec_ok(q)}, q});
       abytes += 4.0 * p.T * C + 4.0 * double(p.T + 1) * p.NS + (fuse_copy ? 4.0 * T * C : 0.0);
     }
-    band_launch(tab, false, "band_forward_score", abytes, fuse_copy ? nullptr : &op->fwd_table);
+    for (size_t i = 1; i < tab.size() && head; ++i) head = tab[i].first == tab[0].first;
+    if (head) {
+      BandPair* slot = fx.rec_pin->as<BandPair>(fx.rec_head_bytes);
+      for (int b = 0; b < n; ++b) slot[b] = tab[size_t(b)].second;
+      std::memset(static_cast<void*>(slot + n), 0, fx.rec_tab_bytes - sizeof(BandPair) * size_t(n));
+      launch_ctc_head(fx.rec_pin->as<CtcTargetArgs>(fx.rec_lab_bytes), n, fx.blank,
+                      static_cast<const char*>(fx.rec_pin->ptr) - fx.rec_mem->as<char>(), slot,
+                      fx.rec_mem->as<char>(fx.rec_head_bytes), fx.rec_tab_bytes, rt.stream());
+      DevMemP table = std::make_shared<DevMem>();
+      table->ptr = fx.rec_mem->as<char>(fx.rec_head_bytes);
+      table->bytes = fx.rec_tab_bytes;
+      table->borrowed = true;
+      table->keep = fx.rec_mem;
+      band_launch(tab, false, "band_forward_score", abytes, &op->fwd_table, &table);
+      op->head = true;
+      fx.rec_pending = false;
+      fx.rec_pin.reset();
+      rec_lock.unlock();
+    } else {
+      if (rec_lock.owns_lock()) {
+        rec_lock.unlock();
+        batch_targets_settle(fx);
+      }
+      band_launch(tab, false, "band_forward_score", abytes, fuse_copy ? nullptr : &op->fwd_table);
+    }
     if (fuse_copy) pend->done.store(true, std::memory_order_release);
     if (want_norm) {
       ch.nc_mem = op->arena;
@@ -1185,6 +1276,7 @@
         throw_invalid("[gtnx_batch_viterbi_align] a frame count beyond the rows the chain carries");
     }
   if (ch.w_pend) ch.w_pend->settle();
+  batch_targets_settle(fx);
   if (asg) {
     const int npl = asg_align_npl(fx.max_nodes);
     const size_t plane = asg_align_plane_bytes(T, npl);
@@ -1721,6 +1813,16 @@
   return r;
 }
 
+namespace {
+void batch_grad_settle(Batch& b) {
+  if (!b.grad_ones_due) return;
+  b.grad_ones_due = false;
+  if (b.g_dev) return;
+  alloc_grad(b, false);
+  launch_fill_f32(b.g_dev, 1.0f, size_t(b.n), Runtime::get().stream());
+}
+}
+
 void batch_backward(const BatchP& root, bool retain) {
   GTNX_HOST_T("batch.backward");
   if (root->tape_cleared)
@@ -1740,6 +1842,7 @@
     stack.pop_back();
     if (!b->calc_grad || !seen.insert(b.get()).second) continue;
     hold.push_back(b);
+    batch_grad_settle(*b);
     if (b->op) {
       order.push_back(b.get());
       for (auto& in : b->op->inputs) stack.push_back(in);
@@ -1816,6 +1919,67 @@
     }
 }
 
+namespace {
+BatchP subtract_backward_fused(const BatchP& a, const BatchP& b, void* items_dev) {
+  if (!g_step_fused.load(std::memory_order_relaxed) || !band_patch_enabled()) return nullptr;
+  if (!a || !b || a.get() == b.get() || a->n != b->n || a->n <= 1) return nullptr;
+  for (const Batch* x : {a.get(), b.get()})
+    if (x->kind != Batch::SCALAR || x->materialised || !x->op || !x->calc_grad || x->g_dev || x->dest || x->tape_cleared ||
+        x->grad_ones_due)
+      return nullptr;
+  auto* lop = dynamic_cast<BFsLinearOp*>(a->op.get());
+  auto* bop = dynamic_cast<BFsBandOp*>(b->op.get());
+  if (!lop || !bop || !bop->head || !bop->patched() || bop->through_acc || lop->inputs.size() != 1 || bop->inputs.size() != 1)
+    return nullptr;
+  const BatchP prodp = bop->inputs[0];
+  Batch& prod = *prodp;
+  if (prod.kind != Batch::PRODUCT || prod.materialised || !prod.op || prod.g_dev || prod.tape_cleared || !prod.fixed ||
+      !prod.chain || prod.n != a->n)
+    return nullptr;
+  Batch& fx = *prod.fixed;
+  Batch& ch = *prod.chain;
+  if (lop->inputs[0].get() != &ch || !ch.nc_norm || !ch.nc_rowlse || ch.nc_mem != bop->arena || a->v_dev != ch.nc_norm ||
+      b->v_dev != bop->arena->as<float>() || bop->pairs.size() != size_t(prod.n) || !bop->pairs[0].norm)
+    return nullptr;
+  if (ch.kind != Batch::LINEAR || fx.kind != Batch::CTC_TARGETS || fx.fal || !ch.calc_grad) return nullptr;
+  for (const Batch* x : {&ch, &fx})
+    if (x->op || x->leaf || x->materialised || x->g_dev || x->tape_cleared) return nullptr;
+  Runtime& rt = Runtime::get();
+  if (items_dev && !ptr_local_to(items_dev, rt.device())) return nullptr;
+
+  GTNX_HOST_T("batch.subtract_backward");
+  const int n = a->n;
+  auto sop = std::make_shared<BScalarOp>();
+  sop->kind = SK_SUBTRACT;
+  sop->inputs = {a, b};
+  BatchP r = result(Batch::SCALAR, n, sop);
+  if (items_dev) {
+    r->v_dev = static_cast<float*>(items_dev);
+  } else {
+    r->v_mem = rt.alloc(sizeof(float) * size_t(n));
+    r->v_dev = r->v_mem->as<float>();
+  }
+  const float* plus = nullptr;
+  const float* minus = seed_constants(rt, size_t(n), &plus);
+  GradTarget ge = grad_target(ch, false), gf;
+  if (fx.calc_grad) gf = grad_target(fx, false);
+  bop->sweep(minus, plus, ge.ptr, gf.ptr, r->v_dev);
+  r->grad_ones_due = true;
+  for (Batch* x : {r.get(), a.get(), b.get(), &prod}) {
+    x->op.reset();
+    x->tape_cleared = true;
+  }
+  return r;
+}
+}
+
+BatchP batch_subtract_backward(const BatchP& a, const BatchP& b, void* items_dev) {
+  if (BatchP r = subtract_backward_fused(a, b, items_dev)) return r;
+  BatchP r = batch_scalar(SK_SUBTRACT, a, b, items_dev);
+  batch_backward(r, false);
+  return r;
+}
+
 void batch_items_device(const BatchP& x, void* dev_out) {
   if (x->kind == Batch::SCALAR && !x->materialised) {
     if (static_cast<const void*>(x->v_dev) == dev_out) return;
@@ -1887,6 +2051,7 @@
     pad_fill(*x, static_cast<float*>(dev_out), offsets);
     return;
   }
+  batch_grad_settle(*x);
   if (!x->g_dev) throw_logic("[gtn::Graph::grad] Gradient not calculated yet.");
   Runtime& rt = Runtime::get();
   std::vector<AxpyArgs> ax;
diff --git a/gtn_amd/csrc/batch.h b/gtn_amd/csrc/batch.h
--- a/gtn_amd/csrc/batch.h
+++ b/gtn_amd/csrc/batch.h
@@ -1,6 +1,7 @@
 #pragma once
 
 #include <memory>
+#include <mutex>
 #include <vector>
 
 #include "ops.h"
@@ -42,6 +43,10 @@
   int max_label = -1, max_nodes = 0;
   DevMemP rec_mem;
   std::vector<size_t> rec_off;
+  PinnedMemP rec_pin;
+  bool rec_pending = false;
+  size_t rec_lab_bytes = 0, rec_head_bytes = 0, rec_tab_bytes = 0;
+  std::mutex rec_mu;
   bool fal = false;
   Graph trans;
   int trans_labels = 0;
@@ -71,6 +76,7 @@
   std::vector<int64_t> g_off;
   DevMemP dest_mem;
   float* dest = nullptr;
+  bool grad_ones_due = false;
 
   int64_t elem_size(int b) const;
   ~Batch();
@@ -102,6 +108,9 @@
 void batch_edit_distance_stats(int64_t* calls, int64_t* pairs);
 BatchP batch_scalar(ScalarKind k, const BatchP& a, const BatchP& b, void* items_dev = nullptr);
 void batch_backward(const BatchP& root, bool retain);
+BatchP batch_subtract_backward(const BatchP& a, const BatchP& b, void* items_dev = nullptr);
+bool batch_step_fused_set(bool on);
+void batch_targets_settle(Batch& x);
 void batch_items_host(const BatchP& x, float* out);
 void batch_items_device(const BatchP& x, void* dev_out);
 void batch_grads_device(const BatchP& x, void* dev_out, const int64_t* offsets);
diff --git a/gtn_amd/csrc/capi.cpp b/gtn_amd/csrc/capi.cpp
--- a/gtn_amd/csrc/capi.cpp
+++ b/gtn_amd/csrc/capi.cpp
@@ -808,6 +808,15 @@
 GTNX_API gtnx_status_t gtnx_batch_subtract_into(gtnx_batch_t a, gtnx_batch_t b, void* items_device, gtnx_batch_t* out) {
   return guard([&] { *out = HB(batch_scalar(SK_SUBTRACT, BH(a), BH(b), items_device)); });
 }
+GTNX_API gtnx_status_t gtnx_batch_subtract_backward(gtnx_batch_t a, gtnx_batch_t b, void* items_device, gtnx_batch_t* out) {
+  return guard([&] { *out = HB(batch_subtract_backward(BH(a), BH(b), items_device)); });
+}
+GTNX_API gtnx_status_t gtnx_batch_set_step_fused(int on, int* previous) {
+  return guard([&] {
+    const bool was = batch_step_fused_set(on != 0);
+    if (previous) *previous = was ? 1 : 0;
+  });
+}
 GTNX_API gtnx_status_t gtnx_batch_compose(gtnx_batch_t a, gtnx_batch_t b, gtnx_batch_t* out) {
   return guard([&] { *out = HB(batch_compose(BH(a), BH(b), false)); });
 }
diff --git a/gtn_amd/csrc/kernels.h b/gtn_amd/csrc/kernels.h
--- a/gtn_amd/csrc/kernels.h
+++ b/gtn_amd/csrc/kernels.h
@@ -388,6 +388,7 @@
   GTNX_G float* grad_em;
   GTNX_G float* grad_fixed;
   int64_t A;
+  GTNX_G float* loss;
 };
 struct BandDecode {
   const GTNX_G BandNode* nodes;
@@ -495,6 +496,8 @@
   int N, pad;
 };
 void launch_ctc_targets(const CtcTargetArgs* d_args, int n, int blank, hipStream_t st);
+void launch_ctc_head(const CtcTargetArgs* args, int n, int blank, int64_t lab_shift, const void* tab_src, void* tab_dst,
+                     size_t tab_bytes, hipStream_t st);
 struct AsgFalArgs {
   const GTNX_G int* labels;
   const GTNX_G float* trans_w;
diff --git a/gtn_amd/csrc/ops.h b/gtn_amd/csrc/ops.h
--- a/gtn_amd/csrc/ops.h
+++ b/gtn_amd/csrc/ops.h
@@ -42,7 +42,7 @@
 };
 int band_vec_ok(const BandPair& p);
 void band_launch(std::vector<std::pair<BandLaunchKey, BandPair>>& tab, bool backward, const char* prof_name = nullptr,
-                 double prof_bytes = 0.0, DevMemP* table_out = nullptr);
+                 double prof_bytes = 0.0, DevMemP* table_out = nullptr, const DevMemP* table_in = nullptr);
 void band_launch_patched(const DevMemP& table, int n, const BandLaunchKey& key, int max_ns, const BandPatch& patch,
                          const char* prof_name, double prof_bytes);
 
diff --git a/gtn_amd/csrc/ops_band.cpp b/gtn_amd/csrc/ops_band.cpp
--- a/gtn_amd/csrc/ops_band.cpp
+++ b/gtn_amd/csrc/ops_band.cpp
@@ -13,7 +13,7 @@
                        &patch);
 }
 void band_launch(std::vector<std::pair<BandLaunchKey, BandPair>>& tab, bool backward, const char* prof_name, double prof_bytes,
-                 DevMemP* table_out) {
+                 DevMemP* table_out, const DevMemP* table_in) {
   Runtime& rt = Runtime::get();
   if (table_out) table_out->reset();
   if (tab.empty()) return;
@@ -30,10 +30,16 @@
       return;
     }
   }
-  std::vector<BandPair> flat;
-  flat.reserve(tab.size());
-  for (auto& e : tab) flat.push_back(e.second);
-  DevMemP d = upload_vec(flat);
+  if (table_in && (!one_key || tab.size() < 2)) throw_logic("band_launch: a table on the device is one launch group");
+  DevMemP d;
+  if (table_in) {
+    d = *table_in;
+  } else {
+    std::vector<BandPair> flat;
+    flat.reserve(tab.size());
+    for (auto& e : tab) flat.push_back(e.second);
+    d = upload_vec(flat);
+  }
   const BandPair* dp = d->as<BandPair>();
   if (table_out && one_key) *table_out = d;
   std::unique_ptr<Runtime::Scope> prof(prof_name ? new Runtime::Scope(&rt, prof_name, prof_bytes) : nullptr);
diff --git a/gtn_amd/csrc/runtime.cpp b/gtn_amd/csrc/runtime.cpp
--- a/gtn_amd/csrc/runtime.cpp
+++ b/gtn_amd/csrc/runtime.cpp
@@ -608,12 +608,16 @@
   }
   HIP_CHECK(hipMemcpyAsync(pinned_dst, src, bytes, hipMemcpyDeviceToHost, stream_));
 }
-void Runtime::h2d_pinned(void* dst, const void* pinned_src, size_t bytes) {
-  if (!bytes) return;
+size_t Runtime::h2d_kernel_limit() {
   static const size_t lim = [] {
     const char* e = std::getenv("GTNX_H2D_KERNEL_BYTES");
     return e ? size_t(std::atol(e)) : size_t(1) << 20;
   }();
+  return lim;
+}
+void Runtime::h2d_pinned(void* dst, const void* pinned_src, size_t bytes) {
+  if (!bytes) return;
+  const size_t lim = h2d_kernel_limit();
   if (bytes <= lim && local_to(dst, device_)) {
     launch_copy_small(dst, pinned_src, bytes, stream_);
     return;
diff --git a/gtn_amd/csrc/runtime.h b/gtn_amd/csrc/runtime.h
--- a/gtn_amd/csrc/runtime.h
+++ b/gtn_amd/csrc/runtime.h
@@ -92,6 +92,7 @@
   void d2h_sync(void* dst, const void* src, size_t bytes);
   void d2d(void* dst, const void* src, size_t bytes);
   void h2d_pinned(void* dst, const void* pinned_src, size_t bytes);
+  static size_t h2d_kernel_limit();
   void d2h_pinned_async(void* pinned_dst, const void* src, size_t bytes);
 
   struct MirrorSlot {
diff --git a/include/gtn/batch.h b/include/gtn/batch.h
--- a/include/gtn/batch.h
+++ b/include/gtn/batch.h
@@ -118,6 +118,11 @@
   detail::check(gtnx_batch_subtract_into(a.handle(), b.handle(), itemsDevice, &out));
   return Batch::fromHandle(out);
 }
+inline Batch subtractBackward(const Batch& a, const Batch& b, void* itemsDevice = nullptr) {
+  gtnx_batch_t out;
+  detail::check(gtnx_batch_subtract_backward(a.handle(), b.handle(), itemsDevice, &out));
+  return Batch::fromHandle(out);
+}
 inline Batch compose(const Batch& a, const Batch& b) { return detail::batchBinary(&gtnx_batch_compose, a, b); }
 inline Batch intersect(const Batch& a, const Batch& b) { return detail::batchBinary(&gtnx_batch_intersect, a, b); }
 inline Batch forwardScore(const Batch& a) { return detail::batchUnary(&gtnx_batch_forward_score, a); }
diff --git a/include/gtn_amd.h b/include/gtn_amd.h
--- a/include/gtn_amd.h
+++ b/include/gtn_amd.h
@@ -146,6 +146,8 @@
 gtnx_status_t gtnx_batch_add(gtnx_batch_t a, gtnx_batch_t b, gtnx_batch_t* out);
 gtnx_status_t gtnx_batch_subtract(gtnx_batch_t a, gtnx_batch_t b, gtnx_batch_t* out);
 gtnx_status_t gtnx_batch_subtract_into(gtnx_batch_t a, gtnx_batch_t b, void* items_device, gtnx_batch_t* out);
+gtnx_status_t gtnx_batch_subtract_backward(gtnx_batch_t a, gtnx_batch_t b, void* items_device, gtnx_batch_t* out);
+gtnx_status_t gtnx_batch_set_step_fused(int on, int* previous);
 gtnx_status_t gtnx_batch_compose(gtnx_batch_t a, gtnx_batch_t b, gtnx_batch_t* out);
 gtnx_status_t gtnx_batch_intersect(gtnx_batch_t a, gtnx_batch_t b, gtnx_batch_t* out);
 gtnx_status_t gtnx_batch_forward_score(gtnx_batch_t a, gtnx_batch_t* out);
```
